# wang-xinyu/tensorrtx

Measured on AMD Instinct MI355X. Metric: images/sec @ batch=32 640x640 fp16 (yolov8n conv backbone + YoloLayer decode + NMS), higher is better.
Workload: dtype f16

## Files before the change

### include/trtx_hip.h

```cpp
#ifndef TRTX_HIP_H_
#define TRTX_HIP_H_

#include <stddef.h>
#include <stdint.h>

#ifdef __cplusplus
extern "C" {
#endif

#ifndef TRTX_NO_HIP_TYPES
struct ihipStream_t;
typedef struct ihipStream_t* trtx_stream_t;
#endif

#define TRTX_ABI_VERSION 1
#define TRTX_OK 0
#define TRTX_ERR_INVALID 1
#define TRTX_ERR_HIP 2
#define TRTX_ERR_WORKSPACE 3
#define TRTX_ERR_UNSUPPORTED 4
#define TRTX_ERR_NO_DEVICE 5
#define TRTX_ERR_IO 6
#define TRTX_ERR_STATE 7

const char* trtx_status_string(int32_t status);
int32_t trtx_abi_version(void);
int32_t trtx_device_count(void);


size_t trtx_yolo_decode_workspace(int batch, int net_h, int net_w, const int* strides, int n_levels);
int32_t trtx_yolo_decode(const float* const* inputs, int n_levels, int batch, int classes, int net_h, int net_w,
                         const int* strides, int max_out, float* output, void* workspace, size_t workspace_bytes,
                         trtx_stream_t stream);

int32_t trtx_yolo_decode_ex(const float* const* inputs, int n_levels, int batch, int classes, int net_h, int net_w,
                            const int* strides, int max_out, int n_kpt, float kpt_conf, int is_seg, int is_pose, int is_obb,
                            float* output, void* workspace, size_t workspace_bytes, trtx_stream_t stream);
size_t trtx_yolo_head_decode_workspace(int batch, int net_h, int net_w, const int* strides, int n_levels);
int32_t trtx_yolo_head_decode_nhwc(const void* const* heads, const int* ld, int n_levels, int batch, int classes,
                                   int net_h, int net_w, const int* strides, const float* dfl_weights, int max_out,
                                   float* output, void* workspace, size_t workspace_bytes, trtx_stream_t stream);
int32_t trtx_yolo_head_decode_nhwc_f32(const void* const* heads, const int* ld, int n_levels, int batch, int classes,
                                   int net_h, int net_w, const int* strides, const float* dfl_weights, int max_out,
                                   float* output, void* workspace, size_t workspace_bytes, trtx_stream_t stream);
int32_t trtx_yolo_task_head_decode_nhwc(const void* const* heads, const int* ld, const void* const* branches, const int* branch_ld,
                                        int n_levels, int batch, int classes, int net_h, int net_w, const int* strides,
                                        const float* dfl_weights, int max_out, int is_seg, int is_pose, int is_obb, int n_kpt,
                                        float kpt_conf, float* output, void* workspace, size_t workspace_bytes, trtx_stream_t stream);
int32_t trtx_yolo_task_head_decode_nhwc_f32(const void* const* heads, const int* ld, const void* const* branches, const int* branch_ld,
                                            int n_levels, int batch, int classes, int net_h, int net_w, const int* strides,
                                            const float* dfl_weights, int max_out, int is_seg, int is_pose, int is_obb, int n_kpt,
                                            float kpt_conf, float* output, void* workspace, size_t workspace_bytes, trtx_stream_t stream);

size_t trtx_yolo_nms_workspace(int batch);
int32_t trtx_yolo_nms(const float* decode_out, int batch, int max_out, float conf_thresh, float nms_thresh,
                      int32_t* keep_idx, int32_t* keep_cnt, float* keep_det, void* workspace, size_t workspace_bytes,
                      trtx_stream_t stream);


size_t trtx_yolov5_decode_workspace(int batch, const int* grid_w, const int* grid_h, int n_levels);
int32_t trtx_yolov5_decode(const float* const* inputs, int n_levels, int batch, int classes, int net_h, int net_w,
                           const int* grid_w, const int* grid_h, const float* anchors, int max_out, int is_segmentation,
                           float* output, void* workspace, size_t workspace_bytes, trtx_stream_t stream);
size_t trtx_yolov5_head_decode_workspace(int batch, const int* grid_w, const int* grid_h, int n_levels);
int32_t trtx_yolov5_head_decode_nhwc(const void* const* heads, const int* ld, int n_levels, int batch, int classes, int net_h, int net_w,
                                     const int* grid_w, const int* grid_h, const float* anchors, int max_out, float* output,
                                     void* workspace, size_t workspace_bytes, trtx_stream_t stream);
int32_t trtx_yolov5_head_decode_nhwc_f32(const void* const* heads, const int* ld, int n_levels, int batch, int classes, int net_h, int net_w,
                                         const int* grid_w, const int* grid_h, const float* anchors, int max_out, float* output,
                                         void* workspace, size_t workspace_bytes, trtx_stream_t stream);
int32_t trtx_yolo_nms_obb(const float* decode_out, int batch, int max_out, float conf_thresh, float nms_thresh, int32_t* keep_idx,
                          int32_t* keep_cnt, float* keep_det, void* workspace, size_t workspace_bytes, trtx_stream_t stream);
int32_t trtx_yolo_postprocess_gpu_obb(const float* decode_out, int batch, int max_out, float conf_thresh, float nms_thresh, float* out,
                                      trtx_stream_t stream);
int32_t trtx_yolov5_nms(const float* decode_out, int batch, int max_out, float conf_thresh, float nms_thresh, int32_t* keep_idx,
                        int32_t* keep_cnt, float* keep_det, void* workspace, size_t workspace_bytes, trtx_stream_t stream);
int32_t trtx_seg_masks(const float* decode_out, int det_floats, int box_format, const int32_t* keep_idx, const int32_t* keep_cnt, int batch,
                       int max_out, int max_keep, const float* proto, int mask_h, int mask_w, int net_h, int net_w, float* masks,
                       trtx_stream_t stream);

void trtx_letterbox_matrix(int src_w, int src_h, int dst_w, int dst_h, float* d2s_out );
int32_t trtx_letterbox_batch(const void* const* src, const int* src_w, const int* src_h, int batch, float* dst, int dst_w, int dst_h,
                             trtx_stream_t stream);
int32_t trtx_preprocess_init(int max_image_size, int ring_depth);
void trtx_preprocess_destroy(void);
int32_t trtx_batch_preprocess(const void* const* src_host, const int* src_w, const int* src_h, int batch, float* dst, int dst_w, int dst_h,
                              trtx_stream_t stream);

int32_t trtx_yolo_postprocess_gpu(const float* decode_out, int batch, int max_out, float conf_thresh, float nms_thresh,
                                  float* out, trtx_stream_t stream);

int32_t trtx_mish(const float* in, float* out, size_t n, trtx_stream_t stream);

size_t trtx_retina_decode_output_floats(int net_h, int net_w);
size_t trtx_retina_decode_workspace(int batch, int net_h, int net_w);
int32_t trtx_retina_decode(const float* const* inputs, int batch, int net_h, int net_w, float* output, void* workspace,
                           size_t workspace_bytes, trtx_stream_t stream);
size_t trtx_retina_nms_workspace(int batch, int net_h, int net_w);
int32_t trtx_retina_nms(const float* decode_out, int batch, int net_h, int net_w, double conf_thresh, float nms_thresh,
                        int max_keep, int32_t* keep_idx, int32_t* keep_cnt, float* keep_det, void* workspace,
                        size_t workspace_bytes, trtx_stream_t stream);

size_t trtx_rpn_decode_workspace(int batch, int num_anchors, int height, int width);
int32_t trtx_rpn_decode(int batch, const float* scores, const float* deltas, int height, int width, int image_height,
                        int image_width, float stride, const float* anchors_host, int num_anchors, int top_n,
                        float* out_scores, float* out_boxes, void* workspace, size_t workspace_bytes,
                        trtx_stream_t stream);
size_t trtx_sorted_nms_workspace(int batch, int n);
int32_t trtx_rpn_nms(int batch, const float* scores, const float* boxes, int pre_nms_topk, int post_nms_topk,
                     float nms_thresh, float* out_boxes, void* workspace, size_t workspace_bytes,
                     trtx_stream_t stream);
int32_t trtx_roi_align(int batch, const float* boxes, const float* features, int pooler_resolution, float spatial_scale,
                       int sampling_ratio, int num_proposals, int channels, int feature_h, int feature_w, float* out,
                       trtx_stream_t stream);
int32_t trtx_roi_align_nhwc_f16(int batch, const float* boxes, const void* features, int ld_in, int pooler_resolution,
                                float spatial_scale, int sampling_ratio, int num_proposals, int channels, int feature_h,
                                int feature_w, void* out, int ld_out, trtx_stream_t stream);
int32_t trtx_roi_align_nhwc_f16_strided(int batch, const float* boxes, const void* features, int ld_in, int pooler_resolution,
                                        float spatial_scale, int sampling_ratio, int num_proposals, int channels, int feature_h,
                                        int feature_w, void* out, int ld_out, int bin_step, trtx_stream_t stream);
size_t trtx_predictor_decode_workspace(int batch, int num_boxes, int num_classes);
int32_t trtx_predictor_decode(int batch, const float* scores, const float* deltas, const float* proposals, int num_boxes,
                              int num_classes, int image_height, int image_width, const float* bbox_reg_weights_host,
                              float* out_scores, float* out_boxes, float* out_classes, void* workspace,
                              size_t workspace_bytes, trtx_stream_t stream);
int32_t trtx_batched_nms(int nms_method, int batch, const float* scores, const float* boxes, const float* classes,
                         int count, int detections_per_im, float nms_thresh, float* out_scores, float* out_boxes,
                         float* out_classes, void* workspace, size_t workspace_bytes, trtx_stream_t stream);

int32_t trtx_mask_rcnn_inference(int batch, const float* labels, const float* masks, int detections_per_im, int output_size,
                                 int num_classes, float* out_masks, trtx_stream_t stream);

#define TRTX_ACT_NONE 0
#define TRTX_ACT_RELU 1
#define TRTX_ACT_SIGMOID 2
#define TRTX_ACT_SILU 3
#define TRTX_ACT_LEAKY 4
#define TRTX_ACT_TANH 5
int32_t trtx_conv_packed_dims(int cout, int cin_pad, int kh, int kw, int32_t* cout_pad, int32_t* kpad, int32_t* bn);
int32_t trtx_conv_pack_weights_f16(const float* w_kcrs, int cout, int cin, int kh, int kw, int cin_pad,
                                   const float* ch_scale, uint16_t* packed);
int32_t trtx_op_conv2d_nhwc_f16(const void* in, int N, int H, int W, int Cin, int ld_in, const void* wpacked,
                                const float* bias, void* out, int Cout, int ld_out, int kh, int kw, int sh, int sw,
                                int ph, int pw, int act1, const void* residual, int ld_res, int act2,
                                trtx_stream_t stream);
int32_t trtx_op_conv2d_tactics(int N, int H, int W, int Cin, int ld_in, int Cout, int ld_out, int kh, int kw, int sh, int sw, int ph, int pw,
                               int has_residual, int ld_res, int32_t* out6, int32_t max_out);
int32_t trtx_op_conv_force_tactic(const int32_t* tactic6);
int32_t trtx_conv_packed_dims_f32(int cout, int cin_pad, int kh, int kw, int32_t* cout_pad, int32_t* kpad, int32_t* cink);
int32_t trtx_conv_pack_weights_f32(const float* w_kcrs, int cout, int cin, int kh, int kw, int cin_pad, const float* ch_scale, float* packed);
int32_t trtx_op_conv2d_nhwc_f32(const void* in, int N, int H, int W, int Cin, int ld_in, const void* wpacked, const float* bias, void* out, int Cout,
                                int ld_out, int kh, int kw, int sh, int sw, int ph, int pw, int act1, const void* residual, int ld_res, int act2,
                                const int32_t* tile4, trtx_stream_t stream);
int32_t trtx_op_conv2d_tactics_f32(int N, int H, int W, int Cin, int ld_in, int Cout, int ld_out, int kh, int kw, int sh, int sw, int ph, int pw,
                                   int has_residual, int ld_res, int32_t* out4, int32_t max_out);
int32_t trtx_conv_pack_weights_i8(const float* w_kcrs, int cout, int cin, int kh, int kw, const float* ch_scale, int8_t* packed, float* wscale_out,
                                  int32_t* cout_pad_out, int32_t* kpad_out);
int32_t trtx_op_conv2d_nhwc_i8(const void* in, int N, int H, int W, int Cin, int ld_in, const void* wpacked, const float* cscale, const float* bias, void* out,
                               int out_is_i8, float out_inv_scale, int Cout, int ld_out, int kh, int kw, int sh, int sw, int ph, int pw, int act1,
                               const void* residual, int res_is_i8, float res_scale, int ld_res, int act2, trtx_stream_t stream);
int32_t trtx_conv_pack_weights_grouped_f16(const float* w_kcrs, int cout, int cin_g, int kh, int kw, const float* ch_scale, uint16_t* packed,
                                           int32_t* kpad_out);
int32_t trtx_op_conv2d_grouped_nhwc_f16(const void* in, int N, int H, int W, int Cin, int ld_in, const void* wpacked, const float* bias, void* out,
                                        int Cout, int ld_out, int groups, int k, int pad, int act1, const void* residual, int ld_res, int act2,
                                        trtx_stream_t stream);
int32_t trtx_op_conv2d_dw_nhwc(const void* in, int dtype, int N, int H, int W, int C, int ld_in, const float* w_taps_c, const float* bias, void* out, int ld_out,
                               const void* residual, int ld_res, int k, int stride, int pad, int dilation, int act1, float alpha1, int act2, float alpha2,
                               trtx_stream_t stream);
int32_t trtx_op_psa_attention_f16(const void* qkv, int ld_qkv, void* out, int ld_out, void* vimg, int ld_v, int B, int heads, int N, int kd, int hd, float scale,
                                  trtx_stream_t stream);
int32_t trtx_op_area_attention_f16(const void* qkv, int ld_qkv, void* out, int ld_out, void* vimg, int ld_v, int B, int heads, int N, int area, int kd, int hd,
                                   float scale, trtx_stream_t stream);
int32_t trtx_op_poison_lds(void* device_word, trtx_stream_t stream);
int32_t trtx_op_nchw_f32_to_nhwc_f16(const float* in, void* out, int N, int C, int H, int W, int Cpad, int ld_out,
                                     trtx_stream_t stream);
int32_t trtx_op_nhwc_f16_to_nchw_f32(const void* in, float* out, int N, int C, int H, int W, int ld_in,
                                     trtx_stream_t stream);

typedef struct trtx_builder trtx_builder;
typedef struct trtx_network trtx_network;
typedef struct trtx_hostmem trtx_hostmem;
typedef struct trtx_engine trtx_engine;
typedef struct trtx_context trtx_context;
typedef struct trtx_plugin trtx_plugin;

#define TRTX_MAX_DIMS 8
typedef struct trtx_dims {
    int32_t nb;
    int64_t d[TRTX_MAX_DIMS];
} trtx_dims;

#define TRTX_DTYPE_FLOAT 0
#define TRTX_DTYPE_HALF 1
#define TRTX_DTYPE_INT8 2
#define TRTX_DTYPE_INT32 3
#define TRTX_ACTIVATION_RELU 0
#define TRTX_ACTIVATION_SIGMOID 1
#define TRTX_ACTIVATION_TANH 2
#define TRTX_ACTIVATION_LEAKY_RELU 3
#define TRTX_POOLING_MAX 0
#define TRTX_POOLING_AVERAGE 1
#define TRTX_ELEMENTWISE_SUM 0
#define TRTX_ELEMENTWISE_PROD 1
#define TRTX_ELEMENTWISE_MAX 2
#define TRTX_ELEMENTWISE_MIN 3
#define TRTX_ELEMENTWISE_SUB 4
#define TRTX_ELEMENTWISE_DIV 5
#define TRTX_ELEMENTWISE_POW 6
#define TRTX_SCALE_UNIFORM 0
#define TRTX_SCALE_CHANNEL 1
#define TRTX_SCALE_ELEMENTWISE 2
#define TRTX_REDUCE_SUM 0
#define TRTX_REDUCE_PROD 1
#define TRTX_REDUCE_MAX 2
#define TRTX_REDUCE_MIN 3
#define TRTX_REDUCE_AVG 4
#define TRTX_MATMUL_NONE 0
#define TRTX_MATMUL_TRANSPOSE 1
#define TRTX_MATMUL_VECTOR 2
#define TRTX_RESIZE_NEAREST 0
#define TRTX_RESIZE_LINEAR 1
#define TRTX_FLAG_FP16 0
#define TRTX_FLAG_INT8 1
#define TRTX_P_STRIDE 1
#define TRTX_P_PADDING 2
#define TRTX_P_DILATION 3
#define TRTX_P_GROUPS 4
#define TRTX_P_ALPHA 5
#define TRTX_P_BETA 6
#define TRTX_P_AXIS 7
#define TRTX_P_RESHAPE 8
#define TRTX_P_FIRST_TRANSPOSE 9
#define TRTX_P_SECOND_TRANSPOSE 10
#define TRTX_P_RESIZE_MODE 11
#define TRTX_P_RESIZE_SCALES 12
#define TRTX_P_RESIZE_OUT_DIMS 13
#define TRTX_P_AVG_EXCLUSIVE 14
#define TRTX_P_KERNEL 15
#define TRTX_P_NB_OUT 16

typedef struct trtx_plugin_vtbl {
    void* self;
    int32_t (*get_nb_outputs)(void* self);
    int32_t (*get_output_dims)(void* self, int32_t index, const trtx_dims* inputs, int32_t nb_inputs, trtx_dims* out);
    int32_t (*configure)(void* self, const trtx_dims* in, int32_t nb_in, const trtx_dims* out, int32_t nb_out,
                         int32_t max_batch);
    int32_t (*initialize)(void* self);
    void (*terminate)(void* self);
    size_t (*workspace_size)(void* self, int32_t max_batch);
    int32_t (*enqueue)(void* self, int32_t batch, const void* const* inputs, void* const* outputs, void* workspace,
                       trtx_stream_t stream);
    size_t (*serialization_size)(void* self);
    void (*serialize)(void* self, void* buffer);
    const char* (*plugin_type)(void* self);
    const char* (*plugin_version)(void* self);
    int32_t (*clone)(void* self, struct trtx_plugin_vtbl* out);
    void (*destroy)(void* self);
} trtx_plugin_vtbl;

typedef struct trtx_plugin_field {
    const char* name;
    const void* data;
    int32_t type;
    int32_t length;
} trtx_plugin_field;

typedef struct trtx_creator_vtbl {
    void* self;
    const char* (*plugin_name)(void* self);
    const char* (*plugin_version)(void* self);
    int32_t (*create)(void* self, const char* name, const trtx_plugin_field* fields, int32_t nb_fields,
                      trtx_plugin_vtbl* out);
    int32_t (*deserialize)(void* self, const char* name, const void* data, size_t length, trtx_plugin_vtbl* out);
} trtx_creator_vtbl;

int32_t trtx_registry_register(const trtx_creator_vtbl* creator);
int32_t trtx_registry_get(const char* name, const char* version, trtx_creator_vtbl* out);

typedef struct trtx_wts trtx_wts;
int32_t trtx_wts_load(const char* path, trtx_wts** out);
int32_t trtx_wts_count(const trtx_wts* w);
int32_t trtx_wts_entry(const trtx_wts* w, int32_t i, const char** name, const float** values, int64_t* count);
int32_t trtx_wts_find(const trtx_wts* w, const char* name, const float** values, int64_t* count);
void trtx_wts_free(trtx_wts* w);

int32_t trtx_builder_create(trtx_builder** out);
void trtx_builder_destroy(trtx_builder* b);
int32_t trtx_builder_set_max_batch(trtx_builder* b, int32_t n);
int32_t trtx_builder_set_flag(trtx_builder* b, int32_t flag, int32_t on);
int32_t trtx_builder_set_workspace(trtx_builder* b, size_t bytes);
typedef struct trtx_calibrator_vtbl {
    void* self;
    int32_t (*get_batch_size)(void* self);
    int32_t (*get_batch)(void* self, void** bindings, const char* const* names, int32_t nb_bindings);
    const void* (*read_cache)(void* self, size_t* length);
    void (*write_cache)(void* self, const void* cache, size_t length);
    int32_t (*get_algorithm)(void* self);
} trtx_calibrator_vtbl;
int32_t trtx_builder_set_max_aux_streams(trtx_builder* b, int32_t n);
int32_t trtx_builder_set_int8_calibrator(trtx_builder* b, const trtx_calibrator_vtbl* calibrator);
float trtx_int8_entropy_threshold(const double* hist, int32_t bins, float range);
float trtx_int8_clip_limited_threshold(const double* hist, int32_t bins, float range, float thr, double limit);
int32_t trtx_network_create(trtx_builder* b, uint32_t flags, trtx_network** out);
void trtx_network_destroy(trtx_network* n);
const char* trtx_network_last_error(const trtx_network* n);

int32_t trtx_add_input(trtx_network* n, const char* name, int32_t dtype, const trtx_dims* dims);
int32_t trtx_add_convolution(trtx_network* n, int32_t input, int32_t nb_out, int32_t kh, int32_t kw,
                             const float* kernel, int64_t kernel_count, const float* bias, int64_t bias_count);
int32_t trtx_add_deconvolution(trtx_network* n, int32_t input, int32_t nb_out, int32_t kh, int32_t kw,
                               const float* kernel, int64_t kernel_count, const float* bias, int64_t bias_count);
int32_t trtx_add_fully_connected(trtx_network* n, int32_t input, int32_t nb_out, const float* kernel,
                                 int64_t kernel_count, const float* bias, int64_t bias_count);
int32_t trtx_add_activation(trtx_network* n, int32_t input, int32_t type);
int32_t trtx_add_pooling(trtx_network* n, int32_t input, int32_t type, int32_t kh, int32_t kw);
int32_t trtx_add_scale(trtx_network* n, int32_t input, int32_t mode, const float* shift, int64_t shift_count,
                       const float* scale, int64_t scale_count, const float* power, int64_t power_count);
int32_t trtx_add_elementwise(trtx_network* n, int32_t a, int32_t b, int32_t op);
int32_t trtx_add_concatenation(trtx_network* n, const int32_t* inputs, int32_t nb_inputs);
int32_t trtx_add_slice(trtx_network* n, int32_t input, const trtx_dims* start, const trtx_dims* size,
                       const trtx_dims* stride);
int32_t trtx_add_shuffle(trtx_network* n, int32_t input);
int32_t trtx_add_resize(trtx_network* n, int32_t input);
int32_t trtx_add_softmax(trtx_network* n, int32_t input);
int32_t trtx_add_matrix_multiply(trtx_network* n, int32_t a, int32_t op_a, int32_t b, int32_t op_b);
int32_t trtx_add_constant(trtx_network* n, const trtx_dims* dims, const float* values, int64_t count);
int32_t trtx_add_reduce(trtx_network* n, int32_t input, int32_t op, uint32_t axes, int32_t keep_dims);
int32_t trtx_add_identity(trtx_network* n, int32_t input);
int32_t trtx_add_plugin_v2(trtx_network* n, const int32_t* inputs, int32_t nb_inputs, const trtx_plugin_vtbl* plugin);

int32_t trtx_layer_nb_outputs(const trtx_network* n, int32_t layer);
int32_t trtx_layer_output(const trtx_network* n, int32_t layer, int32_t index);
int32_t trtx_layer_set_name(trtx_network* n, int32_t layer, const char* name);
int32_t trtx_layer_set_ints(trtx_network* n, int32_t layer, int32_t param, const int32_t* v, int32_t count);
int32_t trtx_layer_set_floats(trtx_network* n, int32_t layer, int32_t param, const float* v, int32_t count);
int32_t trtx_layer_set_dims(trtx_network* n, int32_t layer, int32_t param, const trtx_dims* d);
int32_t trtx_tensor_get_dims(const trtx_network* n, int32_t tensor, trtx_dims* out);
int32_t trtx_tensor_set_name(trtx_network* n, int32_t tensor, const char* name);
const char* trtx_tensor_get_name(const trtx_network* n, int32_t tensor);
int32_t trtx_mark_output(trtx_network* n, int32_t tensor);

int32_t trtx_build_serialized(trtx_builder* b, trtx_network* n, trtx_hostmem** out);
const void* trtx_hostmem_data(const trtx_hostmem* m);
size_t trtx_hostmem_size(const trtx_hostmem* m);
void trtx_hostmem_destroy(trtx_hostmem* m);
int32_t trtx_hostmem_create(const void* data, size_t size, trtx_hostmem** out);
int32_t trtx_plan_describe(const void* plan, size_t size, int32_t lowered, char** json_out);
void trtx_string_free(char* s);

int32_t trtx_engine_deserialize(const void* plan, size_t size, trtx_engine** out);
int32_t trtx_engine_serialize(const trtx_engine* e, trtx_hostmem** out);
void trtx_engine_destroy(trtx_engine* e);
int32_t trtx_engine_nb_bindings(const trtx_engine* e);
int32_t trtx_engine_binding_index(const trtx_engine* e, const char* name);
const char* trtx_engine_binding_name(const trtx_engine* e, int32_t index);
int32_t trtx_engine_binding_is_input(const trtx_engine* e, int32_t index);
int32_t trtx_engine_binding_dims(const trtx_engine* e, int32_t index, trtx_dims* out);
int32_t trtx_engine_binding_dtype(const trtx_engine* e, int32_t index);
int32_t trtx_engine_max_batch(const trtx_engine* e);
size_t trtx_engine_device_memory(const trtx_engine* e);
int32_t trtx_engine_tactics(const trtx_engine* e, char** json_out);
int32_t trtx_engine_device(const trtx_engine* e);
int32_t trtx_context_create(trtx_engine* e, trtx_context** out);
void trtx_context_destroy(trtx_context* c);
int32_t trtx_context_enqueue(trtx_context* c, int32_t batch, void* const* bindings, trtx_stream_t stream);
int32_t trtx_context_enqueue_frames(trtx_context* c, int32_t batch, const void* const* frames, const int32_t* frame_w, const int32_t* frame_h,
                                    void* const* bindings, trtx_stream_t stream);
int32_t trtx_context_set_tensor_address(trtx_context* c, const char* name, void* ptr);
int32_t trtx_context_enqueue_v3(trtx_context* c, trtx_stream_t stream);
int32_t trtx_context_profile(trtx_context* c, int32_t batch, void* const* bindings, trtx_stream_t stream,
                             char** json_out);

#ifdef __cplusplus
}
#endif
#endif
```

### tensorrtx_amd/capi.py

```python
import ctypes
import os

_HERE = os.path.dirname(os.path.abspath(__file__))
_LIB = None


class TrtxError(RuntimeError):
    def __init__(self, status, what):
        self.status = status
        msg = lib().trtx_status_string(status).decode() if _LIB is not None else "?"
        super().__init__(f"{what}: status {status} ({msg})")


def lib_path() -> str:
    return os.environ.get("TRTX_HIP_LIB") or os.path.join(_HERE, "lib", "libtrtx_hip.so")


def hip_runtimes_mapped():
    seen = []
    with open("/proc/self/maps") as f:
        for line in f:
            path = line.rsplit(" ", 1)[-1].strip()
            if "libamdhip64" in os.path.basename(path) and path not in seen:
                seen.append(path)
    return seen


def _bind_hip_runtime():
    import torch


def lib() -> ctypes.CDLL:
    global _LIB
    if _LIB is None:
        p = lib_path()
        if not os.path.exists(p):
            raise ImportError(f"{p} is missing: run `python -c 'import __graft_entry__ as g; g.build()'` "
                              "(hipcc --offload-arch=gfx950); there is no CPU fallback")
        _bind_hip_runtime()
        L = ctypes.CDLL(p)
        rts = hip_runtimes_mapped()
        if len(rts) > 1:
            raise ImportError("two HIP runtimes are mapped in this process (%s): something dlopened a HIP library "
                              "before tensorrtx_amd/torch; import torch (or tensorrtx_amd) first" % ", ".join(rts))
        L.trtx_status_string.restype = ctypes.c_char_p
        L.trtx_status_string.argtypes = [ctypes.c_int32]
        L.trtx_yolo_decode_workspace.restype = ctypes.c_size_t
        _LIB = L
    return _LIB


def check(status, what):
    if status != 0:
        raise TrtxError(status, what)


def _stream():
    import torch
    return ctypes.c_void_p(torch.cuda.current_stream().cuda_stream)


def _p(t):
    return ctypes.c_void_p(t.data_ptr() if t is not None else 0)


DET_FLOATS = 90


def yolo_decode(inputs, classes, net_h, net_w, strides, max_out=1000, out=None):
    import torch
    L = lib()
    B = inputs[0].shape[0]
    n = len(inputs)
    ins = [x.contiguous() for x in inputs]
    for x in ins:
        assert x.is_cuda and x.dtype == torch.float32
    arr = (ctypes.c_void_p * n)(*[x.data_ptr() for x in ins])
    st = (ctypes.c_int * n)(*strides)
    ws_bytes = L.trtx_yolo_decode_workspace(B, net_h, net_w, st, n)
    ws = torch.empty(ws_bytes, dtype=torch.uint8, device=ins[0].device)
    if out is None:
        out = torch.empty((B, 1 + max_out * DET_FLOATS), dtype=torch.float32, device=ins[0].device)
    check(L.trtx_yolo_decode(arr, n, B, classes, net_h, net_w, st, max_out, _p(out), _p(ws),
                             ctypes.c_size_t(ws_bytes), _stream()), "trtx_yolo_decode")
    return out


def yolo_nms(decode_out, max_out=1000, conf_thresh=0.5, nms_thresh=0.45, with_dets=True):
    import torch
    L = lib()
    B = decode_out.shape[0]
    dev = decode_out.device
    keep_idx = torch.full((B, max_out), -1, dtype=torch.int32, device=dev)
    keep_cnt = torch.zeros((B,), dtype=torch.int32, device=dev)
    keep_det = torch.zeros((B, max_out, 6), dtype=torch.float32, device=dev) if with_dets else None
    L.trtx_yolo_nms_workspace.restype = ctypes.c_size_t
    ws_bytes = L.trtx_yolo_nms_workspace(B)
    ws = torch.empty((ws_bytes,), dtype=torch.uint8, device=dev)
    check(L.trtx_yolo_nms(_p(decode_out), B, max_out, ctypes.c_float(conf_thresh), ctypes.c_float(nms_thresh),
                          _p(keep_idx), _p(keep_cnt), _p(keep_det), _p(ws), ctypes.c_size_t(ws_bytes), _stream()),
          "trtx_yolo_nms")
    return keep_idx, keep_cnt, keep_det


def yolo_decode_ex(inputs, classes, net_h, net_w, strides, max_out=1000, nk=17, kpt_conf=0.0, seg=False, pose=False, obb=False):
    import torch
    L = lib()
    B, n = inputs[0].shape[0], len(inputs)
    ins = [x.contiguous() for x in inputs]
    arr = (ctypes.c_void_p * n)(*[x.data_ptr() for x in ins])
    st = (ctypes.c_int * n)(*strides)
    ws_bytes = L.trtx_yolo_decode_workspace(B, net_h, net_w, st, n)
    ws = torch.empty(ws_bytes, dtype=torch.uint8, device=ins[0].device)
    out = torch.zeros((B, 1 + max_out * DET_FLOATS), dtype=torch.float32, device=ins[0].device)
    check(L.trtx_yolo_decode_ex(arr, n, B, classes, net_h, net_w, st, max_out, nk, ctypes.c_float(kpt_conf), int(seg), int(pose), int(obb),
                                _p(out), _p(ws), ctypes.c_size_t(ws_bytes), _stream()), "trtx_yolo_decode_ex")
    return out


def _head_table(tensors):
    n = len(tensors)
    return (ctypes.c_void_p * n)(*[x.data_ptr() for x in tensors]), (ctypes.c_int * n)(*[x.shape[-1] for x in tensors])


def yolo_head_decode_nhwc(heads, classes, net_h, net_w, strides, dfl_w, max_out=1000):
    import torch
    L = lib()
    B, n = heads[0].shape[0], len(heads)
    hp, hl = _head_table(heads)
    st = (ctypes.c_int * n)(*strides)
    L.trtx_yolo_head_decode_workspace.restype = ctypes.c_size_t
    ws_bytes = L.trtx_yolo_head_decode_workspace(B, net_h, net_w, st, n)
    ws = torch.empty(ws_bytes, dtype=torch.uint8, device=heads[0].device)
    out = torch.zeros(B, 1 + max_out * DET_FLOATS, dtype=torch.float32, device=heads[0].device)
    fn = L.trtx_yolo_head_decode_nhwc_f32 if heads[0].dtype == torch.float32 else L.trtx_yolo_head_decode_nhwc
    check(fn(hp, hl, n, B, classes, net_h, net_w, st, _p(dfl_w), max_out, _p(out), _p(ws), ctypes.c_size_t(ws_bytes), _stream()),
          "trtx_yolo_head_decode_nhwc")
    return out


def yolo_task_head_decode_nhwc(heads, branches, classes, net_h, net_w, strides, dfl_w, max_out=1000, nk=17, kpt_conf=0.0, seg=False,
                               pose=False, obb=False):
    import torch
    L = lib()
    B, n = heads[0].shape[0], len(heads)
    hp, hl = _head_table(heads)
    bp, bl = _head_table(branches)
    st = (ctypes.c_int * n)(*strides)
    L.trtx_yolo_head_decode_workspace.restype = ctypes.c_size_t
    ws_bytes = L.trtx_yolo_head_decode_workspace(B, net_h, net_w, st, n)
    ws = torch.empty(ws_bytes, dtype=torch.uint8, device=heads[0].device)
    out = torch.zeros(B, 1 + max_out * DET_FLOATS, dtype=torch.float32, device=heads[0].device)
    fn = L.trtx_yolo_task_head_decode_nhwc_f32 if heads[0].dtype == torch.float32 else L.trtx_yolo_task_head_decode_nhwc
    check(fn(hp, hl, bp, bl, n, B, classes, net_h, net_w, st, _p(dfl_w), max_out, int(seg), int(pose), int(obb), nk, ctypes.c_float(kpt_conf),
             _p(out), _p(ws), ctypes.c_size_t(ws_bytes), _stream()), "trtx_yolo_task_head_decode_nhwc")
    return out


def yolo_nms_obb(decode_out, max_out=1000, conf_thresh=0.5, nms_thresh=0.45):
    import torch
    L = lib()
    B, dev = decode_out.shape[0], decode_out.device
    keep_idx = torch.full((B, max_out), -1, dtype=torch.int32, device=dev)
    keep_cnt = torch.zeros((B,), dtype=torch.int32, device=dev)
    keep_det = torch.zeros((B, max_out, 7), dtype=torch.float32, device=dev)
    L.trtx_yolo_nms_workspace.restype = ctypes.c_size_t
    ws_bytes = L.trtx_yolo_nms_workspace(B)
    ws = torch.empty((ws_bytes,), dtype=torch.uint8, device=dev)
    check(L.trtx_yolo_nms_obb(_p(decode_out), B, max_out, ctypes.c_float(conf_thresh), ctypes.c_float(nms_thresh), _p(keep_idx), _p(keep_cnt),
                              _p(keep_det), _p(ws), ctypes.c_size_t(ws_bytes), _stream()), "trtx_yolo_nms_obb")
    return keep_idx, keep_cnt, keep_det


def yolo_postprocess_gpu_obb(decode_out, max_out=1000, conf_thresh=0.5, nms_thresh=0.45):
    import torch
    out = torch.empty((decode_out.shape[0], 1 + max_out * 8), dtype=torch.float32, device=decode_out.device)
    check(lib().trtx_yolo_postprocess_gpu_obb(_p(decode_out), decode_out.shape[0], max_out, ctypes.c_float(conf_thresh), ctypes.c_float(nms_thresh),
                                              _p(out), _stream()), "trtx_yolo_postprocess_gpu_obb")
    return out


DET5_FLOATS = 38


def yolov5_decode(inputs, classes, net_h, net_w, grids, anchors, max_out=1000, is_seg=False):
    import numpy as np
    import torch
    L = lib()
    n = len(inputs)
    ins = [x.contiguous() for x in inputs]
    B, dev = ins[0].shape[0], ins[0].device
    arr = (ctypes.c_void_p * n)(*[x.data_ptr() for x in ins])
    gw = (ctypes.c_int * n)(*[g[0] for g in grids])
    gh = (ctypes.c_int * n)(*[g[1] for g in grids])
    an = np.ascontiguousarray(anchors, dtype=np.float32).reshape(n, 6)
    L.trtx_yolov5_decode_workspace.restype = ctypes.c_size_t
    ws_bytes = L.trtx_yolov5_decode_workspace(B, gw, gh, n)
    ws = torch.empty(max(ws_bytes, 256), dtype=torch.uint8, device=dev)
    out = torch.zeros((B, 1 + max_out * DET5_FLOATS), dtype=torch.float32, device=dev)
    check(L.trtx_yolov5_decode(arr, n, B, classes, net_h, net_w, gw, gh, an.ctypes.data_as(ctypes.c_void_p), max_out, 1 if is_seg else 0,
                               _p(out), _p(ws), ctypes.c_size_t(ws_bytes), _stream()), "trtx_yolov5_decode")
    return out


def yolov5_head_decode_nhwc(heads, classes, net_h, net_w, grids, anchors, max_out=1000):
    import numpy as np
    import torch
    L = lib()
    B, n, dev = heads[0].shape[0], len(heads), heads[0].device
    hp, hl = _head_table(heads)
    gw = (ctypes.c_int * n)(*[g[0] for g in grids])
    gh = (ctypes.c_int * n)(*[g[1] for g in grids])
    an = np.ascontiguousarray(anchors, dtype=np.float32).reshape(n, 6)
    L.trtx_yolov5_head_decode_workspace.restype = ctypes.c_size_t
    ws_bytes = L.trtx_yolov5_head_decode_workspace(B, gw, gh, n)
    ws = torch.empty(max(ws_bytes, 256), dtype=torch.uint8, device=dev)
    out = torch.zeros((B, 1 + max_out * DET5_FLOATS), dtype=torch.float32, device=dev)
    fn = L.trtx_yolov5_head_decode_nhwc_f32 if heads[0].dtype == torch.float32 else L.trtx_yolov5_head_decode_nhwc
    check(fn(hp, hl, n, B, classes, net_h, net_w, gw, gh, an.ctypes.data_as(ctypes.c_void_p), max_out, _p(out), _p(ws), ctypes.c_size_t(ws_bytes),
             _stream()), "trtx_yolov5_head_decode_nhwc")
    return out


def yolov5_nms(decode_out, max_out=1000, conf_thresh=0.5, nms_thresh=0.45):
    import torch
    L = lib()
    B, dev = decode_out.shape[0], decode_out.device
    keep_idx = torch.full((B, max_out), -1, dtype=torch.int32, device=dev)
    keep_cnt = torch.zeros((B,), dtype=torch.int32, device=dev)
    keep_det = torch.zeros((B, max_out, 6), dtype=torch.float32, device=dev)
    L.trtx_yolo_nms_workspace.restype = ctypes.c_size_t
    ws_bytes = L.trtx_yolo_nms_workspace(B)
    ws = torch.empty((ws_bytes,), dtype=torch.uint8, device=dev)
    check(L.trtx_yolov5_nms(_p(decode_out), B, max_out, ctypes.c_float(conf_thresh), ctypes.c_float(nms_thresh), _p(keep_idx), _p(keep_cnt),
                            _p(keep_det), _p(ws), ctypes.c_size_t(ws_bytes), _stream()), "trtx_yolov5_nms")
    return keep_idx, keep_cnt, keep_det


def seg_masks(decode_out, keep_idx, keep_cnt, proto, net_h, net_w, max_keep, box_format=0, out=None):
    import torch
    B, max_out = keep_idx.shape
    assert decode_out.shape[0] == B and (decode_out.shape[1] - 1) % max_out == 0
    det_floats = (decode_out.shape[1] - 1) // max_out
    assert proto.dim() == 4 and proto.shape[0] == B and proto.shape[1] == 32
    mask_h, mask_w = int(proto.shape[2]), int(proto.shape[3])
    for t, dt in ((decode_out, torch.float32), (keep_idx, torch.int32), (keep_cnt, torch.int32), (proto, torch.float32)):
        assert t.is_cuda and t.dtype == dt and t.is_contiguous()
    if out is None:
        out = torch.zeros((B, max(max_keep, 0), mask_h, mask_w), dtype=torch.float32, device=proto.device)
    assert out.is_cuda and out.dtype == torch.float32 and out.is_contiguous() and out.numel() >= B * max(max_keep, 0) * mask_h * mask_w
    check(lib().trtx_seg_masks(_p(decode_out), det_floats, box_format, _p(keep_idx), _p(keep_cnt), B, max_out, max_keep, _p(proto), mask_h,
                               mask_w, net_h, net_w, _p(out), _stream()), "trtx_seg_masks")
    return out


def yolo_postprocess_gpu(decode_out, max_out=1000, conf_thresh=0.5, nms_thresh=0.45):
    import torch
    B = decode_out.shape[0]
    out = torch.empty((B, 1 + max_out * 7), dtype=torch.float32, device=decode_out.device)
    check(lib().trtx_yolo_postprocess_gpu(_p(decode_out), B, max_out, ctypes.c_float(conf_thresh), ctypes.c_float(nms_thresh),
                                          _p(out), _stream()), "trtx_yolo_postprocess_gpu")
    return out


ACT = {"none": 0, "relu": 1, "sigmoid": 2, "silu": 3, "leaky": 4, "tanh": 5, "mish": 6}


def _hw(v):
    if isinstance(v, (tuple, list)):
        h, w = v
        return int(h), int(w)
    return int(v), int(v)


def pack_conv_weights_f16(w_kcrs, cin_pad=None, ch_scale=None):
    import numpy as np
    L = lib()
    w = np.ascontiguousarray(w_kcrs, dtype=np.float32)
    cout, cin, kh, kw = w.shape
    cin_pad = cin_pad or (cin + 7) // 8 * 8
    cp, kp, bn = ctypes.c_int32(), ctypes.c_int32(), ctypes.c_int32()
    check(L.trtx_conv_packed_dims(cout, cin_pad, kh, kw, ctypes.byref(cp), ctypes.byref(kp), ctypes.byref(bn)),
          "trtx_conv_packed_dims")
    packed = np.zeros((cp.value, kp.value), dtype=np.uint16)
    sc = None
    if ch_scale is not None:
        sc = np.ascontiguousarray(ch_scale, dtype=np.float32)
    check(L.trtx_conv_pack_weights_f16(w.ctypes.data_as(ctypes.c_void_p), cout, cin, kh, kw, cin_pad,
                                       sc.ctypes.data_as(ctypes.c_void_p) if sc is not None else None,
                                       packed.ctypes.data_as(ctypes.c_void_p)), "trtx_conv_pack_weights_f16")
    return packed, cp.value, kp.value, bn.value


def conv2d_nhwc_f16(x, wpacked, bias, cout, kh, kw, stride, pad, act1="none", residual=None, act2="none",
                    out=None, out_ld=None):
    import torch
    L = lib()
    N, H, W, Cin = x.shape
    (sh, sw), (ph, pw) = _hw(stride), _hw(pad)
    Ho = (H + 2 * ph - kh) // sh + 1
    Wo = (W + 2 * pw - kw) // sw + 1
    if out is None:
        out = torch.empty((N, Ho, Wo, cout), dtype=torch.float16, device=x.device)
    ld_out = out_ld or out.shape[-1]
    check(L.trtx_op_conv2d_nhwc_f16(_p(x), N, H, W, Cin, x.stride(2), _p(wpacked), _p(bias), _p(out), cout, ld_out,
                                    kh, kw, sh, sw, ph, pw, ACT[act1], _p(residual),
                                    residual.stride(2) if residual is not None else 0, ACT[act2], _stream()),
          "trtx_op_conv2d_nhwc_f16")
    return out


def pack_conv_weights_grouped_f16(w_kcrs, ch_scale=None):
    import numpy as np
    L = lib()
    w = np.ascontiguousarray(w_kcrs, dtype=np.float32)
    cout, cin_g, kh, kw = w.shape
    kp = ctypes.c_int32()
    check(L.trtx_conv_pack_weights_grouped_f16(w.ctypes.data_as(ctypes.c_void_p), cout, cin_g, kh, kw, None, None, ctypes.byref(kp)),
          "trtx_conv_pack_weights_grouped_f16 (dims)")
    packed = np.zeros((cout, kp.value), dtype=np.uint16)
    sc = None if ch_scale is None else np.ascontiguousarray(ch_scale, dtype=np.float32)
    check(L.trtx_conv_pack_weights_grouped_f16(w.ctypes.data_as(ctypes.c_void_p), cout, cin_g, kh, kw,
                                               sc.ctypes.data_as(ctypes.c_void_p) if sc is not None else None,
                                               packed.ctypes.data_as(ctypes.c_void_p), ctypes.byref(kp)), "trtx_conv_pack_weights_grouped_f16")
    return packed


def conv2d_grouped_nhwc_f16(x, wpacked, bias, cout, groups, k, pad, act1="none", residual=None, act2="none", out=None, out_ld=None):
    import torch
    N, H, W, Cin = x.shape
    if out is None:
        out = torch.empty((N, H + 2 * pad - k + 1, W + 2 * pad - k + 1, cout), dtype=torch.float16, device=x.device)
    check(lib().trtx_op_conv2d_grouped_nhwc_f16(_p(x), N, H, W, Cin, x.stride(2), _p(wpacked), _p(bias), _p(out), cout, out_ld or out.shape[-1], groups, k,
                                                pad, ACT[act1], _p(residual), residual.stride(2) if residual is not None else 0, ACT[act2], _stream()),
          "trtx_op_conv2d_grouped_nhwc_f16")
    return out


def conv2d_dw_nhwc(x, w, bias, k, stride, act1="none", residual=None, act2="none", out=None, out_ld=None, alpha1=0.1, alpha2=0.1, pad=None, dilation=1):
    import numpy as np
    import torch
    N, H, W, C = x.shape
    assert x.dtype in (torch.float16, torch.float32) and (residual is None or residual.dtype == x.dtype)
    pad = k // 2 if pad is None else pad
    Ho, Wo = (H + 2 * pad - dilation * (k - 1) - 1) // stride + 1, (W + 2 * pad - dilation * (k - 1) - 1) // stride + 1
    taps = np.ascontiguousarray(np.asarray(w, dtype=np.float32).reshape(C, k * k).T)
    wg = torch.from_numpy(taps).to(x.device)
    if out is None:
        out = torch.empty((N, Ho, Wo, C), dtype=x.dtype, device=x.device)
    assert out.dtype == x.dtype
    check(lib().trtx_op_conv2d_dw_nhwc(_p(x), 1 if x.dtype == torch.float16 else 0, N, H, W, C, x.stride(2), _p(wg), _p(bias), _p(out),
                                       out_ld or out.shape[-1], _p(residual), residual.stride(2) if residual is not None else 0, k, stride, pad, dilation,
                                       ACT[act1], ctypes.c_float(alpha1), ACT[act2], ctypes.c_float(alpha2), _stream()), "trtx_op_conv2d_dw_nhwc")
    return out


def _attention(fn, what, qkv, heads, scale, out, vimg, out_ld, v_ld, qkv_ld, kd, hd, extra):
    import torch
    B, N, _ = qkv.shape
    for t in (qkv, out, vimg):
        assert t.is_cuda and t.dtype == torch.float16
    check(fn(_p(qkv), qkv_ld or qkv.stride(1), _p(out), out_ld or out.stride(1), _p(vimg), v_ld or vimg.stride(1), B, heads, N, *extra, kd, hd,
             ctypes.c_float(scale), _stream()), what)
    return out, vimg


def psa_attention(qkv, heads, scale, out=None, vimg=None, out_ld=None, v_ld=None, qkv_ld=None, kd=32, hd=64):
    import torch
    B, N, _ = qkv.shape
    out = torch.empty((B, N, heads * hd), dtype=torch.float16, device=qkv.device) if out is None else out
    vimg = torch.empty((B, N, heads * hd), dtype=torch.float16, device=qkv.device) if vimg is None else vimg
    return _attention(lib().trtx_op_psa_attention_f16, "trtx_op_psa_attention_f16", qkv, heads, scale, out, vimg, out_ld, v_ld, qkv_ld, kd, hd, ())


def area_attention(qkv, heads, area, scale, out=None, vimg=None, out_ld=None, v_ld=None, qkv_ld=None, kd=32, hd=32):
    import torch
    B, N, _ = qkv.shape
    out = torch.empty((B, N, heads * hd), dtype=torch.float16, device=qkv.device) if out is None else out
    vimg = torch.empty((B, N, heads * hd), dtype=torch.float16, device=qkv.device) if vimg is None else vimg
    return _attention(lib().trtx_op_area_attention_f16, "trtx_op_area_attention_f16", qkv, heads, scale, out, vimg, out_ld, v_ld, qkv_ld, kd, hd, (area,))


def pack_conv_weights_f32(w_kcrs, cin_pad=None, ch_scale=None):
    import numpy as np
    L = lib()
    w = np.ascontiguousarray(w_kcrs, dtype=np.float32)
    cout, cin, kh, kw = w.shape
    cin_pad = cin_pad or (cin + 3) // 4 * 4
    cp, kp, ck = ctypes.c_int32(), ctypes.c_int32(), ctypes.c_int32()
    check(L.trtx_conv_packed_dims_f32(cout, cin_pad, kh, kw, ctypes.byref(cp), ctypes.byref(kp), ctypes.byref(ck)), "trtx_conv_packed_dims_f32")
    packed = np.zeros((cp.value, kp.value), dtype=np.float32)
    sc = np.ascontiguousarray(ch_scale, dtype=np.float32) if ch_scale is not None else None
    check(L.trtx_conv_pack_weights_f32(w.ctypes.data_as(ctypes.c_void_p), cout, cin, kh, kw, cin_pad,
                                       sc.ctypes.data_as(ctypes.c_void_p) if sc is not None else None,
                                       packed.ctypes.data_as(ctypes.c_void_p)), "trtx_conv_pack_weights_f32")
    return packed, cp.value, kp.value, ck.value


def conv2d_nhwc_f32(x, wpacked, bias, cout, kh, kw, stride, pad, act1="none", residual=None, act2="none", out=None, out_ld=None, tile=None):
    import torch
    L = lib()
    N, H, W, Cin = x.shape
    if bias is not None and bias.numel() < (cout + 15) // 16 * 16:
        raise ValueError(f"bias holds {bias.numel()} floats, the fp32 tile reads cout_pad = {(cout + 15) // 16 * 16}")
    (sh, sw), (ph, pw) = _hw(stride), _hw(pad)
    Ho = (H + 2 * ph - kh) // sh + 1
    Wo = (W + 2 * pw - kw) // sw + 1
    if out is None:
        out = torch.empty((N, Ho, Wo, cout), dtype=torch.float32, device=x.device)
    ld_out = out_ld or out.shape[-1]
    t2 = (ctypes.c_int32 * 4)(*tile) if tile is not None else None
    check(L.trtx_op_conv2d_nhwc_f32(_p(x), N, H, W, Cin, x.stride(2), _p(wpacked), _p(bias), _p(out), cout, ld_out, kh, kw, sh, sw, ph, pw,
                                    ACT[act1], _p(residual), residual.stride(2) if residual is not None else 0, ACT[act2], t2, _stream()),
          "trtx_op_conv2d_nhwc_f32")
    return out


def conv2d_tactics_f32(N, H, W, Cin, Cout, k, stride, pad, residual=False, ld_in=None, ld_out=None, ld_res=None, max_out=32):
    arr = (ctypes.c_int32 * (4 * max_out))()
    (kh, kw), (sh, sw), (ph, pw) = _hw(k), _hw(stride), _hw(pad)
    n = lib().trtx_op_conv2d_tactics_f32(N, H, W, Cin, ld_in or Cin, Cout, ld_out or Cout, kh, kw, sh, sw, ph, pw, 1 if residual else 0,
                                         (ld_res or Cout) if residual else 0, arr, max_out)
    return [(arr[4 * i], arr[4 * i + 1], arr[4 * i + 2], arr[4 * i + 3]) for i in range(n)]


def poison_lds(sync=True):
    import torch
    w = torch.zeros(4, dtype=torch.int32, device="cuda")
    check(lib().trtx_op_poison_lds(_p(w), _stream()), "trtx_op_poison_lds")
    if sync:
        torch.cuda.synchronize()


def conv2d_tactics(N, H, W, Cin, Cout, k, stride, pad, residual=False, ld_in=None, ld_out=None, ld_res=None, max_out=32):
    arr = (ctypes.c_int32 * (6 * max_out))()
    (kh, kw), (sh, sw), (ph, pw) = _hw(k), _hw(stride), _hw(pad)
    n = lib().trtx_op_conv2d_tactics(N, H, W, Cin, ld_in or Cin, Cout, ld_out or Cout, kh, kw, sh, sw, ph, pw, 1 if residual else 0,
                                     (ld_res or Cout) if residual else 0, arr, max_out)
    return [tuple(arr[6 * i + j] for j in range(6)) for i in range(n)]


def conv_force_tactic(tactic=None):
    if tactic is None:
        check(lib().trtx_op_conv_force_tactic(None), "trtx_op_conv_force_tactic")
    else:
        check(lib().trtx_op_conv_force_tactic((ctypes.c_int32 * 6)(*tactic)), "trtx_op_conv_force_tactic")


def pack_conv_weights_i8(w_kcrs, ch_scale=None):
    import numpy as np
    L = lib()
    w = np.ascontiguousarray(w_kcrs, dtype=np.float32)
    cout, cin, kh, kw = w.shape
    cp, kp = ctypes.c_int32(), ctypes.c_int32()
    check(L.trtx_conv_pack_weights_i8(w.ctypes.data_as(ctypes.c_void_p), cout, cin, kh, kw, None, None, None, ctypes.byref(cp), ctypes.byref(kp)),
          "trtx_conv_pack_weights_i8 (dims)")
    packed = np.zeros((cp.value, kp.value), dtype=np.int8)
    wscale = np.zeros((cp.value,), dtype=np.float32)
    sc = None if ch_scale is None else np.ascontiguousarray(ch_scale, dtype=np.float32)
    check(L.trtx_conv_pack_weights_i8(w.ctypes.data_as(ctypes.c_void_p), cout, cin, kh, kw,
                                      sc.ctypes.data_as(ctypes.c_void_p) if sc is not None else None, packed.ctypes.data_as(ctypes.c_void_p),
                                      wscale.ctypes.data_as(ctypes.c_void_p), ctypes.byref(cp), ctypes.byref(kp)), "trtx_conv_pack_weights_i8")
    return packed, wscale


def conv2d_nhwc_i8(x_i8, wpacked, cscale, bias, cout, kh, kw, stride, pad, act1="none", out_scale=None, residual=None, res_scale=1.0,
                   act2="none", out=None, out_ld=None):
    import torch
    N, H, W, Cin = x_i8.shape
    (sh, sw), (ph, pw) = _hw(stride), _hw(pad)
    Ho, Wo = (H + 2 * ph - kh) // sh + 1, (W + 2 * pw - kw) // sw + 1
    if out is None:
        out = torch.empty((N, Ho, Wo, cout), dtype=torch.int8 if out_scale else torch.float16, device=x_i8.device)
    res_i8 = residual is not None and residual.dtype == torch.int8
    check(lib().trtx_op_conv2d_nhwc_i8(_p(x_i8), N, H, W, Cin, x_i8.stride(2), _p(wpacked), _p(cscale), _p(bias), _p(out), 1 if out_scale else 0,
                                       ctypes.c_float(1.0 / out_scale if out_scale else 0.0), cout, out_ld or out.shape[-1], kh, kw, sh, sw, ph, pw, ACT[act1],
                                       _p(residual), 1 if res_i8 else 0, ctypes.c_float(res_scale), residual.stride(2) if residual is not None else 0,
                                       ACT[act2], _stream()), "trtx_op_conv2d_nhwc_i8")
    return out
```

### tensorrtx_amd/csrc/kernels/conv_stem.hip

```cpp
#include <hip/hip_fp16.h>
#include <hip/hip_runtime.h>
#include <stdint.h>
#include <stdlib.h>
#include <string.h>

#include "../common.h"
#include "act.h"
#include "kernels.h"

namespace trtx {
namespace {

template <int COUT>
__global__ __launch_bounds__(256) void conv_stem_kernel(const ConvArgs p) {
    extern __shared__ __attribute__((aligned(16))) float s_w[];
    const float* __restrict__ w = static_cast<const float*>(p.wgt);
    const int K = p.kh * p.kw * p.Cin;
    for (int i = threadIdx.x; i < K * COUT; i += 256) s_w[i] = w[i];
    __syncthreads();
    const long m = (long)blockIdx.x * 256 + threadIdx.x;
    if (m >= p.M) return;
    const int wo = (int)(m % p.Wo);
    const long t = m / p.Wo;
    const int ho = (int)(t % p.Ho);
    const long n = t / p.Ho;
    const float* __restrict__ in = static_cast<const float*>(p.in) + n * p.Cin * p.H * p.W;
    float acc[COUT];
#pragma unroll
    for (int c = 0; c < COUT; ++c) acc[c] = p.bias ? p.bias[c] : 0.f;
    const int hi0 = ho * p.stride_h - p.pad_h, wi0 = wo * p.stride_w - p.pad_w;
    int tap = 0;
    for (int c = 0; c < p.Cin; ++c) {
        const float* plane = in + (long)c * p.H * p.W;
        for (int r = 0; r < p.kh; ++r) {
            const int hi = hi0 + r;
            const bool hok = (unsigned)hi < (unsigned)p.H;
            for (int q = 0; q < p.kw; ++q, ++tap) {
                const int wi = wi0 + q;
                float x = 0.f;
                if (hok && (unsigned)wi < (unsigned)p.W) x = plane[(long)hi * p.W + wi];
                const float4* wr = reinterpret_cast<const float4*>(s_w + tap * COUT);
#pragma unroll
                for (int c4 = 0; c4 < COUT / 4; ++c4) {
                    const float4 wv = wr[c4];
                    acc[c4 * 4 + 0] = fmaf(x, wv.x, acc[c4 * 4 + 0]);
                    acc[c4 * 4 + 1] = fmaf(x, wv.y, acc[c4 * 4 + 1]);
                    acc[c4 * 4 + 2] = fmaf(x, wv.z, acc[c4 * 4 + 2]);
                    acc[c4 * 4 + 3] = fmaf(x, wv.w, acc[c4 * 4 + 3]);
                }
            }
        }
    }
    _Float16* __restrict__ out = static_cast<_Float16*>(p.out) + m * p.ld_out;
#pragma unroll
    for (int c8 = 0; c8 < COUT / 8; ++c8) {
        half8 v;
#pragma unroll
        for (int e = 0; e < 8; ++e) v[e] = round_to_half(act_stem(acc[c8 * 8 + e], p.act1, p.alpha1));
        *reinterpret_cast<half8*>(out + c8 * 8) = v;
    }
}

typedef __attribute__((address_space(3))) void* lds_ptr_t;

constexpr int kStemTW = 64, kStemTH = 4;

struct StemGeom {
    int PR, PCA;
    int tiles_x, tiles_y;
    int chunks;
};

struct FramePack {
    StemFrame img[kStemMaxFrames];
};

struct AxisSample {
    float pos;
    int low;
    float l;
};
__device__ __forceinline__ AxisSample frame_axis(float m, float z, int d) {
#pragma clang fp contract(off)
    AxisSample a;
    a.pos = m * (float)d + z + 0.5f;
    a.low = (int)floorf(a.pos);
    a.l = a.pos - (float)a.low;
    return a;
}
__device__ __forceinline__ void frame_pixel(const StemFrame& im, const AxisSample& cx, const AxisSample& cy, float& r, float& g, float& b) {
#pragma clang fp contract(off)
    float c0, c1, c2;
    if (cx.pos <= -1 || cx.pos >= im.w || cy.pos <= -1 || cy.pos >= im.h) {
        c0 = c1 = c2 = 128.0f;
    } else {
        const int x_low = cx.low, y_low = cy.low, x_high = x_low + 1, y_high = y_low + 1;
        const float lx = cx.l, ly = cy.l, hx = 1 - lx, hy = 1 - ly;
        const float w1 = hy * hx, w2 = hy * lx, w3 = ly * hx, w4 = ly * lx;
        const uint8_t* base = static_cast<const uint8_t*>(im.src);
        const size_t line = (size_t)im.w * 3;
        float v[4][3];
#pragma unroll
        for (int q = 0; q < 4; ++q) {
            const int yy = q < 2 ? y_low : y_high, xx = (q & 1) ? x_high : x_low;
            const bool in = (q < 2 ? y_low >= 0 : y_high < im.h) && ((q & 1) ? x_high < im.w : x_low >= 0);
            const uint8_t* px = base + (size_t)(in ? yy : 0) * line + (size_t)(in ? xx : 0) * 3;
#pragma unroll
            for (int c = 0; c < 3; ++c) v[q][c] = in ? (float)px[c] : 128.0f;
        }
        c0 = w1 * v[0][0] + w2 * v[1][0] + w3 * v[2][0] + w4 * v[3][0];
        c1 = w1 * v[0][1] + w2 * v[1][1] + w3 * v[2][1] + w4 * v[3][1];
        c2 = w1 * v[0][2] + w2 * v[1][2] + w3 * v[2][2] + w4 * v[3][2];
    }
    r = c2 / 255.0f;
    g = c1 / 255.0f;
    b = c0 / 255.0f;
}

template <int NFRAG, int KS>
struct StemRegs {
    half8 wf[NFRAG][KS];
    int l_off[KS][8];
    float bias4[NFRAG][4];
};
template <int NFRAG, int KS>
__device__ __forceinline__ void stem_setup(const ConvArgs& p, const StemGeom& g, StemRegs<NFRAG, KS>& R);
template <int NFRAG, int KS>
__device__ __forceinline__ void stem_compute(const ConvArgs& p, const StemGeom& g, const StemRegs<NFRAG, KS>& R, const float* s_patch, int n, int tx0, int ty0, int shift);
template <int NFRAG, int KS>
__device__ __forceinline__ void stem_stage2(const ConvArgs& p, const StemGeom& g, const float* s_patch, int n, int tx0, int ty0, int shift) {
    StemRegs<NFRAG, KS> R;
    stem_setup<NFRAG, KS>(p, g, R);
    stem_compute<NFRAG, KS>(p, g, R, s_patch, n, tx0, ty0, shift);
}

template <int NFRAG, int KS>
__global__ __launch_bounds__(256) void conv_stem_frames_kernel(const ConvArgs p, const StemGeom g, const FramePack fr) {
    extern __shared__ __attribute__((aligned(16))) float s_patch[];
    const int tid = threadIdx.x;
    int t = blockIdx.x;
    const int tx0 = (t % g.tiles_x) * kStemTW;
    t /= g.tiles_x;
    const int ty0 = (t % g.tiles_y) * kStemTH;
    const int n = t / g.tiles_y;
    const int hi_start = ty0 * p.stride_h - p.pad_h;
    const int wi_start = tx0 * p.stride_w - p.pad_w;
    const int al_start = (wi_start >= 0 ? wi_start : wi_start - 3) / 4 * 4;
    const int shift = wi_start - al_start;
    const StemFrame& im = fr.img[n];
    const int plane = g.PR * g.PCA;
    const float inv_pca = 1.0f / (float)g.PCA;
    for (int e = tid; e < plane; e += 256) {
        int pr = (int)((float)e * inv_pca);
        int pc = e - pr * g.PCA;
        if (pc < 0) { --pr; pc += g.PCA; }
        if (pc >= g.PCA) { ++pr; pc -= g.PCA; }
        const int hi = hi_start + pr, wi = al_start + pc;
        float r = 0.f, gg = 0.f, b = 0.f;
        if ((unsigned)hi < (unsigned)p.H && (unsigned)wi < (unsigned)p.W) {
            const AxisSample cx = frame_axis(im.d2s[0], im.d2s[2], wi), cy = frame_axis(im.d2s[4], im.d2s[5], hi);
            frame_pixel(im, cx, cy, r, gg, b);
        }
        s_patch[e] = r;
        s_patch[plane + e] = gg;
        s_patch[2 * plane + e] = b;
    }
    __syncthreads();
    stem_stage2<NFRAG, KS>(p, g, s_patch, n, tx0, ty0, shift);
}

template <int NFRAG, int KS>
__global__ __launch_bounds__(256) void conv_stem_lds_kernel(const ConvArgs p, const StemGeom g, unsigned in_bytes, int total_tiles) {
    extern __shared__ __attribute__((aligned(16))) float s_patch[];
    const int tid = threadIdx.x;
    const int wave = tid >> 6;
    StemRegs<NFRAG, KS> R;
    stem_setup<NFRAG, KS>(p, g, R);
    for (int tile = blockIdx.x; tile < total_tiles; tile += gridDim.x) {
    int t = tile;
    const int tx0 = (t % g.tiles_x) * kStemTW;
    t /= g.tiles_x;
    const int ty0 = (t % g.tiles_y) * kStemTH;
    const int n = t / g.tiles_y;
    const int hi_start = ty0 * p.stride_h - p.pad_h;
    const int wi_start = tx0 * p.stride_w - p.pad_w;
    const int al_start = (wi_start >= 0 ? wi_start : wi_start - 3) / 4 * 4;
    const int shift = wi_start - al_start;
    {
        const __amdgpu_buffer_rsrc_t rs = __builtin_amdgcn_make_buffer_rsrc(const_cast<void*>(p.in), 0, in_bytes, 0x00020000);
        const int cpr = g.PCA / 4;
        const float inv_cpr = 1.0f / (float)cpr, inv_pr = 1.0f / (float)g.PR;
        for (int base = 0; base < g.chunks; base += 256) {
            const int ci = base + tid;
            int row = (int)((float)ci * inv_cpr);
            int cq = ci - row * cpr;
            if (cq < 0) { --row; cq += cpr; }
            if (cq >= cpr) { ++row; cq -= cpr; }
            int c = (int)((float)row * inv_pr);
            int pr = row - c * g.PR;
            if (pr < 0) { --c; pr += g.PR; }
            if (pr >= g.PR) { ++c; pr -= g.PR; }
            const int hi = hi_start + pr, wi = al_start + cq * 4;
            const bool ok = ci < g.chunks && (unsigned)hi < (unsigned)p.H && wi >= 0 && wi + 3 < p.W;
            const unsigned off = ok ? (unsigned)(((((long)n * p.Cin + c) * p.H + hi) * p.W + wi) * 4) : 0x80000000u;
            __builtin_amdgcn_raw_ptr_buffer_load_lds(rs, (lds_ptr_t)(s_patch + (size_t)(base + wave * 64) * 4), 16, off, 0, 0, 0);
        }
    }
    asm volatile("s_waitcnt vmcnt(0)" ::: "memory");
    __syncthreads();
    if (p.W & 3) {
        const int cpr = g.PCA / 4, rows = p.Cin * g.PR, wtail = p.W & ~3;
        const int cq = (wtail - al_start) >> 2;
        if (cq >= 0 && cq < cpr && wtail >= al_start) {
            const float* __restrict__ src = static_cast<const float*>(p.in);
            for (int rrow = tid; rrow < rows; rrow += 256) {
                const int c = rrow / g.PR, pr = rrow - c * g.PR, hi = hi_start + pr;
                if ((unsigned)hi >= (unsigned)p.H) continue;
                const size_t base = (((size_t)n * p.Cin + c) * p.H + hi) * p.W;
                for (int e = 0; e < 4; ++e)
                    if (wtail + e < p.W) s_patch[((size_t)rrow * cpr + cq) * 4 + e] = src[base + wtail + e];
            }
        }
        __syncthreads();
    }
    stem_compute<NFRAG, KS>(p, g, R, s_patch, n, tx0, ty0, shift);
    __syncthreads();
    }
}

template <int NFRAG, int KS>
__device__ __forceinline__ void stem_setup(const ConvArgs& p, const StemGeom& g, StemRegs<NFRAG, KS>& R) {
    const int lane = threadIdx.x & 63;
    const int khw = p.kh * p.kw;
    const int K = khw * p.Cin;
    const float* __restrict__ w = static_cast<const float*>(p.wgt);
    const int kq = (lane >> 4) * 8;
    auto& wf = R.wf;
    auto& l_off = R.l_off;
    auto& bias4 = R.bias4;
    const float inv_khw = 1.0f / (float)khw, inv_kw = 1.0f / (float)p.kw;
#pragma unroll
    for (int ks = 0; ks < KS; ++ks)
#pragma unroll
        for (int e = 0; e < 8; ++e) {
            const int k = ks * 32 + kq + e;
            const int c = (int)(((float)k + 0.5f) * inv_khw), rem = k - c * khw;
            const int r = (int)(((float)rem + 0.5f) * inv_kw), q = rem - r * p.kw;
            l_off[ks][e] = k < K ? (c * g.PR + r) * g.PCA + q : 0;
#pragma unroll
            for (int j = 0; j < NFRAG; ++j) {
                const int co = j * 16 + (lane & 15);
                const float wv = w[(size_t)(k < K ? k : K - 1) * p.Cout + (co < p.Cout ? co : p.Cout - 1)];
                wf[j][ks][e] = (k < K && co < p.Cout) ? (_Float16)wv : (_Float16)0.f;
            }
        }
    const int ch4 = (lane >> 4) * 4;
    const float* __restrict__ bsrc = p.bias ? p.bias : w;
#pragma unroll
    for (int j = 0; j < NFRAG; ++j)
#pragma unroll
        for (int e = 0; e < 4; ++e) {
            const int co = j * 16 + ch4 + e;
            const float bv = bsrc[co < p.Cout ? co : p.Cout - 1];
            bias4[j][e] = (p.bias && co < p.Cout) ? bv : 0.f;
        }
}

template <int NFRAG, int KS>
__device__ __forceinline__ void stem_compute(const ConvArgs& p, const StemGeom& g, const StemRegs<NFRAG, KS>& R, const float* s_patch, int n, int tx0, int ty0,
                                             int shift) {
    const int tid = threadIdx.x;
    const int lane = tid & 63;
    const int wave = tid >> 6;
    const int ch4 = (lane >> 4) * 4;
    const auto& wf = R.wf;
    const auto& l_off = R.l_off;
    const auto& bias4 = R.bias4;
    _Float16* __restrict__ out = static_cast<_Float16*>(p.out);
#pragma nounroll
    for (int gi = 0; gi < 4; ++gi) {
        const int ty = wave, tx = gi * 16 + (lane & 15);
        const int ho = ty0 + ty, wo = tx0 + tx;
        const float* src = s_patch + (ty * p.stride_h) * g.PCA + tx * p.stride_w + shift;
        floatx4 acc[NFRAG];
#pragma unroll
        for (int j = 0; j < NFRAG; ++j) acc[j] = floatx4{0.f, 0.f, 0.f, 0.f};
#pragma unroll
        for (int ks = 0; ks < KS; ++ks) {
            half8 xf;
#pragma unroll
            for (int e = 0; e < 8; ++e) xf[e] = (_Float16)src[l_off[ks][e]];
#pragma unroll
            for (int j = 0; j < NFRAG; ++j) acc[j] = __builtin_amdgcn_mfma_f32_16x16x32_f16(wf[j][ks], xf, acc[j], 0, 0, 0);
        }
        if (ho >= p.Ho || wo >= p.Wo) continue;
        const long m = ((long)n * p.Ho + ho) * p.Wo + wo;
#pragma unroll
        for (int j = 0; j < NFRAG; ++j) {
            const int co = j * 16 + ch4;
            if (co >= p.Cout) continue;
            half4 o;
            if (p.act1 == ACT_SILU) {
#pragma unroll
                for (int e = 0; e < 4; ++e) {
                    const float x = acc[j][e] + bias4[j][e];
                    o[e] = round_to_half(x * __builtin_amdgcn_rcpf(1.0f + __expf(-x)));
                }
            } else if (p.act1 == ACT_RELU) {
#pragma unroll
                for (int e = 0; e < 4; ++e) {
                    const float x = acc[j][e] + bias4[j][e];
                    o[e] = (_Float16)(x > 0.f ? x : 0.f);
                }
            } else {
#pragma unroll
                for (int e = 0; e < 4; ++e) o[e] = round_to_half(act_stem(acc[j][e] + bias4[j][e], p.act1, p.alpha1));
            }
            *reinterpret_cast<half4*>(out + m * p.ld_out + co) = o;
        }
    }
}

template <int NFRAG, int KS>
void launch_lds(const ConvArgs& a, hipStream_t s) {
    StemGeom g;
    g.PR = (kStemTH - 1) * a.stride_h + a.kh;
    g.PCA = ((kStemTW - 1) * a.stride_w + a.kw + 3 + 3) / 4 * 4;
    g.tiles_x = (a.Wo + kStemTW - 1) / kStemTW;
    g.tiles_y = (a.Ho + kStemTH - 1) / kStemTH;
    g.chunks = a.Cin * g.PR * g.PCA / 4;
    const size_t lds = (size_t)((g.chunks + 255) / 256 * 256) * 16;
    const unsigned in_bytes = (unsigned)((size_t)a.N * a.Cin * a.H * a.W * 4);
    const int total = a.N * g.tiles_x * g.tiles_y;
    static thread_local int resident[3] = {-1, 0, 0};
    int dev = 0;
    if (hipGetDevice(&dev) != hipSuccess) dev = 0;
    if (resident[0] != dev || resident[1] != (int)lds || resident[2] <= 0) {
        int per_cu = 0, cus = 0;
        if (hipOccupancyMaxActiveBlocksPerMultiprocessor(&per_cu, conv_stem_lds_kernel<NFRAG, KS>, 256, lds) != hipSuccess || per_cu < 1) per_cu = 1;
        if (hipDeviceGetAttribute(&cus, hipDeviceAttributeMultiprocessorCount, dev) != hipSuccess || cus < 1) cus = 256;
        (void)hipGetLastError();
        resident[0] = dev;
        resident[1] = (int)lds;
        resident[2] = per_cu * cus;
    }
    const int grid = total < resident[2] ? total : resident[2];
    hipLaunchKernelGGL((conv_stem_lds_kernel<NFRAG, KS>), dim3((unsigned)grid), dim3(256), lds, s, a, g, in_bytes, total);
}

template <int NFRAG, int KS>
void launch_frames(const ConvArgs& a0, const StemFrame* frames, hipStream_t s) {
    StemGeom g;
    g.PR = (kStemTH - 1) * a0.stride_h + a0.kh;
    g.PCA = ((kStemTW - 1) * a0.stride_w + a0.kw + 3 + 3) / 4 * 4;
    g.tiles_x = (a0.Wo + kStemTW - 1) / kStemTW;
    g.tiles_y = (a0.Ho + kStemTH - 1) / kStemTH;
    g.chunks = a0.Cin * g.PR * g.PCA / 4;
    const size_t lds = (size_t)((g.chunks + 255) / 256 * 256) * 16;
    for (int n0 = 0; n0 < a0.N; n0 += kStemMaxFrames) {
        ConvArgs a = a0;
        a.N = a0.N - n0 < kStemMaxFrames ? a0.N - n0 : kStemMaxFrames;
        a.M = a.N * a.Ho * a.Wo;
        a.out = static_cast<char*>(a0.out) + (size_t)n0 * a.Ho * a.Wo * a.ld_out * 2;
        FramePack fr;
        memset(&fr, 0, sizeof(fr));
        for (int i = 0; i < a.N; ++i) fr.img[i] = frames[n0 + i];
        hipLaunchKernelGGL((conv_stem_frames_kernel<NFRAG, KS>), dim3((unsigned)(a.N * g.tiles_x * g.tiles_y)), dim3(256), lds, s, a, g, fr);
    }
}

template <int COUT>
void launch(const ConvArgs& a, hipStream_t s) {
    const size_t lds = (size_t)a.kh * a.kw * a.Cin * COUT * sizeof(float);
    hipLaunchKernelGGL(conv_stem_kernel<COUT>, dim3((unsigned)((a.M + 255) / 256)), dim3(256), lds, s, a);
}

}

bool conv_stem_supported(const ConvArgs& a) {
    const bool cout_ok = a.Cout == 8 || a.Cout == 16 || a.Cout == 32 || a.Cout == 64;
    return cout_ok && a.Cin >= 1 && a.Cin <= 4 && a.groups == 1 && a.dil_h == 1 && a.dil_w == 1 && !a.residual &&
           a.act2 == ACT_NONE && (size_t)a.kh * a.kw * a.Cin * a.Cout * 4 <= 48 * 1024;
}

int32_t conv_stem_nchw_f32(const ConvArgs& a, hipStream_t s) {
    if (!conv_stem_supported(a) || a.ld_out % 8 || (reinterpret_cast<uintptr_t>(a.out) & 15)) return TRTX_ERR_UNSUPPORTED;
    const int K = a.kh * a.kw * a.Cin;
    const size_t patch = (size_t)a.Cin * ((kStemTH - 1) * a.stride_h + a.kh) * ((kStemTW - 1) * a.stride_w + a.kw + 9) * 4;
    if (a.Cout % 16 == 0 && K <= 160 && patch <= 60 * 1024 &&
        (size_t)a.N * a.Cin * a.H * a.W * 4 < 2000000000u && (reinterpret_cast<uintptr_t>(a.in) & 15) == 0) {
        const int ks = K <= 32 ? 1 : 5;
        bool done = true;
        if (a.Cout == 16 && ks == 1) launch_lds<1, 1>(a, s);
        else if (a.Cout == 32 && ks == 1) launch_lds<2, 1>(a, s);
        else if (a.Cout == 64 && ks == 1) launch_lds<4, 1>(a, s);
        else if (a.Cout == 16 && ks == 5) launch_lds<1, 5>(a, s);
        else if (a.Cout == 32 && ks == 5) launch_lds<2, 5>(a, s);
        else if (a.Cout == 64 && ks == 5) launch_lds<4, 5>(a, s);
        else done = false;
        if (done) return check_launch("conv_stem_nchw_f32");
    }
    switch (a.Cout) {
        case 8: launch<8>(a, s); break;
        case 16: launch<16>(a, s); break;
        case 32: launch<32>(a, s); break;
        case 64: launch<64>(a, s); break;
        default: return TRTX_ERR_UNSUPPORTED;
    }
    return check_launch("conv_stem_nchw_f32");
}

int32_t conv_stem_frames_f32(const ConvArgs& a, const StemFrame* frames, hipStream_t s) {
    if (!frames || !conv_stem_supported(a) || a.ld_out % 8 || (reinterpret_cast<uintptr_t>(a.out) & 15) || a.Cin != 3) return TRTX_ERR_UNSUPPORTED;
    const int K = a.kh * a.kw * a.Cin;
    const size_t patch = (size_t)a.Cin * ((kStemTH - 1) * a.stride_h + a.kh) * ((kStemTW - 1) * a.stride_w + a.kw + 9) * 4;
    if (a.Cout % 16 || K > 160 || patch > 60 * 1024) return TRTX_ERR_UNSUPPORTED;
    for (int i = 0; i < a.N; ++i)
        if (!frames[i].src || frames[i].w < 1 || frames[i].h < 1) return TRTX_ERR_INVALID;
    const int ks = K <= 32 ? 1 : 5;
    if (a.Cout == 16 && ks == 1) launch_frames<1, 1>(a, frames, s);
    else if (a.Cout == 32 && ks == 1) launch_frames<2, 1>(a, frames, s);
    else if (a.Cout == 64 && ks == 1) launch_frames<4, 1>(a, frames, s);
    else if (a.Cout == 16 && ks == 5) launch_frames<1, 5>(a, frames, s);
    else if (a.Cout == 32 && ks == 5) launch_frames<2, 5>(a, frames, s);
    else if (a.Cout == 64 && ks == 5) launch_frames<4, 5>(a, frames, s);
    else return TRTX_ERR_UNSUPPORTED;
    return check_launch("conv_stem_frames_f32");
}

}
```

### tensorrtx_amd/csrc/kernels/kernels.h

```cpp
#pragma once
#include <hip/hip_runtime.h>
#include <stddef.h>
#include <stdint.h>

namespace trtx {

enum Act : int { ACT_NONE = 0, ACT_RELU = 1, ACT_SIGMOID = 2, ACT_SILU = 3, ACT_LEAKY = 4, ACT_TANH = 5,
                 ACT_MISH = 6  };
enum DType : int { DT_F32 = 0, DT_F16 = 1, DT_I8 = 2 };
inline size_t dtype_size(int dt) { return dt == DT_F16 ? 2 : (dt == DT_I8 ? 1 : 4); }
enum EwOp : int { EW_SUM = 0, EW_PROD = 1, EW_MAX = 2, EW_MIN = 3, EW_SUB = 4, EW_DIV = 5, EW_POW = 6 };
enum PoolOp : int { POOL_MAX = 0, POOL_AVG = 1 };

enum Ws : int {
    WS_AUTO = 0,
    WS_OFF = 1,
    WS_ON = 2,
    WS_PATCH = 3,
    WS_F32_REGS = 5,
    WS_F32_ROLES = 6,
    WS_RES3 = 7,
    WS_RES1 = 8,
};
enum Wsk : int {
    WSK_RULE = 0,
    WSK_OFF = 1,
    WSK_ON = 2,
};

struct ConvArgs {
    const void* in;
    const void* wgt;
    const float* bias;
    void* out;
    const void* residual;
    int N, H, W, Cin, ld_in;
    int Ho, Wo, Cout, Cout_pad, ld_out, ld_res;
    int kh, kw, stride_h, stride_w, pad_h, pad_w, dil_h, dil_w, groups;
    int K, Kpad, M;
    int act1, act2;
    float alpha1, alpha2;
    int bn;
    int scalar_out;
    int CinK;
    int bk;
    int in_i8, out_i8, res_i8;
    const float* cscale;
    float out_inv_scale, res_scale;
    int bm;
    int t_wsk;
    int t_ws;
    int t_rs;
    const void* up_in;
    int up_C, up_ld, up_H, up_W;
    int f32;
    int k_pinned;
};

struct ConvTactic {
    int bn, bk, bm;
    int wsk, ws;
};

struct LaunchProbe {
    hipEvent_t start = nullptr, stop = nullptr;
    int launches = 0;
};
void conv_set_launch_probe(LaunchProbe* p);
LaunchProbe* conv_launch_probe();

int conv_igemm_pick_bn(int cout);
int conv_igemm_pick_bk(int cin, int taps);
int conv_igemm_pick_cink(int cin, int bk);
bool conv_igemm_supported(const ConvArgs& a);
void conv_pack_weights_i8(const float* w_kcrs, int cout, int cin, int kh, int kw, int cink, const float* ch_scale, int cout_pad, int kpad,
                          int8_t* packed, float* wscale_out);
int32_t conv_igemm_f16(const ConvArgs& a, hipStream_t s);
int conv_tactics(const ConvArgs& a, ConvTactic* out, int max_out, bool work_efficient_only = false);
void conv_apply_tactic(ConvArgs* a, const ConvTactic& t);
constexpr int kMaxConvGroup = 4;
bool conv_igemm_group_supported(const ConvArgs* a, int n);
int32_t conv_igemm_group_f16(const ConvArgs* a, int n, hipStream_t s);
bool conv_gemm256_possible(const ConvArgs& a);
bool conv_gemm256_worthwhile(const ConvArgs& a);
int32_t conv_gemm256_f16(const ConvArgs& a, hipStream_t s);
int conv_igemm_f32_pick_cink(int cin);
bool conv_igemm_f32_supported(const ConvArgs& a);
int32_t conv_igemm_f32(const ConvArgs& a, hipStream_t s);
int conv_tactics_f32(const ConvArgs& a, ConvTactic* out, int max_out);
void conv_pack_weights_igemm_f32(const float* w_kcrs, int cout, int cin, int kh, int kw, int cink, int kpad, int cout_pad, const float* ch_scale, float* packed);
bool conv_res_possible(const ConvArgs& a);
bool conv_res_group_possible(const ConvArgs* a, int n);
int32_t conv_res_f16(const ConvArgs* a, int n, hipStream_t s);
bool conv_res1_possible(const ConvArgs& a);
int32_t conv_res1_f16(const ConvArgs& a, hipStream_t s);
bool conv_ws_supported(const ConvArgs& a);
int32_t conv_ws_f16(const ConvArgs& a, hipStream_t s);
int32_t poison_lds(unsigned* device_word, hipStream_t s);
bool conv_stem_supported(const ConvArgs& a);
int32_t conv_stem_nchw_f32(const ConvArgs& a, hipStream_t s);
bool conv_stem_f32_supported(const ConvArgs& a);
int32_t conv_stem_nchw_f32_out_f32(const ConvArgs& a, hipStream_t s);
constexpr int kStemMaxFrames = 64;
struct StemFrame {
    const void* src;
    int w, h;
    float d2s[6];
};
int32_t conv_stem_frames_f32(const ConvArgs& a, const StemFrame* frames, hipStream_t s);
int32_t conv_direct(const ConvArgs& a, int dtype, hipStream_t s);
bool conv_dw_supported(const ConvArgs& a);
bool psa_attention_supported(int kd, int hd);
int32_t psa_attention_f16(const void* qkv, int ld_qkv, void* out, int ld_out, void* vimg, int ld_v, int B, int heads, int N, int kd, int hd,
                          float scale, hipStream_t s);
bool area_attention_supported(int kd, int hd);
int32_t area_attention_f16(const void* qkv, int ld_qkv, void* out, int ld_out, void* vimg, int ld_v, int B, int heads, int N, int area, int kd,
                           int hd, float scale, hipStream_t s);
int32_t conv_dw(const ConvArgs& a, int dtype, hipStream_t s);
bool conv_grouped_supported(const ConvArgs& a);
int conv_grouped_kpad(const ConvArgs& a);
int32_t conv_grouped(const ConvArgs& a, hipStream_t s);
int32_t deconv_direct(const ConvArgs& a, int dtype, hipStream_t s);

int32_t nchw_f32_to_nhwc(const float* in, void* out, int dtype, int N, int C, int H, int W, int Cpad, int ld_out,
                         hipStream_t s);
int32_t nhwc_to_nchw_f32(const void* in, int dtype, float* out, int N, int C, int H, int W, int ld_in, hipStream_t s);

int32_t nhwc_maxpool_chain3_f16(const void* in, void* o1, void* o2, void* o3, int N, int H, int W, int C, int ld_in, int ld1,
                                int ld2, int ld3, int k, hipStream_t s, int f32 = 0);
int32_t nhwc_depth_to_space_f16(const void* in, void* out, int N, int H, int W, int C, int bh, int bw, int ld_in, int ld_out,
                                hipStream_t s);
int32_t nhwc_pool(const void* in, void* out, int dtype, int op, int N, int H, int W, int C, int ld_in, int Ho, int Wo,
                  int ld_out, int kh, int kw, int sh, int sw, int ph, int pw, int avg_exclusive, hipStream_t s);
int32_t nhwc_resize_nearest(const void* in, void* out, int dtype, int N, int H, int W, int C, int ld_in, int Ho,
                            int Wo, int ld_out, hipStream_t s);
int32_t nhwc_elementwise(const void* a, const void* b, void* out, int dtype, int op, long pixels, int C, int ld_a,
                         int ld_b, int ld_out, hipStream_t s);
int32_t nhwc_activation(const void* in, void* out, int dtype, int act, float alpha, long pixels, int C, int ld_in,
                        int ld_out, hipStream_t s);
int32_t nhwc_scale(const void* in, void* out, int dtype, const float* scale, const float* shift, long pixels, int C,
                   int ld_in, int ld_out, hipStream_t s);
int32_t nhwc_copy(const void* in, void* out, int dtype, long pixels, int C, int ld_in, int ld_out, hipStream_t s);
int32_t nhwc_reduce_hw_avg(const void* in, void* out, int dtype, int N, int HW, int C, int ld_in, int ld_out,
                           hipStream_t s);

int32_t nhwc_absmax_f16(const void* x, long pixels, int C, int ld, unsigned* out_float_bits, hipStream_t s);
int32_t nhwc_hist_f16(const void* x, long pixels, int C, int ld, float range, unsigned long long* hist8192, hipStream_t s);
int32_t nhwc_resize_nearest_i8(const void* in, void* out, int N, int H, int W, int C, int ld_in, int Ho, int Wo, int ld_out, float ratio,
                               hipStream_t s);

struct StridedView {
    int rank;
    long shape[6];
    long stride_in[6];
    long stride_in2[6];
};
int32_t lin_gather(const float* in, float* out, const StridedView& v, hipStream_t s);
int32_t lin_scatter(const float* in, float* out, const StridedView& v, hipStream_t s);
int32_t lin_elementwise(const float* a, const float* b, float* out, int op, const StridedView& v, hipStream_t s);
int32_t lin_activation(const float* in, float* out, int act, float alpha, long n, hipStream_t s);
int32_t lin_softmax(const float* in, float* out, long outer, long axis, long inner, hipStream_t s);
int32_t lin_matmul(const float* A, const float* B, float* C, int batch, int M, int N, int K, int ta, int tb,
                   long bsA, long bsB, hipStream_t s, int binner = 1, long bsA2 = 0, long bsB2 = 0);
int32_t lin_reduce(const float* in, float* out, int op , long outer, long axis, long inner,
                   hipStream_t s);
int32_t lin_scale(const float* in, float* out, const float* scale, const float* shift, const float* power, int mode,
                  long outer, long C, long inner, hipStream_t s);

}
```

### tensorrtx_amd/csrc/ops_capi.cpp

```cpp
#include <hip/hip_runtime.h>
#include <stdlib.h>
#include <string.h>

#include <vector>

#include "common.h"
#include "options.h"
#include "kernels/kernels.h"
#include "runtime/pack.h"

using namespace trtx;

extern "C" const char* trtx_status_string(int32_t s) {
    switch (s) {
        case TRTX_OK: return "ok";
        case TRTX_ERR_INVALID: return "invalid argument";
        case TRTX_ERR_HIP: return "HIP error";
        case TRTX_ERR_WORKSPACE: return "workspace too small";
        case TRTX_ERR_UNSUPPORTED: return "unsupported configuration";
        case TRTX_ERR_NO_DEVICE: return "no HIP device";
        case TRTX_ERR_IO: return "I/O or parse error";
        case TRTX_ERR_STATE: return "invalid call order";
        default: return "unknown status";
    }
}

extern "C" int32_t trtx_abi_version(void) {
    return TRTX_ABI_VERSION;
}

extern "C" int32_t trtx_device_count(void) {
    int n = 0;
    if (hipGetDeviceCount(&n) != hipSuccess) {
        (void)hipGetLastError();
        return 0;
    }
    return n;
}

extern "C" int32_t trtx_conv_packed_dims(int cout, int cin_pad, int kh, int kw, int32_t* cout_pad, int32_t* kpad,
                                         int32_t* bn) {
    if (cout < 1 || cin_pad < 1 || kh < 1 || kw < 1) return TRTX_ERR_INVALID;
    const int b = conv_igemm_pick_bn(cout);
    if (bn) *bn = b;
    if (cout_pad) *cout_pad = (cout + b - 1) / b * b;
    if (kpad) {
        const int bk = conv_igemm_pick_bk(cin_pad, kh * kw);
        *kpad = (kh * kw * conv_igemm_pick_cink(cin_pad, bk) + bk - 1) / bk * bk;
    }
    return TRTX_OK;
}

extern "C" int32_t trtx_conv_pack_weights_f16(const float* w_kcrs, int cout, int cin, int kh, int kw, int cin_pad,
                                              const float* ch_scale, uint16_t* packed) {
    if (!w_kcrs || !packed || cin_pad < cin) return TRTX_ERR_INVALID;
    const int bk = conv_igemm_pick_bk(cin_pad, kh * kw);
    pack_conv_weights_f16(w_kcrs, cout, cin, kh, kw, conv_igemm_pick_cink(cin_pad, bk), bk, ch_scale, packed);
    return TRTX_OK;
}

static ConvArgs op_conv_args(int N, int H, int W, int Cin, int ld_in, int Cout, int ld_out, int kh, int kw, int sh, int sw, int ph, int pw,
                             int act1, int has_res, int ld_res, int act2) {
    ConvArgs a{};
    a.N = N; a.H = H; a.W = W; a.Cin = Cin; a.ld_in = ld_in;
    a.Ho = (H + 2 * ph - kh) / sh + 1;
    a.Wo = (W + 2 * pw - kw) / sw + 1;
    a.Cout = Cout;
    a.bn = conv_igemm_pick_bn(Cout);
    a.Cout_pad = (Cout + a.bn - 1) / a.bn * a.bn;
    a.ld_out = ld_out; a.ld_res = ld_res;
    a.kh = kh; a.kw = kw; a.stride_h = sh; a.stride_w = sw; a.pad_h = ph; a.pad_w = pw; a.dil_h = 1; a.dil_w = 1;
    a.groups = 1;
    a.bk = conv_igemm_pick_bk(Cin, kh * kw);
    a.CinK = conv_igemm_pick_cink(Cin, a.bk);
    a.K = kh * kw * a.CinK;
    a.Kpad = (a.K + a.bk - 1) / a.bk * a.bk;
    a.M = N * a.Ho * a.Wo;
    a.act1 = act1; a.act2 = act2; a.alpha1 = 0.1f; a.alpha2 = 0.1f;
    a.scalar_out = (Cout % 8 || ld_out % 8 || (has_res && ld_res % 8)) ? 1 : 0;
    return a;
}

static bool g_force_tactic = false;
static ConvTactic g_forced{};

extern "C" int32_t trtx_op_conv_force_tactic(const int32_t* t) {
    if (t && t[5] != 0) return TRTX_ERR_UNSUPPORTED;
    g_force_tactic = t != nullptr;
    if (t) g_forced = ConvTactic{t[0], t[1], t[2], t[3], t[4]};
    return TRTX_OK;
}

extern "C" int32_t trtx_op_conv2d_tactics(int N, int H, int W, int Cin, int ld_in, int Cout, int ld_out, int kh, int kw, int sh, int sw, int ph,
                                          int pw, int has_residual, int ld_res, int32_t* out6, int32_t max_out) {
    if (!out6 || max_out < 1 || N < 1 || kh < 1 || kw < 1 || sh < 1 || sw < 1) return 0;
    ConvArgs a = op_conv_args(N, H, W, Cin, ld_in, Cout, ld_out, kh, kw, sh, sw, ph, pw, 0, has_residual, ld_res, 0);
    a.residual = has_residual ? reinterpret_cast<const void*>(1) : nullptr;
    std::vector<ConvTactic> t(max_out);
    const int n = conv_tactics(a, t.data(), max_out);
    for (int i = 0; i < n; ++i) {
        out6[6 * i + 0] = t[i].bn; out6[6 * i + 1] = t[i].bk; out6[6 * i + 2] = t[i].bm; out6[6 * i + 3] = t[i].wsk; out6[6 * i + 4] = t[i].ws;
        out6[6 * i + 5] = 0;
    }
    return n;
}

extern "C" int32_t trtx_op_conv2d_nhwc_f16(const void* in, int N, int H, int W, int Cin, int ld_in, const void* wpacked,
                                           const float* bias, void* out, int Cout, int ld_out, int kh, int kw, int sh,
                                           int sw, int ph, int pw, int act1, const void* residual, int ld_res,
                                           int act2, trtx_stream_t stream) {
    ConvArgs a = op_conv_args(N, H, W, Cin, ld_in, Cout, ld_out, kh, kw, sh, sw, ph, pw, act1, residual != nullptr, ld_res, act2);
    a.in = in;
    a.wgt = wpacked;
    a.bias = bias;
    a.out = out;
    a.residual = residual;
    if (reinterpret_cast<uintptr_t>(out) & 15) a.scalar_out = 1;
    if (g_force_tactic) conv_apply_tactic(&a, g_forced);
    const int reps = options().op_reps;
    int32_t st = TRTX_OK;
    for (int r = 0; r < reps && st == TRTX_OK; ++r) st = conv_igemm_f16(a, stream);
    return st;
}

extern "C" int32_t trtx_conv_pack_weights_grouped_f16(const float* w_kcrs, int cout, int cin_g, int kh, int kw, const float* ch_scale, uint16_t* packed,
                                                      int32_t* kpad_out) {
    if (!w_kcrs || cout < 1 || cin_g < 1 || kh < 1 || kw < 1) return TRTX_ERR_INVALID;
    const int kpad = (kh * kw * cin_g + 31) / 32 * 32;
    if (kpad_out) *kpad_out = kpad;
    if (packed) pack_conv_weights_grouped_f16(w_kcrs, cout, cin_g, kh, kw, kpad, ch_scale, packed);
    return TRTX_OK;
}

extern "C" int32_t trtx_op_conv2d_grouped_nhwc_f16(const void* in, int N, int H, int W, int Cin, int ld_in, const void* wpacked, const float* bias, void* out,
                                                   int Cout, int ld_out, int groups, int k, int pad, int act1, const void* residual, int ld_res, int act2,
                                                   trtx_stream_t stream) {
    if (N < 1 || H < 1 || W < 1 || Cin < 1 || Cout < 1 || groups < 1 || k < 1 || pad < 0 || H + 2 * pad < k || W + 2 * pad < k) return TRTX_ERR_INVALID;
    ConvArgs a{};
    a.in = in; a.wgt = wpacked; a.bias = bias; a.out = out; a.residual = residual;
    a.N = N; a.H = H; a.W = W; a.Cin = Cin; a.ld_in = ld_in;
    a.Ho = H + 2 * pad - k + 1;
    a.Wo = W + 2 * pad - k + 1;
    a.Cout = Cout; a.Cout_pad = Cout; a.ld_out = ld_out; a.ld_res = ld_res;
    a.kh = k; a.kw = k; a.stride_h = 1; a.stride_w = 1; a.pad_h = pad; a.pad_w = pad; a.dil_h = 1; a.dil_w = 1;
    a.groups = groups;
    a.K = k * k * (Cin / groups);
    a.Kpad = conv_grouped_kpad(a);
    a.M = N * a.Ho * a.Wo;
    a.act1 = act1; a.act2 = act2; a.alpha1 = 0.1f; a.alpha2 = 0.1f;
    const int reps = options().op_reps;
    int32_t st = TRTX_OK;
    for (int r = 0; r < reps && st == TRTX_OK; ++r) st = conv_grouped(a, static_cast<hipStream_t>(stream));
    return st;
}

extern "C" int32_t trtx_op_conv2d_dw_nhwc(const void* in, int dtype, int N, int H, int W, int C, int ld_in, const float* w_taps_c, const float* bias, void* out,
                                          int ld_out, const void* residual, int ld_res, int k, int stride, int pad, int dilation, int act1, float alpha1,
                                          int act2, float alpha2, trtx_stream_t stream) {
    if (!in || !w_taps_c || !out || N < 1 || H < 1 || W < 1 || C < 1 || k < 1 || stride < 1 || pad < 0 || dilation < 1) return TRTX_ERR_INVALID;
    if (dtype != DT_F16 && dtype != DT_F32) return TRTX_ERR_UNSUPPORTED;
    if (H + 2 * pad < dilation * (k - 1) + 1 || W + 2 * pad < dilation * (k - 1) + 1) return TRTX_ERR_INVALID;
    ConvArgs a{};
    a.in = in; a.wgt = w_taps_c; a.bias = bias; a.out = out; a.residual = residual;
    a.N = N; a.H = H; a.W = W; a.Cin = C; a.ld_in = ld_in;
    a.Ho = (H + 2 * pad - dilation * (k - 1) - 1) / stride + 1;
    a.Wo = (W + 2 * pad - dilation * (k - 1) - 1) / stride + 1;
    a.Cout = C; a.Cout_pad = C; a.ld_out = ld_out; a.ld_res = ld_res;
    a.kh = k; a.kw = k; a.stride_h = stride; a.stride_w = stride; a.pad_h = pad; a.pad_w = pad; a.dil_h = dilation; a.dil_w = dilation;
    a.groups = C;
    a.K = k * k;
    a.Kpad = a.K;
    a.M = N * a.Ho * a.Wo;
    a.act1 = act1; a.act2 = act2; a.alpha1 = alpha1; a.alpha2 = alpha2;
    a.f32 = dtype == DT_F32;
    return conv_dw(a, dtype, static_cast<hipStream_t>(stream));
}

extern "C" int32_t trtx_op_psa_attention_f16(const void* qkv, int ld_qkv, void* out, int ld_out, void* vimg, int ld_v, int B, int heads, int N, int kd, int hd,
                                             float scale, trtx_stream_t stream) {
    if (!qkv || !out || !vimg) return TRTX_ERR_INVALID;
    return psa_attention_f16(qkv, ld_qkv, out, ld_out, vimg, ld_v, B, heads, N, kd, hd, scale, static_cast<hipStream_t>(stream));
}

extern "C" int32_t trtx_op_area_attention_f16(const void* qkv, int ld_qkv, void* out, int ld_out, void* vimg, int ld_v, int B, int heads, int N, int area,
                                              int kd, int hd, float scale, trtx_stream_t stream) {
    if (!qkv || !out || !vimg) return TRTX_ERR_INVALID;
    return area_attention_f16(qkv, ld_qkv, out, ld_out, vimg, ld_v, B, heads, N, area, kd, hd, scale, static_cast<hipStream_t>(stream));
}

static ConvArgs op_conv_args_f32(int N, int H, int W, int Cin, int ld_in, int Cout, int ld_out, int kh, int kw, int sh, int sw, int ph, int pw,
                                 int act1, int has_res, int ld_res, int act2) {
    ConvArgs a{};
    a.f32 = 1;
    a.N = N; a.H = H; a.W = W; a.Cin = Cin; a.ld_in = ld_in;
    a.Ho = (H + 2 * ph - kh) / sh + 1;
    a.Wo = (W + 2 * pw - kw) / sw + 1;
    a.Cout = Cout;
    a.Cout_pad = (Cout + 15) / 16 * 16;
    a.ld_out = ld_out; a.ld_res = ld_res;
    a.kh = kh; a.kw = kw; a.stride_h = sh; a.stride_w = sw; a.pad_h = ph; a.pad_w = pw; a.dil_h = 1; a.dil_w = 1;
    a.groups = 1;
    a.bk = 16;
    a.CinK = conv_igemm_f32_pick_cink(Cin);
    a.K = kh * kw * a.CinK;
    a.Kpad = (a.K + 15) / 16 * 16;
    a.M = N * a.Ho * a.Wo;
    a.act1 = act1; a.act2 = act2; a.alpha1 = 0.1f; a.alpha2 = 0.1f;
    a.scalar_out = (Cout % 4 || ld_out % 4 || (has_res && ld_res % 4)) ? 1 : 0;
    return a;
}

extern "C" int32_t trtx_conv_packed_dims_f32(int cout, int cin_pad, int kh, int kw, int32_t* cout_pad, int32_t* kpad, int32_t* cink) {
    if (cout < 1 || cin_pad < 1 || kh < 1 || kw < 1) return TRTX_ERR_INVALID;
    const int ck = conv_igemm_f32_pick_cink(cin_pad);
    if (cout_pad) *cout_pad = (cout + 15) / 16 * 16;
    if (kpad) *kpad = (kh * kw * ck + 15) / 16 * 16;
    if (cink) *cink = ck;
    return TRTX_OK;
}

extern "C" int32_t trtx_conv_pack_weights_f32(const float* w_kcrs, int cout, int cin, int kh, int kw, int cin_pad, const float* ch_scale, float* packed) {
    if (!w_kcrs || !packed || cin_pad < cin) return TRTX_ERR_INVALID;
    const int ck = conv_igemm_f32_pick_cink(cin_pad);
    conv_pack_weights_igemm_f32(w_kcrs, cout, cin, kh, kw, ck, (kh * kw * ck + 15) / 16 * 16, (cout + 15) / 16 * 16, ch_scale, packed);
    return TRTX_OK;
}

extern "C" int32_t trtx_op_conv2d_tactics_f32(int N, int H, int W, int Cin, int ld_in, int Cout, int ld_out, int kh, int kw, int sh, int sw, int ph,
                                              int pw, int has_residual, int ld_res, int32_t* out2, int32_t max_out) {
    if (!out2 || max_out < 1 || N < 1 || kh < 1 || kw < 1 || sh < 1 || sw < 1) return 0;
    ConvArgs a = op_conv_args_f32(N, H, W, Cin, ld_in, Cout, ld_out, kh, kw, sh, sw, ph, pw, 0, has_residual, ld_res, 0);
    a.residual = has_residual ? reinterpret_cast<const void*>(1) : nullptr;
    std::vector<ConvTactic> t(max_out);
    const int n = conv_tactics_f32(a, t.data(), max_out);
    for (int i = 0; i < n; ++i) {
        out2[4 * i + 0] = t[i].bn;
        out2[4 * i + 1] = t[i].bm;
        out2[4 * i + 2] = t[i].ws;
        out2[4 * i + 3] = t[i].bk;
    }
    return n;
}

extern "C" int32_t trtx_op_conv2d_nhwc_f32(const void* in, int N, int H, int W, int Cin, int ld_in, const void* wpacked, const float* bias, void* out,
                                           int Cout, int ld_out, int kh, int kw, int sh, int sw, int ph, int pw, int act1, const void* residual,
                                           int ld_res, int act2, const int32_t* tile2, trtx_stream_t stream) {
    ConvArgs a = op_conv_args_f32(N, H, W, Cin, ld_in, Cout, ld_out, kh, kw, sh, sw, ph, pw, act1, residual != nullptr, ld_res, act2);
    a.in = in;
    a.wgt = wpacked;
    a.bias = bias;
    a.out = out;
    a.residual = residual;
    if ((reinterpret_cast<uintptr_t>(out) & 15) || (residual && (reinterpret_cast<uintptr_t>(residual) & 15))) a.scalar_out = 1;
    if (tile2) {
        a.bn = tile2[0];
        a.bm = tile2[1];
        a.t_ws = tile2[2];
        a.bk = tile2[3];
    }
    const int reps = options().op_reps;
    int32_t st = TRTX_OK;
    for (int r = 0; r < reps && st == TRTX_OK; ++r) st = conv_igemm_f32(a, stream);
    return st;
}

extern "C" int32_t trtx_conv_pack_weights_i8(const float* w_kcrs, int cout, int cin, int kh, int kw, const float* ch_scale, int8_t* packed,
                                             float* wscale_out, int32_t* cout_pad_out, int32_t* kpad_out) {
    if (!w_kcrs || cout < 1 || cin < 1) return TRTX_ERR_INVALID;
    const int bn = conv_igemm_pick_bn(cout);
    const int cout_pad = (cout + bn - 1) / bn * bn, cink = (cin + 63) / 64 * 64, kpad = kh * kw * cink;
    if (cout_pad_out) *cout_pad_out = cout_pad;
    if (kpad_out) *kpad_out = kpad;
    if (packed && wscale_out) conv_pack_weights_i8(w_kcrs, cout, cin, kh, kw, cink, ch_scale, cout_pad, kpad, packed, wscale_out);
    return TRTX_OK;
}

extern "C" int32_t trtx_op_conv2d_nhwc_i8(const void* in, int N, int H, int W, int Cin, int ld_in, const void* wpacked, const float* cscale,
                                          const float* bias, void* out, int out_is_i8, float out_inv_scale, int Cout, int ld_out, int kh,
                                          int kw, int sh, int sw, int ph, int pw, int act1, const void* residual, int res_is_i8,
                                          float res_scale, int ld_res, int act2, trtx_stream_t stream) {
    if (Cin % 16 || ld_in % 16) return TRTX_ERR_INVALID;
    ConvArgs a{};
    a.in = in; a.wgt = wpacked; a.bias = bias; a.out = out; a.residual = residual;
    a.N = N; a.H = H; a.W = W;
    a.Ho = (H + 2 * ph - kh) / sh + 1;
    a.Wo = (W + 2 * pw - kw) / sw + 1;
    a.Cout = Cout;
    a.bn = conv_igemm_pick_bn(Cout);
    a.Cout_pad = (Cout + a.bn - 1) / a.bn * a.bn;
    a.ld_out = ld_out; a.ld_res = ld_res;
    a.kh = kh; a.kw = kw; a.stride_h = sh; a.stride_w = sw; a.pad_h = ph; a.pad_w = pw; a.dil_h = 1; a.dil_w = 1; a.groups = 1;
    a.bk = 32;
    const int cink = (Cin + 63) / 64 * 64;
    a.in_i8 = 1; a.out_i8 = out_is_i8; a.res_i8 = res_is_i8;
    a.cscale = cscale; a.out_inv_scale = out_inv_scale; a.res_scale = res_scale;
    a.Cin = Cin / 2; a.ld_in = ld_in / 2; a.CinK = cink / 2;
    a.K = kh * kw * a.CinK;
    a.Kpad = a.K;
    a.M = N * a.Ho * a.Wo;
    a.act1 = act1; a.act2 = act2; a.alpha1 = 0.1f; a.alpha2 = 0.1f;
    a.scalar_out = 0;
    if (Cout % 8 || ld_out % 8 || (residual && ld_res % 8)) return TRTX_ERR_UNSUPPORTED;
    return conv_igemm_f16(a, stream);
}

extern "C" int32_t trtx_op_nchw_f32_to_nhwc_f16(const float* in, void* out, int N, int C, int H, int W, int Cpad,
                                                int ld_out, trtx_stream_t stream) {
    return nchw_f32_to_nhwc(in, out, DT_F16, N, C, H, W, Cpad, ld_out, stream);
}

extern "C" int32_t trtx_op_nhwc_f16_to_nchw_f32(const void* in, float* out, int N, int C, int H, int W, int ld_in,
                                                trtx_stream_t stream) {
    return nhwc_to_nchw_f32(in, DT_F16, out, N, C, H, W, ld_in, stream);
}

extern "C" int32_t trtx_op_poison_lds(void* device_word, trtx_stream_t stream) {
    if (!device_word) return TRTX_ERR_INVALID;
    return poison_lds(static_cast<unsigned*>(device_word), static_cast<hipStream_t>(stream));
}
```

### tensorrtx_amd/csrc/options.cpp

```cpp
#include "options.h"

#include <stdlib.h>

namespace trtx {
namespace {
const char* env(const char* name) { return getenv(name); }
int env_int(const char* name, int unset) {
    const char* v = env(name);
    return (v && *v) ? atoi(v) : unset;
}
bool env_is(const char* name, int value) {
    const char* v = env(name);
    return v && *v && atoi(v) == value;
}
bool env_set(const char* name) { return env(name) != nullptr; }
}

Options read_options() {
    Options o;
    o.tune = env_int("TRTX_TUNE", -1);
    o.tune_verbose = env_set("TRTX_TUNE_VERBOSE");
    o.tune_margin = env_int("TRTX_TUNE_MARGIN", -1);
    if (const char* v = env("TRTX_TACTIC_CACHE")) o.tactic_cache = v;
    o.graph = env_is("TRTX_GRAPH", 1);
    if (const char* v = env("TRTX_CALIB_REPORT")) o.calib_report = v;
    if (const char* v = env("TRTX_INT8_CLIP_LIMIT"); v && *v) o.int8_clip_limit = atof(v);
    o.lanes = env_int("TRTX_LANES", 0);
    o.group_convs = !env_is("TRTX_GROUP_CONVS", 0);
    o.fold_upsample = !env_is("TRTX_FOLD_UPSAMPLE", 0);
    o.ws = !env_set("TRTX_CONV_NOWS");
    o.wsk = !env_set("TRTX_CONV_NOWSK");
    o.gemm256 = !env_is("TRTX_GEMM256", 0);
    o.patch = !env_is("TRTX_CONV_PATCH", 0);
    o.res = env_int("TRTX_CONV_RES", 7);
    o.roles = !env_is("TRTX_CONV_ROLES", 0);
    o.f32_mfma = !env_set("TRTX_F32_DIRECT");
    o.conv_grouped = !env_is("TRTX_CONV_GROUPED", 0);
    o.area_attention = !env_is("TRTX_AREA_ATTENTION", 0);
    o.yolo5_head = !env_is("TRTX_YOLO5_HEAD", 0);
    o.roialign_fused = !env_set("TRTX_ROIALIGN_PLUGIN");
    o.roialign_fold_stride = !env_is("TRTX_ROIALIGN_FOLD_STRIDE", 0);
    o.profile_kernel_events = !env_set("TRTX_PROFILE_NO_KERNEL_EVENTS");
    o.op_reps = env_int("TRTX_OP_REPS", 1);
    return o;
}

const Options& options() {
    static const Options o = read_options();
    return o;
}

}
```

### tensorrtx_amd/csrc/options.h

```cpp
#pragma once
#include <string>

namespace trtx {

struct Options {
    int tune = -1;
    bool tune_verbose = false;
    int tune_margin = -1;
    std::string tactic_cache;
    bool graph = false;
    std::string calib_report;
    double int8_clip_limit = 1e-4;
    int lanes = 0;
    bool group_convs = true;
    bool fold_upsample = true;
    bool ws = true;
    bool wsk = true;
    bool gemm256 = true;
    bool patch = true;
    int res = 7;
    bool roles = true;
    bool f32_mfma = true;
    bool conv_grouped = true;
    bool area_attention = true;
    bool yolo5_head = true;
    bool roialign_fused = true;
    bool roialign_fold_stride = true;
    bool profile_kernel_events = true;
    int op_reps = 1;
};

Options read_options();
const Options& options();

}
```

### tensorrtx_amd/csrc/runtime/engine.cpp

```cpp
#include "engine.h"

#include <stdlib.h>
#include <string.h>

#include <sstream>

#include "../common.h"
#include "../options.h"
#include "int8.h"
#include "plugin.h"

using namespace trtx;

trtx_engine::~trtx_engine() {
    int left = plugins_initialized;
    for (auto& op : plan.ops)
        if (op.kind == OP_PLUGIN && left-- > 0 && op.plugin->v.terminate) op.plugin->v.terminate(op.plugin->v.self);
    if (d_weights) (void)hipFree(d_weights);
}

trtx_context::~trtx_context() {
    for (hipStream_t st : lane_stream)
        if (st) {
            (void)hipStreamSynchronize(st);
            (void)hipStreamDestroy(st);
        }
    for (hipEvent_t ev : op_event)
        if (ev) (void)hipEventDestroy(ev);
    for (hipEvent_t ev : lane_done)
        if (ev) (void)hipEventDestroy(ev);
    if (start_event) (void)hipEventDestroy(start_event);
    for (auto& g : graphs) {
        if (g.exec) (void)hipGraphExecDestroy(g.exec);
        if (g.graph) (void)hipGraphDestroy(g.graph);
    }
    if (d_arena) (void)hipFree(d_arena);
}

namespace trtx {

namespace {

struct Resolver {
    const Plan& plan;
    char* arena;
    char* weights;
    void* const* bindings;
    char* base(const PTensor& t) const {
        const Storage& s = plan.storages[t.storage];
        switch (s.kind) {
            case ST_ARENA: return arena + s.offset;
            case ST_WEIGHTS: return weights + s.offset;
            default: return static_cast<char*>(bindings[s.binding]);
        }
    }
    void* ptr(int tid) const {
        const PTensor& t = plan.tensors[tid];
        const size_t es = dtype_size(t.dtype);
        return base(t) + (t.layout == LAY_NHWC ? (size_t)t.rcoff : (size_t)t.reoff) * es;
    }
};

StridedView batch_view(const StridedView& v, int batch, long bs_in, long bs_in2) {
    StridedView o{};
    o.rank = v.rank + 1;
    o.shape[0] = batch;
    o.stride_in[0] = bs_in;
    o.stride_in2[0] = bs_in2;
    for (int d = 0; d < v.rank; ++d) {
        o.shape[d + 1] = v.shape[d];
        o.stride_in[d + 1] = v.stride_in[d];
        o.stride_in2[d + 1] = v.stride_in2[d];
    }
    return o;
}

}

int32_t execute_plan(trtx_context* c, int batch, void* const* bindings, hipStream_t stream,
                     std::vector<OpTiming>* prof) {
    trtx_engine* e = c->engine;
    const Plan& plan = e->plan;
    if (batch < 1 || batch > plan.max_batch) {
        fprintf(stderr, "[trtx_hip] enqueue: batch %d outside [1, %d]\n", batch, plan.max_batch);
        return TRTX_ERR_INVALID;
    }
    for (size_t b = 0; b < plan.binding_tensor.size(); ++b)
        if (!bindings[b] && !(c->frames && plan.binding_is_input[b])) {
            fprintf(stderr, "[trtx_hip] enqueue: binding %zu is null\n", b);
            return TRTX_ERR_INVALID;
        }
    Resolver R{plan, static_cast<char*>(c->d_arena), static_cast<char*>(e->d_weights), bindings};
    char* W = static_cast<char*>(e->d_weights);
    std::vector<hipEvent_t> evs;
    std::vector<LaunchProbe> probes;
    const bool no_probe = !options().profile_kernel_events;
    if (prof) {
        evs.resize(plan.ops.size() + 1);
        for (auto& ev : evs) TRTX_HIP_TRY(hipEventCreate(&ev));
        probes.resize(plan.ops.size());
        if (!no_probe && !c->tuning)
            for (size_t k = 0; k < plan.ops.size(); ++k)
                if ((plan.ops[k].kind == OP_CONV && plan.ops[k].igemm) || plan.ops[k].kind == OP_CONV_GROUP)
                    if (hipEventCreate(&probes[k].start) != hipSuccess || hipEventCreate(&probes[k].stop) != hipSuccess) (void)hipGetLastError();
        TRTX_HIP_TRY(hipEventRecord(evs[0], stream));
    }
    auto free_probes = [&]() {
        conv_set_launch_probe(nullptr);
        for (auto& pr : probes) {
            if (pr.start) (void)hipEventDestroy(pr.start);
            if (pr.stop) (void)hipEventDestroy(pr.stop);
        }
        probes.clear();
    };
    hipStream_t const user_stream = stream;
    const bool lanes = !prof && !c->observer && plan.num_lanes > 1;
    std::vector<char> lane_started(plan.num_lanes, 0);
    auto bail = [&](int32_t st) {
        (void)hipGetLastError();
        if (lanes)
            for (int l = 1; l < plan.num_lanes; ++l)
                if (lane_started[l] && hipEventRecord(c->lane_done[l], c->lane_stream[l]) == hipSuccess)
                    (void)hipStreamWaitEvent(user_stream, c->lane_done[l], 0);
        for (auto& ev : evs) (void)hipEventDestroy(ev);
        evs.clear();
        free_probes();
        return st;
    };
    if (lanes && hipEventRecord(c->start_event, user_stream) != hipSuccess) return bail(TRTX_ERR_HIP);
    for (size_t k = 0; k < plan.ops.size(); ++k) {
        const POp& op = plan.ops[k];
        hipStream_t stream = user_stream;
        if (lanes) {
            if (op.lane > 0) {
                stream = c->lane_stream[op.lane];
                if (!lane_started[op.lane]) {
                    if (hipStreamWaitEvent(stream, c->start_event, 0) != hipSuccess) return bail(TRTX_ERR_HIP);
                    lane_started[op.lane] = 1;
                }
            }
            for (int d : op.wait_ops)
                if (hipStreamWaitEvent(stream, c->op_event[d], 0) != hipSuccess) return bail(TRTX_ERR_HIP);
        }
        const PTensor& t0 = plan.tensors[op.in.empty() ? op.out[0] : op.in[0]];
        const PTensor& to = plan.tensors[op.out[0]];
        auto nb = [&](const PTensor& t) { return (t.nfix ? t.nfix : batch) * t.nmul; };
        int32_t st = TRTX_OK;
        const bool skip = c->tuning && (op.kind == OP_PLUGIN || op.kind == OP_YOLO_HEAD || op.kind == OP_YOLO_TASK_HEAD || op.kind == OP_YOLO5_HEAD || op.kind == OP_ROI_ALIGN);
        if (!skip) switch (op.kind) {
            case OP_CONV:
            case OP_DECONV: {
                ConvArgs a = op.conv;
                a.in = R.ptr(op.in[0]);
                a.out = R.ptr(op.out[0]);
                a.residual = op.in.size() > 1 ? R.ptr(op.in[1]) : nullptr;
                a.up_in = op.extra_in.empty() ? nullptr : R.ptr(op.extra_in[0]);
                a.wgt = W + op.w_off;
                a.bias = reinterpret_cast<const float*>(W + op.b_off);
                a.cscale = a.in_i8 ? reinterpret_cast<const float*>(W + op.s_off) : nullptr;
                a.N = op.stem ? (plan.explicit_batch ? (int)t0.dims.d[0] : batch) : nb(t0);
                a.M = a.N * a.Ho * a.Wo;
                if (op.kind == OP_DECONV)
                    st = deconv_direct(a, op.dtype, stream);
                else if (op.stem && c->frames)
                    st = a.f32 ? TRTX_ERR_UNSUPPORTED : conv_stem_frames_f32(a, c->frames, stream);
                else if (op.stem)
                    st = a.f32 ? conv_stem_nchw_f32_out_f32(a, stream) : conv_stem_nchw_f32(a, stream);
                else if (op.igemm) {
                    if (prof && probes[k].start && probes[k].stop) conv_set_launch_probe(&probes[k]);
                    st = a.f32 ? conv_igemm_f32(a, stream) : conv_igemm_f16(a, stream);
                    conv_set_launch_probe(nullptr);
                } else if (op.dw)
                    st = conv_dw(a, op.dtype, stream);
                else if (op.grouped)
                    st = conv_grouped(a, stream);
                else
                    st = conv_direct(a, op.dtype, stream);
                break;
            }
            case OP_CONV_GROUP: {
                ConvArgs ga[kMaxConvGroup];
                const int gn = (int)op.group.size();
                if (gn < 2 || gn > kMaxConvGroup) { st = TRTX_ERR_STATE; break; }
                for (int m = 0; m < gn; ++m) {
                    const POp& mo = op.group[m];
                    ConvArgs& a = ga[m];
                    a = mo.conv;
                    a.in = R.ptr(mo.in[0]);
                    a.out = R.ptr(mo.out[0]);
                    a.residual = mo.in.size() > 1 ? R.ptr(mo.in[1]) : nullptr;
                    a.up_in = nullptr;
                    a.wgt = W + mo.w_off;
                    a.bias = reinterpret_cast<const float*>(W + mo.b_off);
                    a.cscale = a.in_i8 ? reinterpret_cast<const float*>(W + mo.s_off) : nullptr;
                    a.N = nb(plan.tensors[mo.in[0]]);
                    a.M = a.N * a.Ho * a.Wo;
                }
                if (prof && probes[k].start && probes[k].stop) conv_set_launch_probe(&probes[k]);
                st = conv_igemm_group_f16(ga, gn, stream);
                conv_set_launch_probe(nullptr);
                if (st == TRTX_ERR_UNSUPPORTED) {
                    st = TRTX_OK;
                    for (int m = 0; m < gn && st == TRTX_OK; ++m) st = conv_igemm_f16(ga[m], stream);
                }
                break;
            }
            case OP_POOL:
                st = nhwc_pool(R.ptr(op.in[0]), R.ptr(op.out[0]), op.dtype, op.i[0], nb(t0), t0.H, t0.W, t0.C, t0.ld, to.H,
                               to.W, to.ld, op.i[1], op.i[2], op.i[3], op.i[4], op.i[5], op.i[6], op.i[7], stream);
                break;
            case OP_POOL_CHAIN: {
                const PTensor &y1 = plan.tensors[op.out[0]], &y2 = plan.tensors[op.out[1]], &y3 = plan.tensors[op.out[2]];
                st = nhwc_maxpool_chain3_f16(R.ptr(op.in[0]), R.ptr(op.out[0]), R.ptr(op.out[1]), R.ptr(op.out[2]), nb(t0), t0.H,
                                             t0.W, t0.C, t0.ld, y1.ld, y2.ld, y3.ld, op.i[1], stream, op.dtype == DT_F32 ? 1 : 0);
                break;
            }
            case OP_D2S:
                st = nhwc_depth_to_space_f16(R.ptr(op.in[0]), R.ptr(op.out[0]), nb(t0), t0.H, t0.W, to.C, op.i[0], op.i[1], t0.ld,
                                             to.ld, stream);
                break;
            case OP_RESIZE:
                if (t0.dtype == DT_I8) {
                    st = nhwc_resize_nearest_i8(R.ptr(op.in[0]), R.ptr(op.out[0]), nb(t0), t0.H, t0.W, t0.C, t0.ld, to.H, to.W, to.ld,
                                                t0.scale / to.scale, stream);
                    break;
                }
                st = nhwc_resize_nearest(R.ptr(op.in[0]), R.ptr(op.out[0]), op.dtype, nb(t0), t0.H, t0.W, t0.C, t0.ld, to.H,
                                         to.W, to.ld, stream);
                break;
            case OP_EW_NHWC: {
                const PTensor& t1 = plan.tensors[op.in[1]];
                st = nhwc_elementwise(R.ptr(op.in[0]), R.ptr(op.in[1]), R.ptr(op.out[0]), op.dtype, op.i[0],
                                      (long)nb(t0) * t0.H * t0.W, t0.C, t0.ld, t1.ld, to.ld, stream);
                break;
            }
            case OP_ACT_NHWC:
                st = nhwc_activation(R.ptr(op.in[0]), R.ptr(op.out[0]), op.dtype, op.i[0], op.f[0],
                                     (long)nb(t0) * t0.H * t0.W, t0.C, t0.ld, to.ld, stream);
                break;
            case OP_SCALE_NHWC:
                st = nhwc_scale(R.ptr(op.in[0]), R.ptr(op.out[0]), op.dtype, reinterpret_cast<const float*>(W + op.s_off),
                                reinterpret_cast<const float*>(W + op.b_off), (long)nb(t0) * t0.H * t0.W, t0.C, t0.ld,
                                to.ld, stream);
                break;
            case OP_COPY_NHWC:
                st = nhwc_copy(R.ptr(op.in[0]), R.ptr(op.out[0]), op.dtype, (long)nb(t0) * t0.H * t0.W, t0.C, t0.ld, to.ld,
                               stream);
                break;
            case OP_REDUCE_HW:
                st = nhwc_reduce_hw_avg(R.ptr(op.in[0]), R.ptr(op.out[0]), op.dtype, nb(t0), t0.H * t0.W, t0.C, t0.ld, to.ld,
                                        stream);
                break;
            case OP_TO_NHWC:
                st = nchw_f32_to_nhwc(static_cast<const float*>(R.ptr(op.in[0])), R.ptr(op.out[0]), to.dtype, nb(to), to.C,
                                      to.H, to.W, to.Calloc ? to.Calloc : to.C, to.ld, stream);
                break;
            case OP_TO_LINEAR:
                st = nhwc_to_nchw_f32(R.ptr(op.in[0]), t0.dtype, static_cast<float*>(R.ptr(op.out[0])), nb(t0), t0.C, t0.H,
                                      t0.W, t0.ld, stream);
                break;
            case OP_GATHER: {
                const float* src = static_cast<const float*>(R.ptr(op.in[0])) + op.off0;
                const StridedView v = to.batched ? batch_view(op.view, batch, t0.batched ? t0.dims.volume() : 0, 0) : op.view;
                st = lin_gather(src, static_cast<float*>(R.ptr(op.out[0])), v, stream);
                break;
            }
            case OP_SCATTER: {
                float* dst = static_cast<float*>(R.ptr(op.out[0])) + op.off0;
                StridedView v = op.view;
                if (to.batched) {
                    if (!t0.batched) {
                        for (int b = 0; b < batch && st == TRTX_OK; ++b)
                            st = lin_scatter(static_cast<const float*>(R.ptr(op.in[0])), dst + (long)b * to.dims.volume(), v,
                                             stream);
                        break;
                    }
                    v = batch_view(op.view, batch, to.dims.volume(), 0);
                }
                st = lin_scatter(static_cast<const float*>(R.ptr(op.in[0])), dst, v, stream);
                break;
            }
            case OP_EW_LIN: {
                const PTensor& t1 = plan.tensors[op.in[1]];
                const StridedView v = to.batched ? batch_view(op.view, batch, t0.batched ? t0.dims.volume() : 0,
                                                              t1.batched ? t1.dims.volume() : 0)
                                                 : op.view;
                st = lin_elementwise(static_cast<const float*>(R.ptr(op.in[0])), static_cast<const float*>(R.ptr(op.in[1])),
                                     static_cast<float*>(R.ptr(op.out[0])), op.i[0], v, stream);
                break;
            }
            case OP_ACT_LIN:
                st = lin_activation(static_cast<const float*>(R.ptr(op.in[0])), static_cast<float*>(R.ptr(op.out[0])), op.i[0],
                                    op.f[0], (long)(to.batched ? batch : 1) * to.dims.volume(), stream);
                break;
            case OP_SCALE_LIN: {
                const long bmul = to.batched ? batch : 1;
                st = lin_scale(static_cast<const float*>(R.ptr(op.in[0])), static_cast<float*>(R.ptr(op.out[0])),
                               reinterpret_cast<const float*>(W + op.s_off), reinterpret_cast<const float*>(W + op.b_off),
                               reinterpret_cast<const float*>(W + op.w_off), op.i[0], bmul * op.i[1], op.i[2], op.i[3],
                               stream);
                break;
            }
            case OP_SOFTMAX:
                st = lin_softmax(static_cast<const float*>(R.ptr(op.in[0])), static_cast<float*>(R.ptr(op.out[0])),
                                 (long)(to.batched ? batch : 1) * op.i[0], op.i[1], op.i[2], stream);
                break;
            case OP_MATMUL: {
                const PTensor& t1 = plan.tensors[op.in[1]];
                if (op.view.rank > 0) {
                    const StridedView& v = op.view;
                    const long outer = v.rank == 2 ? v.shape[0] : 1, inner = v.shape[v.rank - 1];
                    st = lin_matmul(static_cast<const float*>(R.ptr(op.in[0])), static_cast<const float*>(R.ptr(op.in[1])),
                                    static_cast<float*>(R.ptr(op.out[0])), (int)(outer * inner), op.i[0], op.i[1], op.i[2], op.i[3], op.i[4],
                                    v.rank == 2 ? v.stride_in[0] : 0, v.rank == 2 ? v.stride_in2[0] : 0, stream, (int)inner,
                                    v.stride_in[v.rank - 1], v.stride_in2[v.rank - 1]);
                    break;
                }
                st = lin_matmul(static_cast<const float*>(R.ptr(op.in[0])), static_cast<const float*>(R.ptr(op.in[1])),
                                static_cast<float*>(R.ptr(op.out[0])), to.batched ? batch : 1, op.i[0], op.i[1], op.i[2],
                                op.i[3], op.i[4], t0.batched ? t0.dims.volume() : 0, t1.batched ? t1.dims.volume() : 0,
                                stream);
                break;
            }
            case OP_REDUCE_LIN:
                st = lin_reduce(static_cast<const float*>(R.ptr(op.in[0])), static_cast<float*>(R.ptr(op.out[0])), op.i[0],
                                (long)(to.batched ? batch : 1) * op.i[1], op.i[2], op.i[3], stream);
                break;
            case OP_PLUGIN: {
                std::vector<const void*> ins;
                std::vector<void*> outs;
                for (int t : op.in) ins.push_back(R.ptr(t));
                for (int t : op.out) outs.push_back(R.ptr(t));
                void* ws = op.ws_bytes ? static_cast<char*>(c->d_arena) + op.ws_off : nullptr;
                const int pb = plan.explicit_batch && op.i[0] > 0 ? op.i[0] : batch;
                const int rc = op.plugin->v.enqueue(op.plugin->v.self, pb, ins.data(), outs.data(), ws, stream);
                if (rc != 0) {
                    fprintf(stderr, "[trtx_hip] plugin %s enqueue returned %d\n", op.name.c_str(), rc);
                    st = TRTX_ERR_HIP;
                }
                break;
            }
            case OP_YOLO_HEAD: {
                const int nl = op.i[4];
                const void* heads[8];
                int lds[8];
                for (int k = 0; k < nl; ++k) {
                    heads[k] = R.ptr(op.in[k]);
                    lds[k] = plan.tensors[op.in[k]].ld;
                }
                st = (t0.dtype == DT_F32 ? trtx_yolo_head_decode_nhwc_f32 : trtx_yolo_head_decode_nhwc)(
                        heads, lds, nl, op.i[11] > 0 ? op.i[11] : batch, op.i[0], op.i[1], op.i[2], &op.i[5], reinterpret_cast<const float*>(W + op.w_off), op.i[3],
                        static_cast<float*>(R.ptr(op.out[0])), static_cast<char*>(c->d_arena) + op.ws_off, op.ws_bytes, stream);
                break;
            }
            case OP_YOLO_TASK_HEAD: {
                const int nl = op.i[4];
                const void* heads[4];
                const void* branches[4];
                int lds[4], blds[4];
                for (int k = 0; k < nl; ++k) {
                    heads[k] = R.ptr(op.in[k]);
                    lds[k] = plan.tensors[op.in[k]].ld;
                    branches[k] = R.ptr(op.extra_in[k]);
                    blds[k] = plan.tensors[op.extra_in[k]].ld;
                }
                st = (t0.dtype == DT_F32 ? trtx_yolo_task_head_decode_nhwc_f32 : trtx_yolo_task_head_decode_nhwc)(
                        heads, lds, branches, blds, nl, op.i[11] > 0 ? op.i[11] : batch, op.i[0], op.i[1], op.i[2], &op.i[5],
                        reinterpret_cast<const float*>(W + op.w_off), op.i[3], op.i[9] == 1, op.i[9] == 2, op.i[9] == 3, op.i[10], op.f[0],
                        static_cast<float*>(R.ptr(op.out[0])), static_cast<char*>(c->d_arena) + op.ws_off, op.ws_bytes, stream);
                break;
            }
            case OP_YOLO5_HEAD: {
                const int nl = op.i[4];
                const void* heads[8];
                int lds[8], gw[8], gh[8];
                if (nl < 1 || nl > 8 || (int)op.iv.size() != 2 * nl || (int)op.fv.size() != 6 * nl) { st = TRTX_ERR_STATE; break; }
                for (int k = 0; k < nl; ++k) {
                    heads[k] = R.ptr(op.in[k]);
                    lds[k] = plan.tensors[op.in[k]].ld;
                    gw[k] = op.iv[2 * k];
                    gh[k] = op.iv[2 * k + 1];
                }
                st = (t0.dtype == DT_F32 ? trtx_yolov5_head_decode_nhwc_f32 : trtx_yolov5_head_decode_nhwc)(
                        heads, lds, nl, op.i[11] > 0 ? op.i[11] : batch, op.i[0], op.i[1], op.i[2], gw, gh, op.fv.data(), op.i[3],
                        static_cast<float*>(R.ptr(op.out[0])), static_cast<char*>(c->d_arena) + op.ws_off, op.ws_bytes, stream);
                break;
            }
            case OP_ATTENTION: {
                const PTensor &to2 = plan.tensors[op.out[1]];
                if (op.i[4] > 0)
                    st = area_attention_f16(R.ptr(op.in[0]), t0.ld, R.ptr(op.out[0]), to.ld, R.ptr(op.out[1]), to2.ld, nb(t0), op.i[0], op.i[1], op.i[4],
                                            op.i[2], op.i[3], op.f[0], stream);
                else
                    st = psa_attention_f16(R.ptr(op.in[0]), t0.ld, R.ptr(op.out[0]), to.ld, R.ptr(op.out[1]), to2.ld, nb(t0), op.i[0], op.i[1], op.i[2],
                                           op.i[3], op.f[0], stream);
                break;
            }
            case OP_ROI_ALIGN: {
                const PTensor& ft = plan.tensors[op.in[1]];
                st = trtx_roi_align_nhwc_f16_strided(batch, static_cast<const float*>(R.ptr(op.in[0])), R.ptr(op.in[1]), ft.ld, op.i[0], op.f[0], op.i[1],
                                                     op.i[2], ft.C, ft.H, ft.W, R.ptr(op.out[0]), to.ld, op.i[3] > 0 ? op.i[3] : 1, stream);
                break;
            }
            case OP_COPY_LIN: {
                const size_t bytes = (size_t)(to.batched ? batch : 1) * to.dims.volume() * 4;
                if (hipMemcpyAsync(R.ptr(op.out[0]), R.ptr(op.in[0]), bytes, hipMemcpyDeviceToDevice, stream) != hipSuccess)
                    st = TRTX_ERR_HIP;
                break;
            }
            default:
                st = TRTX_ERR_UNSUPPORTED;
        }
        if (st != TRTX_OK) {
            fprintf(stderr, "[trtx_hip] op %zu (%s, %s) failed: %s\n", k, op_kind_name(op.kind), op.name.c_str(),
                    trtx_status_string(st));
            return bail(st);
        }
        if (c->observer) {
            for (int t : op.out) {
                const PTensor& pt = plan.tensors[t];
                if (pt.layout != LAY_NHWC || pt.dtype != DT_F16 || pt.C % 8 || pt.ld % 8) continue;
                const long pixels = (long)nb(pt) * pt.H * pt.W;
                CalibObserver& ob = *c->observer;
                if (ob.mode == 1)
                    st = nhwc_absmax_f16(R.ptr(t), pixels, pt.C, pt.ld, ob.d_max + pt.storage, stream);
                else if (ob.mode == 2 && ob.range[pt.storage] > 0.f)
                    st = nhwc_hist_f16(R.ptr(t), pixels, pt.C, pt.ld, ob.range[pt.storage], ob.d_hist + (size_t)pt.storage * kCalibBins, stream);
                if (st != TRTX_OK) return bail(st);
            }
        }
        if (prof && hipEventRecord(evs[k + 1], stream) != hipSuccess) return bail(TRTX_ERR_HIP);
        if (lanes && op.signal && hipEventRecord(c->op_event[k], stream) != hipSuccess) return bail(TRTX_ERR_HIP);
    }
    if (lanes)
        for (int l = 1; l < plan.num_lanes; ++l)
            if (lane_started[l]) {
                if (hipEventRecord(c->lane_done[l], c->lane_stream[l]) != hipSuccess || hipStreamWaitEvent(user_stream, c->lane_done[l], 0) != hipSuccess)
                    return bail(TRTX_ERR_HIP);
            }
    if (prof) {
        if (hipStreamSynchronize(stream) != hipSuccess) return bail(TRTX_ERR_HIP);
        for (size_t k = 0; k < plan.ops.size(); ++k) {
            float ms = 0;
            (void)hipEventElapsedTime(&ms, evs[k], evs[k + 1]);
            OpTiming t{plan.ops[k].name, op_kind_name(plan.ops[k].kind), ms};
            if (probes[k].launches == 1 && probes[k].start && probes[k].stop) {
                float kms = -1.f;
                if (hipEventElapsedTime(&kms, probes[k].start, probes[k].stop) == hipSuccess && kms > 0.f) t.kernel_ms = kms;
                else (void)hipGetLastError();
            }
            prof->push_back(t);
        }
        for (auto& ev : evs) (void)hipEventDestroy(ev);
        free_probes();
    }
    return TRTX_OK;
}

}

struct trtx_hostmem {
    std::vector<uint8_t> data;
};

// ... 317 lines not shown
```

### tensorrtx_amd/csrc/runtime/plan.cpp

```cpp
#include "plan.h"

#include <sstream>

namespace trtx {

const char* op_kind_name(int k) {
    static const char* n[] = {"conv",     "deconv",    "pool",      "resize",     "ew_nhwc", "act_nhwc", "scale_nhwc",
                              "copy_nhwc", "reduce_hw", "to_nhwc",   "to_linear",  "gather",  "scatter",  "ew_lin",
                              "act_lin",  "scale_lin", "softmax",   "matmul",     "reduce_lin", "plugin", "copy_lin", "yolo_head",
                              "pool_chain", "depth_to_space", "roi_align", "conv_chain", "conv_group", "attention",
                              "yolo_task_head", "yolo5_head"};
    return (k >= 0 && k <= OP_YOLO5_HEAD) ? n[k] : "?";
}

std::string Plan::describe_json() const {
    std::ostringstream o;
    double flops = 0, bytes = 0;
    int n_conv = 0, n_igemm = 0;
    for (const auto& op : ops) {
        flops += op.flops;
        bytes += op.bytes;
        if (op.kind == OP_CONV) {
            ++n_conv;
            n_igemm += op.igemm ? 1 : 0;
        }
        n_conv += (int)op.group.size();
        n_igemm += (int)op.group.size();
    }
    o << "{\"fp16\":" << (fp16 ? "true" : "false") << ",\"max_batch\":" << max_batch << ",\"arena_bytes\":" << arena_bytes
      << ",\"weight_bytes\":" << weight_bytes << ",\"n_lanes\":" << num_lanes << ",\"n_ops\":" << ops.size() << ",\"n_conv\":" << n_conv
      << ",\"n_igemm\":" << n_igemm << ",\"flops_per_sample\":" << flops << ",\"bytes_per_sample\":" << bytes
      << ",\"ops\":[";
    for (size_t k = 0; k < ops.size(); ++k) {
        const POp& op = ops[k];
        o << (k ? "," : "") << "{\"kind\":\"" << op_kind_name(op.kind) << "\",\"name\":\"";
        for (char c : op.name) o << ((c == '"' || c == '\\' || (unsigned char)c < 0x20) ? ' ' : c);
        o << "\",\"flops\":" << op.flops << ",\"bytes\":" << op.bytes;
        auto conv_fields = [&](const POp& op) {
            const ConvArgs& a = op.conv;
            o << ",\"igemm\":" << (op.igemm ? "true" : "false") << ",\"stem\":" << (op.stem ? "true" : "false") << ",\"cin\":" << (a.in_i8 ? 2 * a.Cin : a.Cin) << ",\"cout\":" << a.Cout
              << ",\"k\":[" << a.kh << "," << a.kw << "],\"stride\":[" << a.stride_h << "," << a.stride_w << "],\"hw_in\":["
              << a.H << "," << a.W << "],\"hw_out\":[" << a.Ho << "," << a.Wo << "],\"act1\":" << a.act1
              << ",\"act2\":" << a.act2 << ",\"alpha1\":" << a.alpha1 << ",\"alpha2\":" << a.alpha2 << ",\"up_c\":" << a.up_C << ",\"residual\":" << (op.in.size() > 1 ? "true" : "false")
              << ",\"bn_folded\":" << (op.scale_layer >= 0 ? "true" : "false") << ",\"ld_in\":" << a.ld_in
              << ",\"ld_out\":" << a.ld_out << ",\"i8\":[" << a.in_i8 << "," << a.out_i8 << "," << a.res_i8 << "],\"nmul\":" << (op.stem ? 1 : tensors[op.in[0]].nmul) << ",\"nfix\":"
              << (op.stem ? 0 : tensors[op.in[0]].nfix);
            if (op.dw) o << ",\"dw\":true";
            if (op.grouped) o << ",\"grouped\":true";
            if (op.cout_real) o << ",\"cout_real\":" << op.cout_real;
        };
        if (op.kind == OP_CONV || op.kind == OP_DECONV) conv_fields(op);
        if (op.kind == OP_ATTENTION) o << ",\"heads\":" << op.i[0] << ",\"n\":" << op.i[1] << ",\"kd\":" << op.i[2] << ",\"hd\":" << op.i[3];
        if (op.kind == OP_ATTENTION && op.i[4] > 0) o << ",\"area\":" << op.i[4] << ",\"kernel\":\"mfma\"";
        if (op.kind == OP_YOLO_TASK_HEAD) {
            o << ",\"task\":\"" << (op.i[9] == 1 ? "seg" : (op.i[9] == 2 ? "pose" : "obb")) << "\",\"classes\":" << op.i[0] << ",\"nk\":" << op.i[10]
              << ",\"branch_ld\":[";
            for (size_t j = 0; j < op.extra_in.size(); ++j) o << (j ? "," : "") << tensors[op.extra_in[j]].ld;
            o << "]";
        }
        if (op.kind == OP_YOLO5_HEAD) {
            o << ",\"classes\":" << op.i[0] << ",\"levels\":" << op.i[4] << ",\"anchor_levels\":" << op.fv.size() / 6 << ",\"grids\":[";
            for (int j = 0; j < op.i[4]; ++j) o << (j ? "," : "") << "[" << op.iv[2 * j] << "," << op.iv[2 * j + 1] << "]";
            o << "],\"ld\":[";
            for (size_t j = 0; j < op.in.size(); ++j) o << (j ? "," : "") << tensors[op.in[j]].ld;
            o << "]";
        }
        if (op.kind == OP_CONV_GROUP) {
            o << ",\"members\":[";
            for (size_t j = 0; j < op.group.size(); ++j) {
                const POp& m = op.group[j];
                o << (j ? "," : "") << "{\"name\":\"";
                for (char c : m.name) o << ((c == '"' || c == '\\' || (unsigned char)c < 0x20) ? ' ' : c);
                o << "\",\"flops\":" << m.flops << ",\"bytes\":" << m.bytes;
                conv_fields(m);
                o << ",\"in\":[";
                for (size_t q = 0; q < m.in.size(); ++q) o << (q ? "," : "") << m.in[q];
                o << "],\"out\":[" << m.out[0] << "]}";
            }
            o << "]";
        }
        o << ",\"lane\":" << op.lane << ",\"waits\":[";
        for (size_t j = 0; j < op.wait_ops.size(); ++j) o << (j ? "," : "") << op.wait_ops[j];
        o << "],\"in\":[";
        for (size_t j = 0; j < op.in.size(); ++j) o << (j ? "," : "") << op.in[j];
        o << "],\"out\":[";
        for (size_t j = 0; j < op.out.size(); ++j) o << (j ? "," : "") << op.out[j];
        o << "]}";
    }
    o << "],\"tensors\":[";
    for (size_t k = 0; k < tensors.size(); ++k) {
        const PTensor& t = tensors[k];
        o << (k ? "," : "") << "{\"id\":" << t.id << ",\"net\":" << t.net_tensor << ",\"layout\":\""
          << (t.layout == LAY_NHWC ? "nhwc" : "linear") << "\",\"dims\":[";
        for (int d = 0; d < t.dims.nb; ++d) o << (d ? "," : "") << t.dims.d[d];
        o << "],\"storage\":" << t.storage << ",\"coff\":" << t.rcoff << ",\"ld\":" << t.ld << ",\"dtype\":" << t.dtype << ",\"scale\":" << t.scale
          << ",\"view\":"
          << (t.parent >= 0 ? "true" : "false") << "}";
    }
    o << "],\"storages\":[";
    for (size_t k = 0; k < storages.size(); ++k) {
        const Storage& s = storages[k];
        o << (k ? "," : "") << "{\"kind\":" << s.kind << ",\"bytes\":" << s.bytes << ",\"offset\":" << s.offset
          << ",\"first\":" << s.first_use << ",\"last\":" << s.last_use << "}";
    }
    o << "]}";
    return o.str();
}

}
```

### tensorrtx_amd/csrc/runtime/plan.h

```cpp
#pragma once
#include <memory>
#include <string>
#include <vector>

#include "../kernels/kernels.h"
#include "graph.h"
#include "plugin.h"

namespace trtx {

enum Layout : int { LAY_LINEAR = 0, LAY_NHWC = 1 };
enum StorageKind : int { ST_ARENA = 0, ST_WEIGHTS = 1, ST_BINDING = 2 };

enum OpKind : int {
    OP_CONV = 0,
    OP_DECONV,
    OP_POOL,
    OP_RESIZE,
    OP_EW_NHWC,
    OP_ACT_NHWC,
    OP_SCALE_NHWC,
    OP_COPY_NHWC,
    OP_REDUCE_HW,
    OP_TO_NHWC,
    OP_TO_LINEAR,
    OP_GATHER,
    OP_SCATTER,
    OP_EW_LIN,
    OP_ACT_LIN,
    OP_SCALE_LIN,
    OP_SOFTMAX,
    OP_MATMUL,
    OP_REDUCE_LIN,
    OP_PLUGIN,
    OP_COPY_LIN,
    OP_YOLO_HEAD,
    OP_POOL_CHAIN,
    OP_D2S,
    OP_ROI_ALIGN,
    OP_RESERVED_47,
    OP_CONV_GROUP,
    OP_ATTENTION,
    OP_YOLO_TASK_HEAD,
    OP_YOLO5_HEAD,
};
const char* op_kind_name(int k);

struct PTensor {
    int id = -1;
    int net_tensor = -1;
    std::string name;
    Dims dims;
    bool batched = true;
    int layout = LAY_LINEAR;
    int dtype = DT_F32;
    int nfix = 0;
    int nmul = 1;
    int C = 0, H = 0, W = 0;
    bool pad_zeroed = false;
    int parent = -1;
    int coff = 0;
    long eoff = 0;
    int ld = 0;
    int storage = -1;
    int rcoff = 0;
    long reoff = 0;
    int Calloc = 0;
    float scale = 0.f;
    long sample_elems() const { return layout == LAY_NHWC ? (long)nmul * H * W * ld : (long)dims.volume(); }
};

struct Storage {
    int kind = ST_ARENA;
    size_t bytes = 0;
    size_t offset = 0;
    int binding = -1;
    int first_use = 1 << 30, last_use = -1;
};
inline size_t align256(size_t v) { return (v + 255) / 256 * 256; }

struct POp {
    int kind = 0;
    std::string name;
    std::vector<int> in, out;
    std::vector<int> extra_in;
    int dtype = DT_F32;
    ConvArgs conv{};
    bool igemm = false;
    bool stem = false;
    bool from_deconv = false;
    bool dw = false;
    bool grouped = false;
    int cout_real = 0;
    std::vector<POp> group;
    int src_layer = -1;
    int scale_layer = -1;
    size_t w_off = 0, b_off = 0, s_off = 0;
    int i[12] = {0};
    float f[4] = {0};
    std::vector<int> iv;
    std::vector<float> fv;
    StridedView view{};
    long off0 = 0;
    bool view_batched_in = false, view_batched_in2 = false, view_batched_out = true;
    std::shared_ptr<PluginHolder> plugin;
    size_t ws_off = 0, ws_bytes = 0;
    int lane = 0;
    std::vector<int> wait_ops;
    bool signal = false;
    double flops = 0;
    double bytes = 0;
};

struct Plan {
    bool explicit_batch = false;
    bool fp16 = false;
    int max_batch = 1;
    std::vector<PTensor> tensors;
    std::vector<Storage> storages;
    std::vector<POp> ops;
    std::vector<int> binding_tensor;
    std::vector<int> binding_ptensor;
    std::vector<bool> binding_is_input;
    int num_lanes = 1;
    size_t arena_bytes = 0;
    size_t weight_bytes = 0;
    std::vector<uint8_t> weight_blob;
    std::string error;

    std::string describe_json() const;
};

bool lower_network(const Network& net, Plan* plan);
struct CalibrationLowering {
    CalibrationLowering();
    ~CalibrationLowering();
    static bool active();
};
bool pack_weights(const Network& net, Plan* plan);

}
```

### tensorrtx_amd/csrc/runtime/plan_passes.cpp

```cpp
#include "plan_passes.h"

#include <algorithm>

namespace trtx {
namespace {

bool fail(std::string* err, const std::string& m) {
    *err = m;
    return false;
}

size_t tensor_bytes(const Plan& plan, const PTensor& t) {
    const size_t es = dtype_size(t.dtype);
    if (t.layout == LAY_NHWC) {
        const size_t n = (t.nfix ? (size_t)t.nfix : (size_t)plan.max_batch) * (size_t)t.nmul;
        return n * t.H * t.W * (size_t)t.Calloc * es;
    }
    return (t.batched ? (size_t)plan.max_batch : 1) * (size_t)t.dims.volume() * es;
}

bool choose_conv_kernel(const Plan& plan, const PassInputs& e, POp& op) {
    ConvArgs& a = op.conv;
    const PTensor& ti = plan.tensors[op.in[0]];
    const PTensor& to = plan.tensors[op.out[0]];
// ... 258 lines not shown
    }
}

void assign_storages(Plan& plan) {
    for (auto& t : plan.tensors) {
        if (t.parent >= 0 || t.storage >= 0) continue;
        Storage s;
        s.kind = ST_ARENA;
        s.bytes = tensor_bytes(plan, t);
        t.storage = (int)plan.storages.size();
        plan.storages.push_back(s);
    }
    for (auto& t : plan.tensors) t.storage = plan.tensors[owner_of(plan, t.id)].storage;
    for (size_t b = 0; b < plan.binding_ptensor.size(); ++b) {
        const PTensor& t = plan.tensors[plan.binding_ptensor[b]];
        plan.storages[t.storage].bytes = tensor_bytes(plan, t);
    }
}

bool select_conv_kernels(Plan& plan, const PassInputs& e, std::string* err) {
    for (auto& op : plan.ops) {
        if (op.kind != OP_CONV && op.kind != OP_DECONV) continue;
        ConvArgs& a = op.conv;
        const PTensor& ti = plan.tensors[op.in[0]];
        const PTensor& to = plan.tensors[op.out[0]];
        if (op.stem && (e.dt == DT_F16 ? (to.ld % 8 || to.rcoff % 8) : (to.ld % 4 || to.rcoff % 4))) return fail(err, op.name + ": stem convolution output is not 16-byte aligned");
        choose_conv_kernel(plan, e, op);
        if (!op.extra_in.empty() && !op.igemm) return fail(err, op.name + ": folded upsample on a convolution that cannot take the MFMA path");
        if ((ti.dtype == DT_I8 || to.dtype == DT_I8 || (op.in.size() > 1 && plan.tensors[op.in[1]].dtype == DT_I8)) && !op.igemm)
            return fail(err, op.name + ": int8 tensor on a convolution that cannot take the MFMA path");
        const double es_in = (double)dtype_size(ti.dtype), es_out = (double)dtype_size(to.dtype);
        const double cin_real = ti.dtype == DT_I8 ? 2.0 * a.Cin : (double)a.Cin;
        const double in_elems = (double)a.H * a.W * (cin_real - a.up_C) + (double)a.up_H * a.up_W * a.up_C;
        op.bytes = to.nmul * ((op.stem ? 4.0 : es_in) * in_elems + es_out * (double)a.Ho * a.Wo * a.Cout * (op.in.size() > 1 ? 2 : 1));
    }
    return true;
}

bool configure_plugins(Plan& plan, std::string* err) {
    for (size_t k = 0; k < plan.ops.size(); ++k) {
        POp& op = plan.ops[k];
        if (op.kind != OP_PLUGIN) continue;
        const bool eb = plan.explicit_batch && op.i[0] > 0;
        auto strip = [&](Dims d) {
            if (eb && d.nb > 0) {
                for (int q = 1; q < d.nb; ++q) d.d[q - 1] = d.d[q];
                --d.nb;
            }
            return to_c(d);
        };
        const int mb = eb ? op.i[0] : plan.max_batch;
        std::vector<trtx_dims> din, dout;
        for (int t : op.in) din.push_back(strip(plan.tensors[t].dims));
        for (int t : op.out) dout.push_back(strip(plan.tensors[t].dims));
        if (op.plugin->v.configure &&
            op.plugin->v.configure(op.plugin->v.self, din.data(), (int)din.size(), dout.data(), (int)dout.size(), mb) != 0)
            return fail(err, op.name + ": plugin configurePlugin rejected the tensor shapes");
        op.ws_bytes = op.plugin->v.workspace_size ? op.plugin->v.workspace_size(op.plugin->v.self, mb) : 0;
        for (int t : op.in) op.bytes += 4.0 * plan.tensors[t].dims.volume();
        for (int t : op.out) op.bytes += 4.0 * plan.tensors[t].dims.volume();
    }
    return true;
}

void chain_sppf_pools(Plan& plan, const PassInputs& e) {
    for (size_t k = 0; k + 2 < plan.ops.size(); ++k) {
        auto same_max = [&](const POp& o) {
            return o.kind == OP_POOL && o.i[0] == POOL_MAX && o.i[1] == o.i[2] && (o.i[1] & 1) && o.i[3] == 1 && o.i[4] == 1 &&
                   o.i[5] == o.i[1] / 2 && o.i[6] == o.i[1] / 2;
        };
        POp &a = plan.ops[k], &b = plan.ops[k + 1], &c3 = plan.ops[k + 2];
        if (!same_max(a) || !same_max(b) || !same_max(c3) || a.i[1] != b.i[1] || a.i[1] != c3.i[1]) continue;
        if (b.in[0] != a.out[0] || c3.in[0] != b.out[0] || (e.dt != DT_F16 && e.dt != DT_F32)) continue;
        const PTensor& tx = plan.tensors[a.in[0]];
        const int cv = e.dt == DT_F16 ? 8 : 4;
        bool ok = tx.C % cv == 0 && tx.ld % cv == 0 && tx.rcoff % cv == 0 && (long)(tx.H + a.i[1] - 1) * (tx.W + a.i[1] - 1) * 32 <= 64 * 1024 && tx.nmul == 1;
        for (const POp* o : {&a, &b, &c3}) {
            const PTensor& ty = plan.tensors[o->out[0]];
            ok = ok && ty.ld % cv == 0 && ty.rcoff % cv == 0 && ty.H == tx.H && ty.W == tx.W && ty.C == tx.C;
        }
        if (!ok) continue;
        a.kind = OP_POOL_CHAIN;
        a.name += " [x3 chained]";
        a.out = {a.out[0], b.out[0], c3.out[0]};
        plan.ops.erase(plan.ops.begin() + k + 1, plan.ops.begin() + k + 3);
    }
}

std::vector<std::vector<int>> op_dependencies(const Plan& plan) {
    const int nops = (int)plan.ops.size();
    struct Range { int storage; long lo, hi; int op; bool write; };
    auto access_of = [&](int t, int op, bool write) {
        const PTensor& pt = plan.tensors[t];
        Range a{pt.storage, 0, 0, op, write};
        if (pt.layout == LAY_NHWC) {
            a.lo = pt.rcoff;
            a.hi = pt.rcoff + (pt.parent < 0 && pt.Calloc > pt.C ? pt.Calloc : pt.C);
        } else {
            a.lo = pt.reoff;
            a.hi = pt.reoff + pt.dims.volume();
        }
        return a;
    };
    std::vector<std::vector<int>> deps(nops);
    std::vector<Range> log;
    for (int k = 0; k < nops; ++k) {
        const POp& op = plan.ops[k];
        std::vector<Range> mine;
        for (int t : op.in) mine.push_back(access_of(t, k, false));
        for (int t : op.extra_in) mine.push_back(access_of(t, k, false));
        for (int t : op.out) mine.push_back(access_of(t, k, true));
        for (const Range& m : mine)
            for (const Range& o : log)
                if (o.storage == m.storage && o.lo < m.hi && m.lo < o.hi && (o.write || m.write) && o.op != k) deps[k].push_back(o.op);
        std::sort(deps[k].begin(), deps[k].end());
        deps[k].erase(std::unique(deps[k].begin(), deps[k].end()), deps[k].end());
        log.insert(log.end(), mine.begin(), mine.end());
    }
    return deps;
}

struct Ancestors {
    int words;
    std::vector<uint64_t> bits;
    bool has(int a, int of) const { return (bits[(size_t)of * words + (a >> 6)] >> (a & 63)) & 1ull; }
};
Ancestors ancestors(const Plan& plan, const std::vector<std::vector<int>>& deps, bool lane_order) {
    const int n = (int)deps.size();
    Ancestors anc{(n + 63) / 64, {}};
    anc.bits.assign((size_t)n * anc.words, 0);
    std::vector<int> prev_on_lane(plan.num_lanes, -1);
    for (int k = 0; k < n; ++k) {
        uint64_t* row = &anc.bits[(size_t)k * anc.words];
        auto absorb = [&](int d) {
            for (int w = 0; w < anc.words; ++w) row[w] |= anc.bits[(size_t)d * anc.words + w];
            row[d >> 6] |= 1ull << (d & 63);
        };
        for (int d : deps[k]) absorb(d);
        if (!lane_order) continue;
        const int lane = plan.ops[k].lane;
        if (prev_on_lane[lane] >= 0) absorb(prev_on_lane[lane]);
        prev_on_lane[lane] = k;
    }
    return anc;
}

void group_convs(Plan& plan, const PassInputs& e) {
    if (e.dt != DT_F16 || CalibrationLowering::active()) return;
    const bool mark_only = !e.opt.group_convs;
    const int n = (int)plan.ops.size();
    if (n < 2 || n > 4096) return;
    const std::vector<std::vector<int>> deps = op_dependencies(plan);
    const Ancestors anc = ancestors(plan, deps, false);
    auto args_at_max_batch = [&](const POp& op) {
        ConvArgs a = op.conv;
        const PTensor& ti = plan.tensors[op.in[0]];
        a.N = (ti.nfix ? ti.nfix : plan.max_batch) * ti.nmul;
        a.M = a.N * a.Ho * a.Wo;
        a.residual = op.in.size() > 1 ? reinterpret_cast<const void*>(1) : nullptr;
        return a;
    };
    auto candidate = [&](const POp& op) {
        if (op.kind != OP_CONV || !op.igemm || op.stem || op.from_deconv || !op.extra_in.empty()) return false;
        ConvArgs two[2] = {args_at_max_batch(op), args_at_max_batch(op)};
        return conv_igemm_group_supported(two, 2);
    };
    auto same_layer_shape = [&](const POp& x, const POp& y) {
        const ConvArgs &a = x.conv, &b = y.conv;
        return a.kh == b.kh && a.kw == b.kw && a.stride_h == b.stride_h && a.stride_w == b.stride_w && a.pad_h == b.pad_h && a.pad_w == b.pad_w &&
               a.Cout == b.Cout && a.act1 == b.act1 && a.act2 == b.act2 && a.alpha1 == b.alpha1 && a.alpha2 == b.alpha2 && x.in.size() == y.in.size() &&
               a.in_i8 == b.in_i8 && a.out_i8 == b.out_i8 && a.res_i8 == b.res_i8;
    };
    std::vector<int> height(n, 0);
    for (int k = n - 1; k >= 0; --k)
        for (int d : deps[k]) height[d] = std::max(height[d], height[k] + 1);
    std::vector<int> group_of(n, -1);
    std::vector<std::vector<int>> groups;
    struct Contracted { std::vector<int> first_op, indeg; std::vector<std::vector<int>> succ; };
    auto contract = [&]() {
        Contracted c;
        std::vector<int> node(n), gnode(groups.size(), -1);
        for (int k = 0; k < n; ++k) {
            if (group_of[k] >= 0 && gnode[group_of[k]] >= 0) {
                node[k] = gnode[group_of[k]];
                continue;
            }
            if (group_of[k] >= 0) gnode[group_of[k]] = (int)c.first_op.size();
            node[k] = (int)c.first_op.size();
            c.first_op.push_back(k);
        }
        c.succ.resize(c.first_op.size());
        c.indeg.assign(c.first_op.size(), 0);
        for (int k = 0; k < n; ++k)
            for (int d : deps[k])
                if (node[d] != node[k]) {
                    c.succ[node[d]].push_back(node[k]);
                    ++c.indeg[node[k]];
                }
        return c;
    };
    auto acyclic = [&]() {
        Contracted c = contract();
        const int nn = (int)c.first_op.size();
        std::vector<int>& indeg = c.indeg;
        const std::vector<std::vector<int>>& succ = c.succ;
        std::vector<int> q;
        for (int v = 0; v < nn; ++v)
            if (!indeg[v]) q.push_back(v);
        size_t done = 0;
        while (done < q.size()) {
            const int v = q[done++];
            for (int w : succ[v])
                if (--indeg[w] == 0) q.push_back(w);
        }
        return (int)q.size() == nn;
    };
    for (int k = 0; k < n; ++k) {
        if (group_of[k] >= 0 || !candidate(plan.ops[k])) continue;
        std::vector<int> mem = {k};
        std::vector<ConvArgs> margs = {args_at_max_batch(plan.ops[k])};
        for (int j = k + 1; j < n && (int)mem.size() < kMaxConvGroup; ++j) {
            if (group_of[j] >= 0 || height[j] != height[k] || !candidate(plan.ops[j]) || !same_layer_shape(plan.ops[k], plan.ops[j])) continue;
            bool indep = true;
            for (int m : mem) indep = indep && !anc.has(m, j) && !anc.has(j, m);
            if (!indep) continue;
            margs.push_back(args_at_max_batch(plan.ops[j]));
            std::vector<ConvArgs> trial = margs;
            int big = 0;
            for (size_t q = 1; q < trial.size(); ++q)
                if (trial[q].M > trial[big].M) big = (int)q;
            const int rs = trial[big].t_rs;
            for (ConvArgs& ma : trial) ma.t_rs = rs;
            if (!conv_igemm_group_supported(trial.data(), (int)trial.size())) {
                margs.pop_back();
                continue;
            }
            mem.push_back(j);
        }
        if (mem.size() < 2) continue;
        const int gi = (int)groups.size();
        groups.push_back(mem);
        for (int m : mem) group_of[m] = gi;
        if (!acyclic()) {
            for (int m : mem) group_of[m] = -1;
            groups.pop_back();
        }
    }
    if (groups.empty()) return;
    if (mark_only) {
        for (const auto& mem : groups)
            for (int m : mem) {
                plan.ops[m].conv.t_wsk = WSK_OFF;
                plan.ops[m].conv.k_pinned = 1;
            }
        return;
    }
    Contracted c = contract();
    const int nn = (int)c.first_op.size();
    std::vector<int>&indeg = c.indeg, &first_op = c.first_op;
    const std::vector<std::vector<int>>& succ = c.succ;
    std::vector<char> emitted(nn, 0);
    std::vector<POp> out;
    out.reserve(nn);
    for (int step = 0; step < nn; ++step) {
        int pick = -1;
        for (int v = 0; v < nn; ++v)
            if (!emitted[v] && indeg[v] == 0) { pick = v; break; }
        if (pick < 0) return;
        emitted[pick] = 1;
        for (int w : succ[pick]) --indeg[w];
        const int k0 = first_op[pick];
        if (group_of[k0] < 0) {
            out.push_back(plan.ops[k0]);
            continue;
        }
        POp g;
        g.kind = OP_CONV_GROUP;
        g.dtype = plan.ops[k0].dtype;
        g.conv = plan.ops[k0].conv;
        int big = groups[group_of[k0]][0];
        for (int m : groups[group_of[k0]])
            if ((long)plan.ops[m].conv.Ho * plan.ops[m].conv.Wo * plan.tensors[plan.ops[m].in[0]].nmul >
                (long)plan.ops[big].conv.Ho * plan.ops[big].conv.Wo * plan.tensors[plan.ops[big].in[0]].nmul)
                big = m;
        for (int m : groups[group_of[k0]]) {
            POp mo = plan.ops[m];
            mo.conv.t_rs = plan.ops[big].conv.t_rs;
            mo.conv.t_wsk = WSK_OFF;
            mo.conv.k_pinned = 1;
            g.group.push_back(mo);
            g.name += (g.name.empty() ? "" : " + ") + mo.name;
            for (int t : mo.in)
                if (std::find(g.in.begin(), g.in.end(), t) == g.in.end()) g.in.push_back(t);
            g.out.push_back(mo.out[0]);
            g.flops += mo.flops;
            g.bytes += mo.bytes;
        }
        g.name = "[group of " + std::to_string(g.group.size()) + "] " + g.name;
        out.push_back(std::move(g));
    }
    plan.ops = std::move(out);
}

void assign_lanes(Plan& plan, const PassInputs& e, const std::vector<std::vector<int>>& deps) {
    const int nops = (int)plan.ops.size();
    int max_lanes = e.max_aux_streams >= 0 ? 1 + e.max_aux_streams : 4;
    if (e.opt.lanes > 0) max_lanes = std::max(1, std::min(16, e.opt.lanes));
    std::vector<int> tail(max_lanes, -1);
    plan.num_lanes = 1;
    for (int k = 0; k < nops; ++k) {
        int lane = -1;
        for (int d : deps[k])
            if (tail[plan.ops[d].lane] == d && (lane < 0 || d > tail[lane])) lane = plan.ops[d].lane;
        if (lane < 0 && deps[k].empty()) lane = 0;
        if (lane < 0) {
            for (int l = 0; l < max_lanes && lane < 0; ++l)
                if (tail[l] < 0) lane = l;
        }
        if (lane < 0) {
            lane = 0;
            for (int l = 1; l < max_lanes; ++l)
                if (tail[l] < tail[lane]) lane = l;
        }
        plan.ops[k].lane = lane;
        tail[lane] = k;
        plan.num_lanes = std::max(plan.num_lanes, lane + 1);
    }
    std::vector<std::vector<int>> covered(max_lanes, std::vector<int>(max_lanes, -1));
    for (int k = 0; k < nops; ++k) {
        POp& op = plan.ops[k];
        for (int d : deps[k]) {
            const int ld = plan.ops[d].lane;
            if (ld == op.lane || covered[op.lane][ld] >= d) continue;
            op.wait_ops.push_back(d);
            plan.ops[d].signal = true;
            covered[op.lane][ld] = d;
        }
    }
}

void plan_arena(Plan& plan, const Ancestors& anc) {
    const int nops = (int)plan.ops.size();
    auto before = [&](int a, int b) { return a == b || anc.has(a, b); };
    std::vector<std::vector<int>> touch(plan.storages.size());
    for (int k = 0; k < nops; ++k) {
        const POp& op = plan.ops[k];
        auto mark = [&](int t) {
            const int st = plan.tensors[t].storage;
            Storage& s = plan.storages[st];
            s.first_use = std::min(s.first_use, k);
            s.last_use = std::max(s.last_use, k);
            if (touch[st].empty() || touch[st].back() != k) touch[st].push_back(k);
        };
        for (int t : op.in) mark(t);
        for (int t : op.extra_in) mark(t);
        for (int t : op.out) mark(t);
    }
    std::vector<std::pair<int, int>> ws_storage;
    for (int k = 0; k < nops; ++k) {
        const int kind = plan.ops[k].kind;
        if ((kind != OP_PLUGIN && kind != OP_YOLO_HEAD && kind != OP_YOLO_TASK_HEAD && kind != OP_YOLO5_HEAD) || plan.ops[k].ws_bytes == 0) continue;
        Storage s;
        s.kind = ST_ARENA;
        s.bytes = plan.ops[k].ws_bytes;
        s.first_use = s.last_use = k;
        ws_storage.push_back({k, (int)plan.storages.size()});
        plan.storages.push_back(s);
        touch.push_back({k});
    }
    auto ordered = [&](int sa, int sb) {
        for (int x : touch[sa])
            for (int y : touch[sb])
                if (!before(x, y) || x == y) return false;
        return true;
    };
    std::vector<int> order;
    for (size_t si = 0; si < plan.storages.size(); ++si)
        if (plan.storages[si].kind == ST_ARENA && plan.storages[si].last_use >= 0) order.push_back((int)si);
    std::stable_sort(order.begin(), order.end(),
                     [&](int x, int y) { return plan.storages[x].first_use < plan.storages[y].first_use; });
    std::vector<int> placed;
    size_t arena = 0;
    for (int si : order) {
        Storage& st = plan.storages[si];
        const size_t need = align256(st.bytes);
        std::vector<std::pair<size_t, size_t>> busy;
        for (int pj : placed) {
            const Storage& o = plan.storages[pj];
            if (ordered(pj, si) || ordered(si, pj)) continue;
            busy.push_back({o.offset, o.offset + align256(o.bytes)});
        }
        std::sort(busy.begin(), busy.end());
        size_t off = 0;
        for (auto& bz : busy) {
            if (off + need <= bz.first) break;
            off = std::max(off, bz.second);
        }
        st.offset = off;
        arena = std::max(arena, off + need);
        placed.push_back(si);
    }
    plan.arena_bytes = arena;
    for (auto& w : ws_storage) plan.ops[w.first].ws_off = plan.storages[w.second].offset;
}

}

bool finalize_plan(Plan& plan, const PassInputs& e, std::string* err) {
    resolve_view_geometry(plan);
    fold_upsample(plan, e);
    assign_int8_served(plan, e);
    assign_storages(plan);
    if (!select_conv_kernels(plan, e, err) || !configure_plugins(plan, err)) return false;
    chain_sppf_pools(plan, e);
    group_convs(plan, e);
    const std::vector<std::vector<int>> deps = op_dependencies(plan);
    assign_lanes(plan, e, deps);
    plan_arena(plan, ancestors(plan, deps, true));
    return true;
}

}
```

Baseline: 39340.

## Fuse stem conv with following stride-2 conv into one pair kernel

Adds a fused kernel that computes the 3x3/s2 stem conv (Cin≤4→16) into LDS and immediately runs the next 3x3/s2 16→32 conv from that LDS tile. The fetch of the next tile's input patch overlaps the second conv. A plan pass marks eligible stem+conv pairs whose intermediate tensor is private, and the engine dispatches them as one launch. This removes the write and re-read of the largest intermediate activation (320x320x16 fp16 per image) and one launch. The cost is recomputing stem pixels in the halo overlap and a larger LDS footprint per workgroup.

Result: faster. 40130, median of 6 (+2.0%).

```diff
diff --git a/include/trtx_hip.h b/include/trtx_hip.h
--- a/include/trtx_hip.h
+++ b/include/trtx_hip.h
@@ -147,6 +147,10 @@
 int32_t trtx_op_conv2d_tactics(int N, int H, int W, int Cin, int ld_in, int Cout, int ld_out, int kh, int kw, int sh, int sw, int ph, int pw,
                                int has_residual, int ld_res, int32_t* out6, int32_t max_out);
 int32_t trtx_op_conv_force_tactic(const int32_t* tactic6);
+int32_t trtx_op_conv_stem_nchw_f16(const float* in, int N, int C, int H, int W, const float* w_taps_cout, const float* bias, void* out, int Cout,
+                                   int ld_out, int k, int stride, int pad, int act, trtx_stream_t stream);
+int32_t trtx_op_conv_stem_pair_f16(const float* in, int N, int C, int H, int W, const float* stem_w_taps_cout, const float* stem_bias, int stem_act,
+                                   const void* conv_wpacked, const float* conv_bias, int conv_act, void* out, int ld_out, trtx_stream_t stream);
 int32_t trtx_conv_packed_dims_f32(int cout, int cin_pad, int kh, int kw, int32_t* cout_pad, int32_t* kpad, int32_t* cink);
 int32_t trtx_conv_pack_weights_f32(const float* w_kcrs, int cout, int cin, int kh, int kw, int cin_pad, const float* ch_scale, float* packed);
 int32_t trtx_op_conv2d_nhwc_f32(const void* in, int N, int H, int W, int Cin, int ld_in, const void* wpacked, const float* bias, void* out, int Cout,
diff --git a/tensorrtx_amd/capi.py b/tensorrtx_amd/capi.py
--- a/tensorrtx_amd/capi.py
+++ b/tensorrtx_amd/capi.py
@@ -310,6 +310,36 @@
     return out
 
 
+def stem_weights(w_kcrs):
+    import numpy as np
+    w = np.ascontiguousarray(w_kcrs, dtype=np.float32)
+    return np.ascontiguousarray(w.reshape(w.shape[0], -1).T)
+
+
+def conv_stem_nchw_f16(x, w_taps_cout, bias, k, stride, pad, act="none", out=None, out_ld=None):
+    import torch
+    N, C, H, W = x.shape
+    cout = w_taps_cout.shape[1]
+    Ho, Wo = (H + 2 * pad - k) // stride + 1, (W + 2 * pad - k) // stride + 1
+    if out is None:
+        out = torch.empty((N, Ho, Wo, cout), dtype=torch.float16, device=x.device)
+    check(lib().trtx_op_conv_stem_nchw_f16(_p(x), N, C, H, W, _p(w_taps_cout), _p(bias), _p(out), cout, out_ld or out.shape[-1], k, stride, pad,
+                                           ACT[act], _stream()), "trtx_op_conv_stem_nchw_f16")
+    return out
+
+
+def conv_stem_pair_f16(x, stem_w_taps_cout, stem_bias, conv_wpacked, conv_bias, stem_act="silu", conv_act="silu", out=None, out_ld=None):
+    import torch
+    N, C, H, W = x.shape
+    Hi, Wi = (H - 1) // 2 + 1, (W - 1) // 2 + 1
+    Ho, Wo = (Hi - 1) // 2 + 1, (Wi - 1) // 2 + 1
+    if out is None:
+        out = torch.empty((N, Ho, Wo, 32), dtype=torch.float16, device=x.device)
+    check(lib().trtx_op_conv_stem_pair_f16(_p(x), N, C, H, W, _p(stem_w_taps_cout), _p(stem_bias), ACT[stem_act], _p(conv_wpacked), _p(conv_bias),
+                                           ACT[conv_act], _p(out), out_ld or out.shape[-1], _stream()), "trtx_op_conv_stem_pair_f16")
+    return out
+
+
 def pack_conv_weights_grouped_f16(w_kcrs, ch_scale=None):
     import numpy as np
     L = lib()
diff --git a/tensorrtx_amd/csrc/kernels/conv_stem.hip b/tensorrtx_amd/csrc/kernels/conv_stem.hip
--- a/tensorrtx_amd/csrc/kernels/conv_stem.hip
+++ b/tensorrtx_amd/csrc/kernels/conv_stem.hip
@@ -7,6 +7,7 @@
 #include "../common.h"
 #include "act.h"
 #include "kernels.h"
+#include "stem_tile.h"
 
 namespace trtx {
 namespace {
@@ -61,15 +62,7 @@
     }
 }
 
-typedef __attribute__((address_space(3))) void* lds_ptr_t;
-
 constexpr int kStemTW = 64, kStemTH = 4;
-
-struct StemGeom {
-    int PR, PCA;
-    int tiles_x, tiles_y;
-    int chunks;
-};
 
 struct FramePack {
     StemFrame img[kStemMaxFrames];
@@ -117,14 +110,6 @@
     b = c0 / 255.0f;
 }
 
-template <int NFRAG, int KS>
-struct StemRegs {
-    half8 wf[NFRAG][KS];
-    int l_off[KS][8];
-    float bias4[NFRAG][4];
-};
-template <int NFRAG, int KS>
-__device__ __forceinline__ void stem_setup(const ConvArgs& p, const StemGeom& g, StemRegs<NFRAG, KS>& R);
 template <int NFRAG, int KS>
 __device__ __forceinline__ void stem_compute(const ConvArgs& p, const StemGeom& g, const StemRegs<NFRAG, KS>& R, const float* s_patch, int n, int tx0, int ty0, int shift);
 template <int NFRAG, int KS>
@@ -172,8 +157,6 @@
 template <int NFRAG, int KS>
 __global__ __launch_bounds__(256) void conv_stem_lds_kernel(const ConvArgs p, const StemGeom g, unsigned in_bytes, int total_tiles) {
     extern __shared__ __attribute__((aligned(16))) float s_patch[];
-    const int tid = threadIdx.x;
-    const int wave = tid >> 6;
     StemRegs<NFRAG, KS> R;
     stem_setup<NFRAG, KS>(p, g, R);
     for (int tile = blockIdx.x; tile < total_tiles; tile += gridDim.x) {
@@ -186,84 +169,13 @@
     const int wi_start = tx0 * p.stride_w - p.pad_w;
     const int al_start = (wi_start >= 0 ? wi_start : wi_start - 3) / 4 * 4;
     const int shift = wi_start - al_start;
-    {
-        const __amdgpu_buffer_rsrc_t rs = __builtin_amdgcn_make_buffer_rsrc(const_cast<void*>(p.in), 0, in_bytes, 0x00020000);
-        const int cpr = g.PCA / 4;
-        const float inv_cpr = 1.0f / (float)cpr, inv_pr = 1.0f / (float)g.PR;
-        for (int base = 0; base < g.chunks; base += 256) {
-            const int ci = base + tid;
-            int row = (int)((float)ci * inv_cpr);
-            int cq = ci - row * cpr;
-            if (cq < 0) { --row; cq += cpr; }
-            if (cq >= cpr) { ++row; cq -= cpr; }
-            int c = (int)((float)row * inv_pr);
-            int pr = row - c * g.PR;
-            if (pr < 0) { --c; pr += g.PR; }
-            if (pr >= g.PR) { ++c; pr -= g.PR; }
-            const int hi = hi_start + pr, wi = al_start + cq * 4;
-            const bool ok = ci < g.chunks && (unsigned)hi < (unsigned)p.H && wi >= 0 && wi + 3 < p.W;
-            const unsigned off = ok ? (unsigned)(((((long)n * p.Cin + c) * p.H + hi) * p.W + wi) * 4) : 0x80000000u;
-            __builtin_amdgcn_raw_ptr_buffer_load_lds(rs, (lds_ptr_t)(s_patch + (size_t)(base + wave * 64) * 4), 16, off, 0, 0, 0);
-        }
-    }
+    stem_patch_fetch(p, g, in_bytes, s_patch, n, hi_start, al_start);
     asm volatile("s_waitcnt vmcnt(0)" ::: "memory");
     __syncthreads();
-    if (p.W & 3) {
-        const int cpr = g.PCA / 4, rows = p.Cin * g.PR, wtail = p.W & ~3;
-        const int cq = (wtail - al_start) >> 2;
-        if (cq >= 0 && cq < cpr && wtail >= al_start) {
-            const float* __restrict__ src = static_cast<const float*>(p.in);
-            for (int rrow = tid; rrow < rows; rrow += 256) {
-                const int c = rrow / g.PR, pr = rrow - c * g.PR, hi = hi_start + pr;
-                if ((unsigned)hi >= (unsigned)p.H) continue;
-                const size_t base = (((size_t)n * p.Cin + c) * p.H + hi) * p.W;
-                for (int e = 0; e < 4; ++e)
-                    if (wtail + e < p.W) s_patch[((size_t)rrow * cpr + cq) * 4 + e] = src[base + wtail + e];
-            }
-        }
-        __syncthreads();
-    }
+    stem_patch_tail(p, g, s_patch, n, hi_start, al_start);
     stem_compute<NFRAG, KS>(p, g, R, s_patch, n, tx0, ty0, shift);
     __syncthreads();
     }
-}
-
-template <int NFRAG, int KS>
-__device__ __forceinline__ void stem_setup(const ConvArgs& p, const StemGeom& g, StemRegs<NFRAG, KS>& R) {
-    const int lane = threadIdx.x & 63;
-    const int khw = p.kh * p.kw;
-    const int K = khw * p.Cin;
-    const float* __restrict__ w = static_cast<const float*>(p.wgt);
-    const int kq = (lane >> 4) * 8;
-    auto& wf = R.wf;
-    auto& l_off = R.l_off;
-    auto& bias4 = R.bias4;
-    const float inv_khw = 1.0f / (float)khw, inv_kw = 1.0f / (float)p.kw;
-#pragma unroll
-    for (int ks = 0; ks < KS; ++ks)
-#pragma unroll
-        for (int e = 0; e < 8; ++e) {
-            const int k = ks * 32 + kq + e;
-            const int c = (int)(((float)k + 0.5f) * inv_khw), rem = k - c * khw;
-            const int r = (int)(((float)rem + 0.5f) * inv_kw), q = rem - r * p.kw;
-            l_off[ks][e] = k < K ? (c * g.PR + r) * g.PCA + q : 0;
-#pragma unroll
-            for (int j = 0; j < NFRAG; ++j) {
-                const int co = j * 16 + (lane & 15);
-                const float wv = w[(size_t)(k < K ? k : K - 1) * p.Cout + (co < p.Cout ? co : p.Cout - 1)];
-                wf[j][ks][e] = (k < K && co < p.Cout) ? (_Float16)wv : (_Float16)0.f;
-            }
-        }
-    const int ch4 = (lane >> 4) * 4;
-    const float* __restrict__ bsrc = p.bias ? p.bias : w;
-#pragma unroll
-    for (int j = 0; j < NFRAG; ++j)
-#pragma unroll
-        for (int e = 0; e < 4; ++e) {
-            const int co = j * 16 + ch4 + e;
-            const float bv = bsrc[co < p.Cout ? co : p.Cout - 1];
-            bias4[j][e] = (p.bias && co < p.Cout) ? bv : 0.f;
-        }
 }
 
 template <int NFRAG, int KS>
@@ -273,8 +185,6 @@
     const int lane = tid & 63;
     const int wave = tid >> 6;
     const int ch4 = (lane >> 4) * 4;
-    const auto& wf = R.wf;
-    const auto& l_off = R.l_off;
     const auto& bias4 = R.bias4;
     _Float16* __restrict__ out = static_cast<_Float16*>(p.out);
 #pragma nounroll
@@ -283,39 +193,14 @@
         const int ho = ty0 + ty, wo = tx0 + tx;
         const float* src = s_patch + (ty * p.stride_h) * g.PCA + tx * p.stride_w + shift;
         floatx4 acc[NFRAG];
-#pragma unroll
-        for (int j = 0; j < NFRAG; ++j) acc[j] = floatx4{0.f, 0.f, 0.f, 0.f};
-#pragma unroll
-        for (int ks = 0; ks < KS; ++ks) {
-            half8 xf;
-#pragma unroll
-            for (int e = 0; e < 8; ++e) xf[e] = (_Float16)src[l_off[ks][e]];
-#pragma unroll
-            for (int j = 0; j < NFRAG; ++j) acc[j] = __builtin_amdgcn_mfma_f32_16x16x32_f16(wf[j][ks], xf, acc[j], 0, 0, 0);
-        }
+        stem_group_mfma<NFRAG, KS>(R, src, acc);
         if (ho >= p.Ho || wo >= p.Wo) continue;
         const long m = ((long)n * p.Ho + ho) * p.Wo + wo;
 #pragma unroll
         for (int j = 0; j < NFRAG; ++j) {
             const int co = j * 16 + ch4;
             if (co >= p.Cout) continue;
-            half4 o;
-            if (p.act1 == ACT_SILU) {
-#pragma unroll
-                for (int e = 0; e < 4; ++e) {
-                    const float x = acc[j][e] + bias4[j][e];
-                    o[e] = round_to_half(x * __builtin_amdgcn_rcpf(1.0f + __expf(-x)));
-                }
-            } else if (p.act1 == ACT_RELU) {
-#pragma unroll
-                for (int e = 0; e < 4; ++e) {
-                    const float x = acc[j][e] + bias4[j][e];
-                    o[e] = (_Float16)(x > 0.f ? x : 0.f);
-                }
-            } else {
-#pragma unroll
-                for (int e = 0; e < 4; ++e) o[e] = round_to_half(act_stem(acc[j][e] + bias4[j][e], p.act1, p.alpha1));
-            }
+            const half4 o = stem_finish4(p, acc[j], bias4[j]);
             *reinterpret_cast<half4*>(out + m * p.ld_out + co) = o;
         }
     }
diff --git a/tensorrtx_amd/csrc/kernels/conv_stem_pair.hip b/tensorrtx_amd/csrc/kernels/conv_stem_pair.hip
--- /dev/null
+++ b/tensorrtx_amd/csrc/kernels/conv_stem_pair.hip
@@ -0,0 +1,168 @@
+#include <hip/hip_fp16.h>
+#include <hip/hip_runtime.h>
+#include <stdint.h>
+
+#include "../common.h"
+#include "act.h"
+#include "kernels.h"
+#include "launch.h"
+#include "stem_pair_index.h"
+#include "stem_tile.h"
+
+namespace trtx {
+namespace {
+
+namespace px = pairidx;
+
+constexpr int kPairPatchBytesMax = (4 * px::kPR * px::kPCA / 4 + 255) / 256 * 256 * 16;
+static_assert(kPairPatchBytesMax + px::kImageBytes <= 80 * 1024, "two workgroups per CU and room for other contexts");
+
+__device__ __forceinline__ size_t pair_patch_bytes(int cin) { return (size_t)((cin * px::kPR * px::kPCA / 4 + 255) / 256 * 256) * 16; }
+
+__global__ __launch_bounds__(256) void conv_stem_pair_kernel(const ConvArgs ps, const ConvArgs p1, const StemGeom g, unsigned in_bytes, int total_tiles) {
+    extern __shared__ __attribute__((aligned(16))) float s_patch[];
+    char* const s_img = reinterpret_cast<char*>(s_patch) + pair_patch_bytes(ps.Cin);
+    const int tid = threadIdx.x;
+    const int lane = tid & 63;
+    const int wave = __builtin_amdgcn_readfirstlane(tid >> 6);
+    const int grp = lane >> 4, col = lane & 15;
+
+    StemRegs<1, 1> R;
+    stem_setup<1, 1>(ps, g, R);
+    half8 w1[2][px::kSteps];
+    {
+        const _Float16* __restrict__ w = static_cast<const _Float16*>(p1.wgt);
+#pragma unroll
+        for (int j = 0; j < 2; ++j)
+#pragma unroll
+            for (int kt = 0; kt < px::kSteps; ++kt)
+                w1[j][kt] = *reinterpret_cast<const half8*>(w + (size_t)px::weight_row_channel(j, col) * p1.Kpad + kt * 32 + grp * 8);
+    }
+    float4 b0 = make_float4(0.f, 0.f, 0.f, 0.f), b1 = b0;
+    if (p1.bias) {
+        b0 = *reinterpret_cast<const float4*>(p1.bias + grp * 8);
+        b1 = *reinterpret_cast<const float4*>(p1.bias + grp * 8 + 4);
+    }
+    _Float16* __restrict__ out = static_cast<_Float16*>(p1.out);
+
+    auto fetch = [&](int tile) {
+        const px::Tile t = px::tile_of(tile, g.tiles_x, g.tiles_y);
+        stem_patch_fetch(ps, g, in_bytes, s_patch, t.n, px::patch_start(t.y0), px::patch_aligned_start(px::patch_start(t.x0)));
+    };
+    if ((int)blockIdx.x < total_tiles) fetch(blockIdx.x);
+    for (int tile = blockIdx.x; tile < total_tiles; tile += gridDim.x) {
+        const px::Tile t = px::tile_of(tile, g.tiles_x, g.tiles_y);
+        const int hi_start = px::patch_start(t.y0), wi_start = px::patch_start(t.x0);
+        const int al_start = px::patch_aligned_start(wi_start);
+        const int shift = wi_start - al_start;
+        asm volatile("s_waitcnt vmcnt(0)" ::: "memory");
+        __syncthreads();
+        stem_patch_tail(ps, g, s_patch, t.n, hi_start, al_start);
+        const int iy0 = px::region_start(t.y0), ix0 = px::region_start(t.x0);
+#pragma nounroll
+        for (int gi = wave; gi < px::kGroups; gi += 4) {
+            const px::RegionPixel rp = px::region_pixel(gi, lane);
+            floatx4 acc[1];
+            stem_group_mfma<1, 1>(R, s_patch + px::patch_offset(rp.ry, rp.rx, shift), acc);
+            half4 o = stem_finish4(ps, acc[0], R.bias4[0]);
+            const int iy = iy0 + rp.ry, ix = ix0 + rp.rx;
+            if ((unsigned)iy >= (unsigned)p1.H || (unsigned)ix >= (unsigned)p1.W) o = half4{0, 0, 0, 0};
+            if (rp.live) *reinterpret_cast<half4*>(s_img + px::image_offset(rp.ry, rp.rx, grp * 4)) = o;
+        }
+        __syncthreads();
+        const int next = tile + (int)gridDim.x;
+        if (next < total_tiles) fetch(next);
+        floatx4 acc[2][2];
+#pragma unroll
+        for (int i = 0; i < 2; ++i)
+#pragma unroll
+            for (int j = 0; j < 2; ++j) acc[i][j] = floatx4{0.f, 0.f, 0.f, 0.f};
+#pragma unroll
+        for (int kt = 0; kt < px::kSteps; ++kt) {
+            const int tap = px::step_tap(kt, lane);
+            half8 xf[2];
+#pragma unroll
+            for (int i = 0; i < 2; ++i) {
+                xf[i] = half8{0, 0, 0, 0, 0, 0, 0, 0};
+                if (tap < px::kTaps) xf[i] = *reinterpret_cast<const half8*>(s_img + px::frag_offset(2 * wave + i, col, tap, px::step_chunk(lane)));
+            }
+#pragma unroll
+            for (int j = 0; j < 2; ++j)
+#pragma unroll
+                for (int i = 0; i < 2; ++i) acc[i][j] = __builtin_amdgcn_mfma_f32_16x16x32_f16(w1[j][kt], xf[i], acc[i][j], 0, 0, 0);
+        }
+#pragma unroll
+        for (int i = 0; i < 2; ++i) {
+            const int ho = t.y0 + 2 * wave + i, wo = t.x0 + col;
+            if (ho >= p1.Ho || wo >= p1.Wo) continue;
+            float x[8] = {acc[i][0][0], acc[i][0][1], acc[i][0][2], acc[i][0][3], acc[i][1][0], acc[i][1][1], acc[i][1][2], acc[i][1][3]};
+            if (p1.bias) {
+                x[0] += b0.x; x[1] += b0.y; x[2] += b0.z; x[3] += b0.w;
+                x[4] += b1.x; x[5] += b1.y; x[6] += b1.z; x[7] += b1.w;
+            }
+            half8 v;
+            if (p1.act1 == ACT_SILU) {
+#pragma unroll
+                for (int e = 0; e < 8; ++e) v[e] = round_to_half(x[e] * __builtin_amdgcn_rcpf(1.0f + __expf(-x[e])));
+            } else if (p1.act1 == ACT_RELU) {
+#pragma unroll
+                for (int e = 0; e < 8; ++e) v[e] = round_to_half(x[e] > 0.f ? x[e] : 0.f);
+            } else {
+#pragma unroll
+                for (int e = 0; e < 8; ++e) v[e] = round_to_half(x[e]);
+            }
+            const size_t m = ((size_t)t.n * p1.Ho + ho) * p1.Wo + wo;
+            *reinterpret_cast<half8*>(out + m * p1.ld_out + grp * 8) = v;
+        }
+    }
+}
+
+}
+
+bool conv_stem_pair_possible(const ConvArgs& s, const ConvArgs& c) {
+    const bool stem_ok = conv_stem_supported(s) && !s.f32 && s.Cin <= 4 && s.Cout == 16 && s.kh == 3 && s.kw == 3 && s.stride_h == 2 && s.stride_w == 2 &&
+                         s.pad_h == 1 && s.pad_w == 1 && s.N >= 1 && (size_t)s.N * s.Cin * s.H * s.W * 4 < 2000000000u &&
+                         s.Ho == (s.H - 1) / 2 + 1 && s.Wo == (s.W - 1) / 2 + 1;
+    const bool fast_act = c.act1 == ACT_SILU || c.act1 == ACT_RELU || c.act1 == ACT_NONE;
+    const bool conv_ok = !c.f32 && !c.in_i8 && !c.out_i8 && !c.res_i8 && !c.residual && !c.up_C && c.act2 == ACT_NONE && fast_act && !c.scalar_out &&
+                         c.groups == 1 && c.dil_h == 1 && c.dil_w == 1 && c.Cin == 16 && c.CinK == 16 && c.bk == 32 && c.Kpad == 160 && c.Cout == 32 &&
+                         c.Cout_pad == 32 && c.kh == 3 && c.kw == 3 && c.stride_h == 2 && c.stride_w == 2 && c.pad_h == 1 && c.pad_w == 1 &&
+                         c.ld_out % 8 == 0 && c.ld_out >= 32;
+    const bool chained = c.N == s.N && c.H == s.Ho && c.W == s.Wo && c.Ho == (c.H - 1) / 2 + 1 && c.Wo == (c.W - 1) / 2 + 1;
+    const bool aligned = (reinterpret_cast<uintptr_t>(s.in) & 15) == 0 && (reinterpret_cast<uintptr_t>(c.out) & 15) == 0 &&
+                         (reinterpret_cast<uintptr_t>(c.wgt) & 15) == 0 && (reinterpret_cast<uintptr_t>(c.bias) & 15) == 0;
+    return stem_ok && conv_ok && chained && aligned;
+}
+
+int32_t conv_stem_pair_f16(const ConvArgs& s, const ConvArgs& c, hipStream_t stream) {
+    if (!conv_stem_pair_possible(s, c) || !s.in || !s.wgt || !c.wgt || !c.out) return TRTX_ERR_UNSUPPORTED;
+    namespace px = pairidx;
+    StemGeom g;
+    g.PR = px::kPR;
+    g.PCA = px::kPCA;
+    g.tiles_x = (c.Wo + px::kTW - 1) / px::kTW;
+    g.tiles_y = (c.Ho + px::kTH - 1) / px::kTH;
+    g.chunks = s.Cin * g.PR * g.PCA / 4;
+    const size_t lds = (size_t)((g.chunks + 255) / 256 * 256) * 16 + px::kImageBytes;
+    const unsigned in_bytes = (unsigned)((size_t)s.N * s.Cin * s.H * s.W * 4);
+    const long total_l = (long)s.N * g.tiles_x * g.tiles_y;
+    if (total_l > 0x7fffffffL - 65536) return TRTX_ERR_UNSUPPORTED;
+    const int total = (int)total_l;
+    static thread_local int resident[3] = {-1, 0, 0};
+    int dev = 0;
+    if (hipGetDevice(&dev) != hipSuccess) dev = 0;
+    if (resident[0] != dev || resident[1] != (int)lds || resident[2] <= 0) {
+        int per_cu = 0, cus = 0;
+        if (hipOccupancyMaxActiveBlocksPerMultiprocessor(&per_cu, conv_stem_pair_kernel, 256, lds) != hipSuccess || per_cu < 1) per_cu = 1;
+        if (hipDeviceGetAttribute(&cus, hipDeviceAttributeMultiprocessorCount, dev) != hipSuccess || cus < 1) cus = 256;
+        (void)hipGetLastError();
+        resident[0] = dev;
+        resident[1] = (int)lds;
+        resident[2] = per_cu * cus;
+    }
+    const int grid = total < resident[2] ? total : resident[2];
+    TRTX_LAUNCH(conv_stem_pair_kernel, dim3((unsigned)grid), dim3(256), lds, stream, s, c, g, in_bytes, total);
+    return check_launch("conv_stem_pair_f16");
+}
+
+}
diff --git a/tensorrtx_amd/csrc/kernels/kernels.h b/tensorrtx_amd/csrc/kernels/kernels.h
--- a/tensorrtx_amd/csrc/kernels/kernels.h
+++ b/tensorrtx_amd/csrc/kernels/kernels.h
@@ -108,6 +108,8 @@
     float d2s[6];
 };
 int32_t conv_stem_frames_f32(const ConvArgs& a, const StemFrame* frames, hipStream_t s);
+bool conv_stem_pair_possible(const ConvArgs& stem, const ConvArgs& conv);
+int32_t conv_stem_pair_f16(const ConvArgs& stem, const ConvArgs& conv, hipStream_t s);
 int32_t conv_direct(const ConvArgs& a, int dtype, hipStream_t s);
 bool conv_dw_supported(const ConvArgs& a);
 bool psa_attention_supported(int kd, int hd);
diff --git a/tensorrtx_amd/csrc/kernels/stem_pair_index.h b/tensorrtx_amd/csrc/kernels/stem_pair_index.h
--- /dev/null
+++ b/tensorrtx_amd/csrc/kernels/stem_pair_index.h
@@ -0,0 +1,65 @@
+#pragma once
+
+#if defined(__HIPCC__)
+#define TRTX_HD __host__ __device__ __forceinline__
+#else
+#define TRTX_HD inline
+#endif
+
+namespace trtx {
+namespace pairidx {
+
+constexpr int kTH = 8, kTW = 16;
+constexpr int kRH = 2 * kTH + 1, kRW = 2 * kTW + 1;
+constexpr int kRegion = kRH * kRW;
+constexpr int kGroups = (kRegion + 15) / 16;
+constexpr int kPR = 2 * kRH + 1;
+constexpr int kPC = 2 * kRW + 1;
+constexpr int kPCA = (kPC + 3 + 3) / 4 * 4;
+constexpr int kHalf = (kRW + 1) / 2;
+constexpr int kPixelBytes = 32;
+constexpr int kImageBytes = kRH * 2 * kHalf * kPixelBytes;
+constexpr int kTaps = 9, kSteps = 5;
+
+struct Tile {
+    int n, y0, x0;
+};
+TRTX_HD Tile tile_of(int tile, int tiles_x, int tiles_y) {
+    Tile t;
+    const int tx = tile % tiles_x;
+    const int rest = tile / tiles_x;
+    t.x0 = tx * kTW;
+    t.y0 = (rest % tiles_y) * kTH;
+    t.n = rest / tiles_y;
+    return t;
+}
+TRTX_HD int region_start(int o0) { return 2 * o0 - 1; }
+TRTX_HD int patch_start(int o0) { return 4 * o0 - 3; }
+TRTX_HD int patch_aligned_start(int wi_start) { return (wi_start >= 0 ? wi_start : wi_start - 3) / 4 * 4; }
+
+struct RegionPixel {
+    int ry, rx;
+    bool live;
+};
+TRTX_HD RegionPixel region_pixel(int group, int lane) {
+    const int e = group * 16 + (lane & 15);
+    RegionPixel r;
+    r.live = e < kRegion;
+    const int ee = r.live ? e : kRegion - 1;
+    r.ry = ee / kRW;
+    r.rx = ee - r.ry * kRW;
+    return r;
+}
+TRTX_HD int patch_offset(int ry, int rx, int shift) { return 2 * ry * kPCA + 2 * rx + shift; }
+TRTX_HD int image_offset(int ry, int rx, int ch) { return ((ry * 2 + (rx & 1)) * kHalf + (rx >> 1)) * kPixelBytes + ch * 2; }
+
+TRTX_HD int step_tap(int kt, int lane) { return 2 * kt + ((lane >> 4) >> 1); }
+TRTX_HD int step_chunk(int lane) { return (lane >> 4) & 1; }
+TRTX_HD int frag_offset(int oy, int ox, int tap, int chunk) {
+    const int r = tap / 3, q = tap - r * 3;
+    return image_offset(2 * oy + r, 2 * ox + q, chunk * 8);
+}
+TRTX_HD int weight_row_channel(int j, int a) { return 8 * (a >> 2) + 4 * j + (a & 3); }
+
+}
+}
diff --git a/tensorrtx_amd/csrc/kernels/stem_tile.h b/tensorrtx_amd/csrc/kernels/stem_tile.h
--- /dev/null
+++ b/tensorrtx_amd/csrc/kernels/stem_tile.h
@@ -0,0 +1,144 @@
+#pragma once
+#include <hip/hip_fp16.h>
+#include <hip/hip_runtime.h>
+#include <stdint.h>
+
+#include "../common.h"
+#include "act.h"
+#include "kernels.h"
+
+namespace trtx {
+namespace {
+
+typedef __attribute__((address_space(3))) void* stem_lds_ptr_t;
+
+struct StemGeom {
+    int PR, PCA;
+    int tiles_x, tiles_y;
+    int chunks;
+};
+
+__device__ __forceinline__ void stem_patch_fetch(const ConvArgs& p, const StemGeom& g, unsigned in_bytes, float* s_patch, int n, int hi_start, int al_start) {
+    const int tid = threadIdx.x;
+    const int wave = tid >> 6;
+    const __amdgpu_buffer_rsrc_t rs = __builtin_amdgcn_make_buffer_rsrc(const_cast<void*>(p.in), 0, in_bytes, 0x00020000);
+    const int cpr = g.PCA / 4;
+    const float inv_cpr = 1.0f / (float)cpr, inv_pr = 1.0f / (float)g.PR;
+    for (int base = 0; base < g.chunks; base += 256) {
+        const int ci = base + tid;
+        int row = (int)((float)ci * inv_cpr);
+        int cq = ci - row * cpr;
+        if (cq < 0) { --row; cq += cpr; }
+        if (cq >= cpr) { ++row; cq -= cpr; }
+        int c = (int)((float)row * inv_pr);
+        int pr = row - c * g.PR;
+        if (pr < 0) { --c; pr += g.PR; }
+        if (pr >= g.PR) { ++c; pr -= g.PR; }
+        const int hi = hi_start + pr, wi = al_start + cq * 4;
+        const bool ok = ci < g.chunks && (unsigned)hi < (unsigned)p.H && wi >= 0 && wi + 3 < p.W;
+        const unsigned off = ok ? (unsigned)(((((long)n * p.Cin + c) * p.H + hi) * p.W + wi) * 4) : 0x80000000u;
+        __builtin_amdgcn_raw_ptr_buffer_load_lds(rs, (stem_lds_ptr_t)(s_patch + (size_t)(base + wave * 64) * 4), 16, off, 0, 0, 0);
+    }
+}
+
+__device__ __forceinline__ void stem_patch_tail(const ConvArgs& p, const StemGeom& g, float* s_patch, int n, int hi_start, int al_start) {
+    const int tid = threadIdx.x;
+    if (p.W & 3) {
+        const int cpr = g.PCA / 4, rows = p.Cin * g.PR, wtail = p.W & ~3;
+        const int cq = (wtail - al_start) >> 2;
+        if (cq >= 0 && cq < cpr && wtail >= al_start) {
+            const float* __restrict__ src = static_cast<const float*>(p.in);
+            for (int rrow = tid; rrow < rows; rrow += 256) {
+                const int c = rrow / g.PR, pr = rrow - c * g.PR, hi = hi_start + pr;
+                if ((unsigned)hi >= (unsigned)p.H) continue;
+                const size_t base = (((size_t)n * p.Cin + c) * p.H + hi) * p.W;
+                for (int e = 0; e < 4; ++e)
+                    if (wtail + e < p.W) s_patch[((size_t)rrow * cpr + cq) * 4 + e] = src[base + wtail + e];
+            }
+        }
+        __syncthreads();
+    }
+}
+
+template <int NFRAG, int KS>
+struct StemRegs {
+    half8 wf[NFRAG][KS];
+    int l_off[KS][8];
+    float bias4[NFRAG][4];
+};
+
+template <int NFRAG, int KS>
+__device__ __forceinline__ void stem_setup(const ConvArgs& p, const StemGeom& g, StemRegs<NFRAG, KS>& R) {
+    const int lane = threadIdx.x & 63;
+    const int khw = p.kh * p.kw;
+    const int K = khw * p.Cin;
+    const float* __restrict__ w = static_cast<const float*>(p.wgt);
+    const int kq = (lane >> 4) * 8;
+    auto& wf = R.wf;
+    auto& l_off = R.l_off;
+    auto& bias4 = R.bias4;
+    const float inv_khw = 1.0f / (float)khw, inv_kw = 1.0f / (float)p.kw;
+#pragma unroll
+    for (int ks = 0; ks < KS; ++ks)
+#pragma unroll
+        for (int e = 0; e < 8; ++e) {
+            const int k = ks * 32 + kq + e;
+            const int c = (int)(((float)k + 0.5f) * inv_khw), rem = k - c * khw;
+            const int r = (int)(((float)rem + 0.5f) * inv_kw), q = rem - r * p.kw;
+            l_off[ks][e] = k < K ? (c * g.PR + r) * g.PCA + q : 0;
+#pragma unroll
+            for (int j = 0; j < NFRAG; ++j) {
+                const int co = j * 16 + (lane & 15);
+                const float wv = w[(size_t)(k < K ? k : K - 1) * p.Cout + (co < p.Cout ? co : p.Cout - 1)];
+                wf[j][ks][e] = (k < K && co < p.Cout) ? (_Float16)wv : (_Float16)0.f;
+            }
+        }
+    const int ch4 = (lane >> 4) * 4;
+    const float* __restrict__ bsrc = p.bias ? p.bias : w;
+#pragma unroll
+    for (int j = 0; j < NFRAG; ++j)
+#pragma unroll
+        for (int e = 0; e < 4; ++e) {
+            const int co = j * 16 + ch4 + e;
+            const float bv = bsrc[co < p.Cout ? co : p.Cout - 1];
+            bias4[j][e] = (p.bias && co < p.Cout) ? bv : 0.f;
+        }
+}
+
+template <int NFRAG, int KS>
+__device__ __forceinline__ void stem_group_mfma(const StemRegs<NFRAG, KS>& R, const float* src, floatx4 (&acc)[NFRAG]) {
+#pragma unroll
+    for (int j = 0; j < NFRAG; ++j) acc[j] = floatx4{0.f, 0.f, 0.f, 0.f};
+#pragma unroll
+    for (int ks = 0; ks < KS; ++ks) {
+        half8 xf;
+#pragma unroll
+        for (int e = 0; e < 8; ++e) xf[e] = (_Float16)src[R.l_off[ks][e]];
+#pragma unroll
+        for (int j = 0; j < NFRAG; ++j) acc[j] = __builtin_amdgcn_mfma_f32_16x16x32_f16(R.wf[j][ks], xf, acc[j], 0, 0, 0);
+    }
+}
+
+__device__ __forceinline__ half4 stem_finish4(const ConvArgs& p, const floatx4& acc, const float (&bias4)[4]) {
+    half4 o;
+    if (p.act1 == ACT_SILU) {
+#pragma unroll
+        for (int e = 0; e < 4; ++e) {
+            const float x = acc[e] + bias4[e];
+            o[e] = round_to_half(x * __builtin_amdgcn_rcpf(1.0f + __expf(-x)));
+        }
+    } else if (p.act1 == ACT_RELU) {
+#pragma unroll
+        for (int e = 0; e < 4; ++e) {
+            const float x = acc[e] + bias4[e];
+            o[e] = (_Float16)(x > 0.f ? x : 0.f);
+        }
+    } else {
+#pragma unroll
+        for (int e = 0; e < 4; ++e) o[e] = round_to_half(act_stem(acc[e] + bias4[e], p.act1, p.alpha1));
+    }
+    return o;
+}
+
+}
+}
diff --git a/tensorrtx_amd/csrc/ops_capi.cpp b/tensorrtx_amd/csrc/ops_capi.cpp
--- a/tensorrtx_amd/csrc/ops_capi.cpp
+++ b/tensorrtx_amd/csrc/ops_capi.cpp
@@ -123,6 +123,41 @@
     return st;
 }
 
+static ConvArgs op_stem_args(const float* in, int N, int C, int H, int W, const float* w_taps_cout, const float* bias, int Cout, int k, int stride, int pad, int act) {
+    ConvArgs a{};
+    a.in = in; a.wgt = w_taps_cout; a.bias = bias;
+    a.N = N; a.H = H; a.W = W; a.Cin = C; a.ld_in = C;
+    a.Ho = (H + 2 * pad - k) / stride + 1;
+    a.Wo = (W + 2 * pad - k) / stride + 1;
+    a.Cout = Cout; a.Cout_pad = Cout;
+    a.kh = k; a.kw = k; a.stride_h = stride; a.stride_w = stride; a.pad_h = pad; a.pad_w = pad; a.dil_h = 1; a.dil_w = 1;
+    a.groups = 1;
+    a.K = k * k * C; a.Kpad = a.K;
+    a.M = N * a.Ho * a.Wo;
+    a.act1 = act; a.alpha1 = 0.1f; a.alpha2 = 0.1f;
+    return a;
+}
+
+extern "C" int32_t trtx_op_conv_stem_nchw_f16(const float* in, int N, int C, int H, int W, const float* w_taps_cout, const float* bias, void* out, int Cout,
+                                              int ld_out, int k, int stride, int pad, int act, trtx_stream_t stream) {
+    if (!in || !w_taps_cout || !out || N < 1 || C < 1 || H < 1 || W < 1 || k < 1 || stride < 1 || pad < 0 || H + 2 * pad < k || W + 2 * pad < k) return TRTX_ERR_INVALID;
+    ConvArgs a = op_stem_args(in, N, C, H, W, w_taps_cout, bias, Cout, k, stride, pad, act);
+    a.out = out;
+    a.ld_out = ld_out;
+    return conv_stem_nchw_f32(a, static_cast<hipStream_t>(stream));
+}
+
+extern "C" int32_t trtx_op_conv_stem_pair_f16(const float* in, int N, int C, int H, int W, const float* stem_w_taps_cout, const float* stem_bias, int stem_act,
+                                              const void* conv_wpacked, const float* conv_bias, int conv_act, void* out, int ld_out, trtx_stream_t stream) {
+    if (!in || !stem_w_taps_cout || !conv_wpacked || !out || N < 1 || C < 1 || H < 1 || W < 1) return TRTX_ERR_INVALID;
+    const ConvArgs s = op_stem_args(in, N, C, H, W, stem_w_taps_cout, stem_bias, 16, 3, 2, 1, stem_act);
+    ConvArgs c = op_conv_args(N, s.Ho, s.Wo, 16, 16, 32, ld_out, 3, 3, 2, 2, 1, 1, conv_act, 0, 0, 0);
+    c.wgt = conv_wpacked;
+    c.bias = conv_bias;
+    c.out = out;
+    return conv_stem_pair_f16(s, c, static_cast<hipStream_t>(stream));
+}
+
 extern "C" int32_t trtx_conv_pack_weights_grouped_f16(const float* w_kcrs, int cout, int cin_g, int kh, int kw, const float* ch_scale, uint16_t* packed,
                                                       int32_t* kpad_out) {
     if (!w_kcrs || cout < 1 || cin_g < 1 || kh < 1 || kw < 1) return TRTX_ERR_INVALID;
diff --git a/tensorrtx_amd/csrc/options.cpp b/tensorrtx_amd/csrc/options.cpp
--- a/tensorrtx_amd/csrc/options.cpp
+++ b/tensorrtx_amd/csrc/options.cpp
@@ -28,6 +28,7 @@
     o.lanes = env_int("TRTX_LANES", 0);
     o.group_convs = !env_is("TRTX_GROUP_CONVS", 0);
     o.fold_upsample = !env_is("TRTX_FOLD_UPSAMPLE", 0);
+    o.stem_pair = !env_is("TRTX_STEM_PAIR", 0);
     o.ws = !env_set("TRTX_CONV_NOWS");
     o.wsk = !env_set("TRTX_CONV_NOWSK");
     o.gemm256 = !env_is("TRTX_GEMM256", 0);
diff --git a/tensorrtx_amd/csrc/options.h b/tensorrtx_amd/csrc/options.h
--- a/tensorrtx_amd/csrc/options.h
+++ b/tensorrtx_amd/csrc/options.h
@@ -14,6 +14,7 @@
     int lanes = 0;
     bool group_convs = true;
     bool fold_upsample = true;
+    bool stem_pair = true;
     bool ws = true;
     bool wsk = true;
     bool gemm256 = true;
diff --git a/tensorrtx_amd/csrc/runtime/engine.cpp b/tensorrtx_amd/csrc/runtime/engine.cpp
--- a/tensorrtx_amd/csrc/runtime/engine.cpp
+++ b/tensorrtx_amd/csrc/runtime/engine.cpp
@@ -128,6 +128,8 @@
         return st;
     };
     if (lanes && hipEventRecord(c->start_event, user_stream) != hipSuccess) return bail(TRTX_ERR_HIP);
+    ConvArgs pair_stem{};
+    bool pair_pending = false;
     for (size_t k = 0; k < plan.ops.size(); ++k) {
         const POp& op = plan.ops[k];
         hipStream_t stream = user_stream;
@@ -160,6 +162,27 @@
                 a.cscale = a.in_i8 ? reinterpret_cast<const float*>(W + op.s_off) : nullptr;
                 a.N = op.stem ? (plan.explicit_batch ? (int)t0.dims.d[0] : batch) : nb(t0);
                 a.M = a.N * a.Ho * a.Wo;
+                if (op.stem && !c->frames && !c->observer && !c->tuning && k + 1 < plan.ops.size() && plan.ops[k + 1].stem_pair && plan.ops[k + 1].lane == op.lane) {
+                    const POp& nx = plan.ops[k + 1];
+                    ConvArgs b = nx.conv;
+                    b.out = R.ptr(nx.out[0]);
+                    b.wgt = W + nx.w_off;
+                    b.bias = reinterpret_cast<const float*>(W + nx.b_off);
+                    b.N = nb(to);
+                    b.M = b.N * b.Ho * b.Wo;
+                    if (conv_stem_pair_possible(a, b)) {
+                        pair_stem = a;
+                        pair_pending = true;
+                        break;
+                    }
+                }
+                if (op.stem_pair && pair_pending) {
+                    pair_pending = false;
+                    if (prof && probes[k].start && probes[k].stop) conv_set_launch_probe(&probes[k]);
+                    st = conv_stem_pair_f16(pair_stem, a, stream);
+                    conv_set_launch_probe(nullptr);
+                    break;
+                }
                 if (op.kind == OP_DECONV)
                     st = deconv_direct(a, op.dtype, stream);
                 else if (op.stem && c->frames)
diff --git a/tensorrtx_amd/csrc/runtime/plan.cpp b/tensorrtx_amd/csrc/runtime/plan.cpp
--- a/tensorrtx_amd/csrc/runtime/plan.cpp
+++ b/tensorrtx_amd/csrc/runtime/plan.cpp
@@ -38,7 +38,7 @@
         o << "\",\"flops\":" << op.flops << ",\"bytes\":" << op.bytes;
         auto conv_fields = [&](const POp& op) {
             const ConvArgs& a = op.conv;
-            o << ",\"igemm\":" << (op.igemm ? "true" : "false") << ",\"stem\":" << (op.stem ? "true" : "false") << ",\"cin\":" << (a.in_i8 ? 2 * a.Cin : a.Cin) << ",\"cout\":" << a.Cout
+            o << ",\"igemm\":" << (op.igemm ? "true" : "false") << ",\"stem\":" << (op.stem ? "true" : "false") << (op.stem_pair ? ",\"stem_pair\":true" : "") << ",\"cin\":" << (a.in_i8 ? 2 * a.Cin : a.Cin) << ",\"cout\":" << a.Cout
               << ",\"k\":[" << a.kh << "," << a.kw << "],\"stride\":[" << a.stride_h << "," << a.stride_w << "],\"hw_in\":["
               << a.H << "," << a.W << "],\"hw_out\":[" << a.Ho << "," << a.Wo << "],\"act1\":" << a.act1
               << ",\"act2\":" << a.act2 << ",\"alpha1\":" << a.alpha1 << ",\"alpha2\":" << a.alpha2 << ",\"up_c\":" << a.up_C << ",\"residual\":" << (op.in.size() > 1 ? "true" : "false")
diff --git a/tensorrtx_amd/csrc/runtime/plan.h b/tensorrtx_amd/csrc/runtime/plan.h
--- a/tensorrtx_amd/csrc/runtime/plan.h
+++ b/tensorrtx_amd/csrc/runtime/plan.h
@@ -88,6 +88,7 @@
     ConvArgs conv{};
     bool igemm = false;
     bool stem = false;
+    bool stem_pair = false;
     bool from_deconv = false;
     bool dw = false;
     bool grouped = false;
diff --git a/tensorrtx_amd/csrc/runtime/plan_passes.cpp b/tensorrtx_amd/csrc/runtime/plan_passes.cpp
--- a/tensorrtx_amd/csrc/runtime/plan_passes.cpp
+++ b/tensorrtx_amd/csrc/runtime/plan_passes.cpp
@@ -584,6 +584,40 @@
     plan.ops = std::move(out);
 }
 
+void mark_stem_pair(Plan& plan, const PassInputs& e) {
+    if (!e.opt.stem_pair || e.dt != DT_F16 || e.int8 || CalibrationLowering::active()) return;
+    const int n = (int)plan.ops.size();
+    for (int k = 0; k + 1 < n; ++k) {
+        const POp& st = plan.ops[k];
+        POp& cv = plan.ops[k + 1];
+        if (st.kind != OP_CONV || !st.stem || st.conv.f32 || st.out.size() != 1) continue;
+        if (cv.kind != OP_CONV || !cv.igemm || cv.stem || cv.from_deconv || cv.in.size() != 1 || !cv.extra_in.empty() || cv.in[0] != st.out[0]) continue;
+        const PTensor& mid = plan.tensors[st.out[0]];
+        if (mid.storage < 0 || plan.storages[mid.storage].kind != ST_ARENA || is_binding_tensor(plan, mid.id) || is_binding_tensor(plan, owner_of(plan, mid.id))) continue;
+        bool shared = false;
+        auto touches = [&](const POp& op) {
+            for (const std::vector<int>* v : {&op.in, &op.out, &op.extra_in})
+                for (int t : *v)
+                    if (plan.tensors[t].storage == mid.storage) return true;
+            return false;
+        };
+        for (int j = 0; j < n && !shared; ++j) {
+            if (j == k || j == k + 1) continue;
+            shared = touches(plan.ops[j]);
+            for (const POp& m : plan.ops[j].group) shared = shared || touches(m);
+        }
+        if (shared) continue;
+        ConvArgs a = st.conv, b = cv.conv;
+        const PTensor& t_in = plan.tensors[st.in[0]];
+        a.N = plan.explicit_batch ? (int)t_in.dims.d[0] : plan.max_batch;
+        a.M = a.N * a.Ho * a.Wo;
+        b.N = (mid.nfix ? mid.nfix : plan.max_batch) * mid.nmul;
+        b.M = b.N * b.Ho * b.Wo;
+        if (!conv_stem_pair_possible(a, b)) continue;
+        cv.stem_pair = true;
+    }
+}
+
 void assign_lanes(Plan& plan, const PassInputs& e, const std::vector<std::vector<int>>& deps) {
     const int nops = (int)plan.ops.size();
     int max_lanes = e.max_aux_streams >= 0 ? 1 + e.max_aux_streams : 4;
@@ -696,6 +730,7 @@
     if (!select_conv_kernels(plan, e, err) || !configure_plugins(plan, err)) return false;
     chain_sppf_pools(plan, e);
     group_convs(plan, e);
+    mark_stem_pair(plan, e);
     const std::vector<std::vector<int>> deps = op_dependencies(plan);
     assign_lanes(plan, e, deps);
     plan_arena(plan, ancestors(plan, deps, true));
```
